# crowsonkb/k-diffusion

Measured on AMD Instinct MI355X. Metric: images/sec, 256x256 image_transformer_v2, 50-step DPM++2M (whole job), higher is better.
Workload: dtype f32

## Files before the change

### k-diffusion_amd/csrc/gemm.hip

```cpp
#include "kd_common.h"
#include <cstdlib>
#include <type_traits>

namespace kd {

constexpr int BM = 128, BN = 128, BK = 32;

using bf16x8 = __attribute__((ext_vector_type(8))) __bf16;
using u32x2 = __attribute__((ext_vector_type(2))) unsigned;

constexpr int S = BK + 4;
constexpr int NLD = BM * BK / 4 / 256;
constexpr int RT = BK / 4;
constexpr size_t EPI_STRIPS = 4 * 8 * 64 * sizeof(float);
constexpr size_t LDS_EXACT = (size_t)(2 * BM * S + 2 * BN * S + BM) * sizeof(float);
constexpr int IMG = BM * BK * 2;
constexpr int STAGE = 4 * IMG;
constexpr size_t LDS_SPLIT = (size_t)2 * STAGE + BM * sizeof(float) + EPI_STRIPS;
constexpr int WP_BLOCK = 2 * IMG;
constexpr int SCALE_TAB_MAX_K = 512;

__device__ __host__ __forceinline__ int swz(int row, int c) { return row * 64 + ((c ^ ((row >> 2) & 3)) << 4); }

__device__ __forceinline__ unsigned pack_bf16(float a, float b) {
// ... 180 lines not shown
#pragma unroll
        for (int i = 0; i < 2; ++i)
#pragma unroll
          for (int j = 0; j < 2; ++j) acc[i][j] = __builtin_amdgcn_mfma_f32_32x32x16_bf16(al[i], bh[j], acc[i][j], 0, 0, 0);
#pragma unroll
        for (int i = 0; i < 2; ++i)
#pragma unroll
          for (int j = 0; j < 2; ++j) acc[i][j] = __builtin_amdgcn_mfma_f32_32x32x16_bf16(ah[i], bl[j], acc[i][j], 0, 0, 0);
#pragma unroll
        for (int i = 0; i < 2; ++i)
#pragma unroll
          for (int j = 0; j < 2; ++j) acc[i][j] = __builtin_amdgcn_mfma_f32_32x32x16_bf16(ah[i], bh[j], acc[i][j], 0, 0, 0);
      }
    } else {
      const float* a_base = As + (buf * BM + wr * 64) * S + frag_off;
      const float* b_base = Bs + (buf * BN + wc * 64) * S + frag_off;
#pragma unroll
      for (int kk = 0; kk < BK; kk += 8) {
        const f32x4 a0 = *reinterpret_cast<const f32x4*>(a_base + kk);
        const f32x4 a1 = *reinterpret_cast<const f32x4*>(a_base + 32 * S + kk);
        const f32x4 b0 = *reinterpret_cast<const f32x4*>(b_base + kk);
        const f32x4 b1 = *reinterpret_cast<const f32x4*>(b_base + 32 * S + kk);
#pragma unroll
        for (int s = 0; s < 4; ++s) {
          acc[0][0] = __builtin_amdgcn_mfma_f32_32x32x2f32(a0[s], b0[s], acc[0][0], 0, 0, 0);
          acc[0][1] = __builtin_amdgcn_mfma_f32_32x32x2f32(a0[s], b1[s], acc[0][1], 0, 0, 0);
          acc[1][0] = __builtin_amdgcn_mfma_f32_32x32x2f32(a1[s], b0[s], acc[1][0], 0, 0, 0);
          acc[1][1] = __builtin_amdgcn_mfma_f32_32x32x2f32(a1[s], b1[s], acc[1][1], 0, 0, 0);
        }
      }
    }
  };

  load_a(kt0 * BK, ra0); load_b(kt0, rb0);
  if (nk > 1) { load_a((kt0 + 1) * BK, ra1); load_b(kt0 + 1, rb1); }
  store_tiles(0, kt0 * BK, ra0, rb0);
  __syncthreads();
  for (int kt = 0; kt < nk; kt += 2) {
    if (kt + 2 < nk) { load_a((kt0 + kt + 2) * BK, ra0); load_b(kt0 + kt + 2, rb0); }
    compute(0);
    if (kt + 1 < nk) store_tiles(1, (kt0 + kt + 1) * BK, ra1, rb1);
    __syncthreads();
    if (kt + 1 >= nk) break;
    if (kt + 3 < nk) { load_a((kt0 + kt + 3) * BK, ra1); load_b(kt0 + kt + 3, rb1); }
    compute(1);
    if (kt + 2 < nk) store_tiles(0, (kt0 + kt + 2) * BK, ra0, rb0);
    __syncthreads();
  }

  if (KS == 2) {
    f32x4* xch = reinterpret_cast<f32x4*>(reinterpret_cast<char*>(smem) + 2 * STAGE);
    if (grp == 1) {
#pragma unroll
      for (int i = 0; i < 2; ++i)
#pragma unroll
        for (int j = 0; j < 2; ++j)
#pragma unroll
          for (int q = 0; q < 4; ++q)
            xch[((i * 2 + j) * 4 + q) * 256 + tid] = f32x4{acc[i][j][4 * q], acc[i][j][4 * q + 1], acc[i][j][4 * q + 2], acc[i][j][4 * q + 3]};
    }
    __syncthreads();
    if (grp == 1) return;
#pragma unroll
    for (int i = 0; i < 2; ++i)
#pragma unroll
      for (int j = 0; j < 2; ++j)
#pragma unroll
        for (int q = 0; q < 4; ++q) {
          const f32x4 o = xch[((i * 2 + j) * 4 + q) * 256 + tid];
#pragma unroll
          for (int u = 0; u < 4; ++u) acc[i][j][4 * q + u] += o[u];
        }
  }

  if (NORM) {
#pragma unroll
    for (int j = 0; j < NLD; ++j) {
      const float s = wave_sum_xor(ssq[j], RT);
      if ((tid % RT) == 0) rs[r0 + j * (256 / RT)] = rsqrtf(s / (float)K + p.eps);
    }
    __syncthreads();
  }

  if (p.debug & 1) {
#pragma unroll
    for (int i = 0; i < 2; ++i)
#pragma unroll
      for (int j = 0; j < 2; ++j) asm volatile("" ::"v"(acc[i][j]));
    return;
  }
  const int col_l = lane & 31;
  constexpr int NW = (EPI == KD_EPI_GEGLU) ? 32 : 64;
  const int wn0 = n0 + wc * NW;
  float* strip = ebuf + wid * (8 * 64);
  const bool vec_ok = (N & 3) == 0 &&
                      (EPI != KD_EPI_SPLIT_LERP || (N & 15) == 0) &&
                      (EPI != KD_EPI_UNPATCH_NCHW || (p.pw == 4 && N <= 64 && (p.gw & 7) == 0));
  const int qk_vec = wn0 >> 6, qk_which = EPI == KD_EPI_QKV ? qk_vec / p.n_heads : 2, qk_head = EPI == KD_EPI_QKV ? qk_vec - qk_which * p.n_heads : 0;
  const float qk_sqrt = (EPI == KD_EPI_QKV && qk_which < 2) ? sqrtf(p.qk_scale[qk_head]) : 1.0f;
  if (vec_ok) {
    float c_out[2] = {1.f, 1.f}, c_skip[2] = {0.f, 0.f};
#pragma unroll
    for (int i = 0; i < 2; ++i) {
      float rsv[16];
#pragma unroll
      for (int r = 0; r < 16; ++r) rsv[r] = NORM ? rs[wr * 64 + i * 32 + mfma32_row(r, lane)] : 1.0f;
#pragma unroll
      for (int g = 0; g < 4; ++g) {
        if (EPI == KD_EPI_GEGLU) {
#pragma unroll
          for (int q = 0; q < 4; q += 2) {
            const int r = 4 * g + q, row8 = q + 4 * (lane >> 5);
            const f32x2 rs2 = {rsv[r], rsv[r + 1]};
            const f32x2 gate = f32x2{acc[i][1][r], acc[i][1][r + 1]} * rs2;
            const f32x2 val = f32x2{acc[i][0][r], acc[i][0][r + 1]} * rs2;
            const f32x2 o = (p.debug & 8) ? val * gate : geglu_pair(val * 0.5f, gate);
            strip[row8 * NW + col_l] = o.x;
            strip[(row8 + 1) * NW + col_l] = o.y;
          }
        } else {
#pragma unroll
          for (int q = 0; q < 4; ++q) {
            const int r = 4 * g + q, row8 = q + 4 * (lane >> 5);
            strip[row8 * NW + col_l] = acc[i][0][r] * rsv[r];
            strip[row8 * NW + 32 + col_l] = acc[i][1][r] * rsv[r];
          }
        }
        const int row_base = m0 + wr * 64 + i * 32 + 8 * g;
        if (EPI == KD_EPI_UNPATCH_NCHW) {
          if (wn0 < N) {
            const int items = p.chan * p.ph * 8, hw = p.gh * p.gw;
            for (int it = lane; it < items; it += 64) {
              const int tok = it & 7, cb = it >> 3, c = cb % p.chan, nh = cb / p.chan;
              const int gm = row_base + tok, gmc = min(gm, M - 1);
              const int b = gmc / hw, rr = gmc - b * hw, h = rr / p.gw, w = rr - h * p.gw;
              f32x4 v;
#pragma unroll
              for (int nw = 0; nw < 4; ++nw) v[nw] = strip[tok * NW + (nh * 4 + nw) * p.chan + c];
              const long o = (((long)b * p.chan + c) * (p.gh * p.ph) + h * p.ph + nh) * (p.gw * 4) + w * 4;
              if (p.sigma) {
                const float sg = p.sigma[b], sd = p.sigma_data, var = sg * sg + sd * sd;
                const float co = sg * sd / sqrtf(var), cs = sd * sd / var;
                const f32x4 xin = *reinterpret_cast<const f32x4*>(p.R + o);
                v = v * co + xin * cs;
              }
              if (gm < M) *reinterpret_cast<f32x4*>(p.C + o) = v;
            }
          }
          (void)c_out; (void)c_skip;
          continue;
        }
        constexpr int PER_LANE = NW / 32;
        f32x4 v[PER_LANE], rv[PER_LANE], qcs[PER_LANE], qsn[PER_LANE];
        long off[PER_LANE];
        bool ok[PER_LANE];
#pragma unroll
        for (int t = 0; t < PER_LANE; ++t) {
          const int idx = lane + 64 * t, row8 = idx / (NW / 4), c4 = (idx % (NW / 4)) * 4;
          const int gm = row_base + row8, gn = wn0 + c4;
          ok[t] = gm < M && gn < N;
          const int gmc = min(gm, M - 1), gnc = min(gn, N - 4);
          v[t] = *reinterpret_cast<const f32x4*>(strip + row8 * NW + c4);
          if (EPI == KD_EPI_SPLIT_LERP) {
            const int hw = p.gh * p.gw, Cout = N >> 2;
            const int b = gmc / hw, rr = gmc - b * hw, h = rr / p.gw, w = rr - h * p.gw;
            const int q = gnc / Cout, e = gnc - q * Cout;
            off[t] = (((long)b * (2 * p.gh) + 2 * h + (q >> 1)) * (2 * p.gw) + 2 * w + (q & 1)) * Cout + e;
          } else {
            off[t] = (long)gmc * N + gnc;
          }
          if (EPI == KD_EPI_RESIDUAL || EPI == KD_EPI_SPLIT_LERP) rv[t] = *reinterpret_cast<const f32x4*>(p.R + off[t]);
          if (EPI == KD_EPI_QKV && qk_which < 2) {
            const long tr = ((long)(gmc % p.rows_per_sample) * p.n_heads + qk_head) * KD_ROT + 4 * (lane & 3);
            qcs[t] = *reinterpret_cast<const f32x4*>(p.rope_cos + tr);
            qsn[t] = *reinterpret_cast<const f32x4*>(p.rope_sin + tr);
          }
        }
        if (EPI == KD_EPI_QKV && qk_which < 2) {
#pragma unroll
          for (int t = 0; t < PER_LANE; ++t) v[t] = prep_row16_regs(v[t], lane & 15, qk_sqrt, qcs[t], qsn[t], p.eps);
        }
#pragma unroll
        for (int t = 0; t < PER_LANE; ++t) {
          f32x4 o = v[t];
          if (EPI == KD_EPI_STORE) {
            o = o + p.out_add;
          } else if (EPI == KD_EPI_RESIDUAL) {
            o = o + rv[t];
          } else if (EPI == KD_EPI_SPLIT_LERP) {
            const float fac = *p.fac;
#pragma unroll
            for (int u = 0; u < 4; ++u) {
              const float skip = rv[t][u], diff = o[u] - skip;
              o[u] = (fabsf(fac) < 0.5f) ? skip + fac * diff : o[u] - diff * (1.0f - fac);
            }
          }
          if (EPI == KD_EPI_QKV && SPLIT && p.qkv_packed) {
            u32x2 hi, lo;
            split4(o, hi, lo);
            o = f32x4{__uint_as_float(hi[0]), __uint_as_float(hi[1]), __uint_as_float(lo[0]), __uint_as_float(lo[1])};
          }
          if (ok[t]) *reinterpret_cast<f32x4*>(p.C + off[t]) = o;
        }
      }
    }
    return;
  }

#pragma unroll
  for (int i = 0; i < 2; ++i) {
#pragma unroll
    for (int r = 0; r < 16; ++r) {
      const int row_t = wr * 64 + i * 32 + mfma32_row(r, lane);
      const int gm = m0 + row_t;
      if (gm >= M) continue;
      const float rscale = NORM ? rs[row_t] : 1.0f;
      if (EPI == KD_EPI_GEGLU) {
        const int gn = n0 + wc * 32 + col_l;
        if (gn < N) p.C[(long)gm * N + gn] = (acc[i][0][r] * rscale) * gelu_erf_fast(acc[i][1][r] * rscale);
        continue;
      }
#pragma unroll
      for (int j = 0; j < 2; ++j) {
        const int gn = n0 + wc * 64 + j * 32 + col_l;
        if (gn >= N) continue;
        const float v = acc[i][j][r] * rscale;
        if (EPI == KD_EPI_STORE) {
          p.C[(long)gm * N + gn] = v + p.out_add;
        } else if (EPI == KD_EPI_RESIDUAL) {
          const long o = (long)gm * N + gn;
          p.C[o] = v + p.R[o];
        } else if (EPI == KD_EPI_SPLIT_LERP) {
          const int hw = p.gh * p.gw, Cout = N >> 2;
          const int b = gm / hw, rr = gm % hw, h = rr / p.gw, w = rr % p.gw;
          const int q = gn / Cout, e = gn - q * Cout;
          const long o = (((long)b * (2 * p.gh) + 2 * h + (q >> 1)) * (2 * p.gw) + 2 * w + (q & 1)) * Cout + e;
          const float skip = p.R[o], fac = *p.fac;
          const float diff = v - skip;
          p.C[o] = (fabsf(fac) < 0.5f) ? skip + fac * diff : v - diff * (1.0f - fac);
        } else if (EPI == KD_EPI_UNPATCH_NCHW) {
          const int hw = p.gh * p.gw;
          const int b = gm / hw, rr = gm % hw, h = rr / p.gw, w = rr % p.gw;
          const int c = gn % p.chan, q = gn / p.chan, nh = q / p.pw, nw = q - nh * p.pw;
          const long o = (((long)b * p.chan + c) * (p.gh * p.ph) + h * p.ph + nh) * (p.gw * p.pw) + w * p.pw + nw;
          if (p.sigma) {
            const float sg = p.sigma[b], sd = p.sigma_data;
            const float var = sg * sg + sd * sd;
            const float c_skip = sd * sd / var, c_out = sg * sd / sqrtf(var);
            p.C[o] = v * c_out + p.R[o] * c_skip;
          } else {
            p.C[o] = v;
          }
        }
      }
    }
  }
}

__global__ __launch_bounds__(256) void pack_weight_kernel(const float* __restrict__ W, char* __restrict__ out, int N, int K, int geglu,
                                                           int n_tiles, int nk) {
  const long idx = (long)blockIdx.x * 256 + threadIdx.x;
  const long total = (long)n_tiles * nk * BN * 4;
  if (idx >= total) return;
  const int c = idx & 3, r = (idx >> 2) & (BN - 1);
  const long blk = idx >> 9;
  const int ks = blk % nk, nt = blk / nk;
  const int wrow = w_row_of(nt, r, N, (geglu & 1) != 0);
  float v[8];
#pragma unroll
  for (int u = 0; u < 8; ++u) {
    const int k = ks * BK + ((geglu & 2) ? 16 * (c >> 1) + 4 * (c & 1) + (u & 3) + 8 * (u >> 2) : c * 8 + u);
    v[u] = (wrow >= 0 && k < K) ? W[(long)wrow * K + k] : 0.f;
  }
  u32x2 h0, l0, h1, l1;
  split4(f32x4{v[0], v[1], v[2], v[3]}, h0, l0);
  split4(f32x4{v[4], v[5], v[6], v[7]}, h1, l1);
  char* dst = out + blk * WP_BLOCK + swz(r, c);
  *reinterpret_cast<uint4*>(dst) = uint4{h0[0], h0[1], h1[0], h1[1]};
  *reinterpret_cast<uint4*>(dst + IMG) = uint4{l0[0], l0[1], l1[0], l1[1]};
}

template <int AMODE, bool NORM, int EPI, int PREC, int KS = 1>
static int launch(const GemmP& d, hipStream_t s) {
  constexpr size_t LDS_BASE = PREC == KD_PREC_SPLIT3 ? LDS_SPLIT + (KS - 1) * 2 * STAGE : LDS_EXACT;
  constexpr size_t LDS_BYTES = LDS_BASE + (NORM ? SCALE_TAB_MAX_K * sizeof(float) : 0);
  constexpr int NCOL = (EPI == KD_EPI_GEGLU) ? 64 : BN;
  const long tiles = (long)((d.M + BM - 1) / BM) * ((d.N + NCOL - 1) / NCOL);
  const double n_eff = (EPI == KD_EPI_GEGLU) ? 2.0 * d.N : (double)d.N;
  const ProfName nm("gemm", "gemm_%s<a%d,n%d,e%d%s> M=%d N=%d K=%d", PREC == KD_PREC_SPLIT3 ? "bf16x3" : "f32", AMODE, (int)NORM, EPI, KS == 2 ? ",ks2" : "", d.M, d.N, d.K);
  const double r_bytes = (EPI == KD_EPI_RESIDUAL || EPI == KD_EPI_SPLIT_LERP || (EPI == KD_EPI_UNPATCH_NCHW && d.sigma)) ? 4.0 * d.M * d.N : 0.0;
  LaunchScope prof(nm, 2.0 * d.M * n_eff * d.K, 4.0 * ((double)d.M * d.K + n_eff * d.K + (double)d.M * d.N) + r_bytes, s);
  kd::launch<gemm_kernel<AMODE, NORM, EPI, PREC, KS>>(dim3((unsigned)tiles), dim3(256 * KS), (int)LDS_BYTES, s, d);
  return check_launch("kd_gemm_f32");
}

}

namespace kd { int gemm_astat_try(const GemmP& d, hipStream_t s, int* rc); }
namespace kd { int gemm_x3_try(const GemmP& d, hipStream_t s, int* rc); }
namespace kd { int gemm_x3t_try(const GemmP& d, hipStream_t s, int* rc); }
namespace kd { int gemm_skinny_try(const GemmP& d, hipStream_t s, int* rc); }
namespace kd { int gemm_x3r_try(const GemmP& d, hipStream_t s, int* rc); }
namespace kd { int gemm_x3s_try(const GemmP& d, hipStream_t s, int* rc); }

using namespace kd;

extern "C" int kd_gemm_f32(const KdGemm* dp, void* stream) {
  if (!dp) return fail(KD_EINVAL, "kd_gemm_f32: null descriptor");
  const KdGemm& d = *dp;
  hipStream_t s = (hipStream_t)stream;
  if (d.M <= 0 || d.N <= 0 || d.K <= 0 || (d.K & 3)) return fail(KD_EINVAL, "kd_gemm_f32: bad M/N/K %d/%d/%d (K %% 4 != 0?)", d.M, d.N, d.K);
  if (!d.A || !d.C || (!d.W && d.precision == KD_PREC_EXACT)) return fail(KD_EINVAL, "kd_gemm_f32: null A/W/C");
  if (d.norm && (!d.scale || d.rows_per_sample <= 0 || (d.scale_stride & 3))) return fail(KD_EINVAL, "kd_gemm_f32: norm needs scale, rows_per_sample, scale_stride%%4==0");
  if (d.a_mode != KD_A_PLAIN && (d.gh <= 0 || d.gw <= 0 || d.M % (d.gh * d.gw))) return fail(KD_EINVAL, "kd_gemm_f32: gather mode needs gh, gw with M %% (gh*gw) == 0");
  if (d.a_mode == KD_A_MERGE2x2 && (d.K & 15)) return fail(KD_EINVAL, "kd_gemm_f32: merge needs K %% 16 == 0");
  if (d.a_mode == KD_A_PATCH_NCHW && (d.ph <= 0 || d.pw <= 0 || d.chan <= 0 || d.K != d.ph * d.pw * d.chan)) return fail(KD_EINVAL, "kd_gemm_f32: patch gather needs K == ph*pw*chan");
  if (d.epi == KD_EPI_RESIDUAL && !d.R) return fail(KD_EINVAL, "kd_gemm_f32: residual needs R");
  if (d.epi == KD_EPI_SPLIT_LERP && (!d.R || !d.fac || (d.N & 3) || d.gh <= 0 || d.gw <= 0 || d.M % (d.gh * d.gw))) return fail(KD_EINVAL, "kd_gemm_f32: split needs R, fac, N%%4==0, gh, gw");
  if (d.epi == KD_EPI_UNPATCH_NCHW && (d.ph <= 0 || d.pw <= 0 || d.chan <= 0 || d.N != d.ph * d.pw * d.chan || d.gh <= 0 || d.gw <= 0 || d.M % (d.gh * d.gw) || (d.sigma && !d.R)))
    return fail(KD_EINVAL, "kd_gemm_f32: unpatch needs N == ph*pw*chan, gh, gw (and R when sigma is given)");
  if (d.norm && d.rows_per_sample <= 0) return fail(KD_EINVAL, "kd_gemm_f32: rows_per_sample");
  if (d.epi == KD_EPI_QKV && (d.n_heads <= 0 || d.N != 3 * d.n_heads * 64 || d.rows_per_sample <= 0 || !d.qk_scale || !d.rope_cos || !d.rope_sin))
    return fail(KD_EINVAL, "kd_gemm_f32: qkv epilogue needs N == 3*n_heads*64, rows_per_sample, qk_scale, rope_cos, rope_sin");
  if (d.qkv_packed && (d.epi != KD_EPI_QKV || d.precision != KD_PREC_SPLIT3))
    return fail(KD_EINVAL, "kd_gemm_f32: qkv_packed needs the qkv epilogue and split3 precision");
  if ((d.a_split || d.c_split) && d.precision != KD_PREC_SPLIT3) return fail(KD_EINVAL, "kd_gemm_f32: a_split / c_split are KD_PREC_SPLIT3 operand formats");
  if (d.a_split && (d.norm || d.a_mode != KD_A_PLAIN || !d.A_lo)) return fail(KD_EINVAL, "kd_gemm_f32: a_split needs A_lo, a_mode KD_A_PLAIN and no norm prologue (kd_norm_split_f32 does the norm)");
  if (d.c_split && !d.C_lo) return fail(KD_EINVAL, "kd_gemm_f32: c_split needs C_lo");
  GemmP e;
  static_cast<KdGemm&>(e) = d;
  e.debug = opt(KD_OPT_gemm_debug);
  e.warm = code_warm();
  if (e.rows_per_sample <= 0) e.rows_per_sample = e.M;
  e.scale_tab = e.norm && e.a_mode == KD_A_PLAIN && e.K <= SCALE_TAB_MAX_K && (e.scale_stride == 0 || e.rows_per_sample % BM == 0);

  if (e.a_split) {
    if (e.rows_per_sample <= 0) e.rows_per_sample = e.M;
    int rc = 0;
    if (!gemm_x3t_try(e, s, &rc)) return rc;
    return fail(KD_EINVAL, "kd_gemm_f32: no kernel for pre-split A with epi=%d M=%d N=%d K=%d (K %% 32, N %% 128 (GEGLU: 64))", d.epi, d.M, d.N, d.K);
  }
  {
    const bool skinny_on = opt(KD_OPT_skinny) != 0;
    int rc = 0;
    if (skinny_on && !gemm_skinny_try(e, s, &rc)) return rc;
    if (!gemm_x3s_try(e, s, &rc)) return rc;
  }
  {
    const bool astat_on = opt(KD_OPT_astat) != 0;
    int rc = 0;
    if (astat_on && !gemm_x3_try(e, s, &rc)) return rc;
    if (e.c_split) return fail(KD_EINVAL, "kd_gemm_f32: c_split is produced by the GEGLU projections of gemm_x3.hip (K = 128 / 256, norm) and gemm_x3t.hip (a_split) only");
    if (astat_on && !gemm_astat_try(e, s, &rc)) return rc;
    if (!gemm_x3r_try(e, s, &rc)) return rc;
  }
  if (e.precision != KD_PREC_EXACT && e.precision != KD_PREC_SPLIT3) return fail(KD_EINVAL, "kd_gemm_f32: unknown precision %d", e.precision);
  if (e.precision == KD_PREC_SPLIT3 && !e.Wp) return fail(KD_EINVAL, "kd_gemm_f32: split3 needs the packed weight image Wp (kd_pack_weight_bf16x3)");
  {
    const bool ks_on = opt(KD_OPT_ksplit) != 0;
    const long tiles = (long)((e.M + BM - 1) / BM) * ((e.N + BN - 1) / BN);
    const int nk = (e.K + BK - 1) / BK;
    if (ks_on && e.precision == KD_PREC_SPLIT3 && e.Wp && e.a_mode == KD_A_PLAIN && !e.norm && !e.debug && tiles <= 256 && nk >= 8 && nk % 4 == 0) {
      if (e.epi == KD_EPI_RESIDUAL) return launch<KD_A_PLAIN, false, KD_EPI_RESIDUAL, KD_PREC_SPLIT3, 2>(e, s);
      if (e.epi == KD_EPI_STORE) return launch<KD_A_PLAIN, false, KD_EPI_STORE, KD_PREC_SPLIT3, 2>(e, s);
    }
  }
#define KD_CASE(AM, NO, EP)                                             \
  if (e.a_mode == AM && (e.norm != 0) == NO && e.epi == EP)             \
    return e.precision == KD_PREC_SPLIT3 ? launch<AM, NO, EP, KD_PREC_SPLIT3>(e, s) : launch<AM, NO, EP, KD_PREC_EXACT>(e, s);
  KD_CASE(KD_A_PLAIN, true, KD_EPI_STORE)
  KD_CASE(KD_A_PLAIN, false, KD_EPI_STORE)
  KD_CASE(KD_A_PLAIN, false, KD_EPI_RESIDUAL)
  KD_CASE(KD_A_PLAIN, true, KD_EPI_QKV)
  KD_CASE(KD_A_PLAIN, false, KD_EPI_QKV)
  KD_CASE(KD_A_PLAIN, true, KD_EPI_GEGLU)
  KD_CASE(KD_A_PLAIN, false, KD_EPI_GEGLU)
  KD_CASE(KD_A_MERGE2x2, false, KD_EPI_STORE)
  KD_CASE(KD_A_PLAIN, false, KD_EPI_SPLIT_LERP)
  KD_CASE(KD_A_PATCH_NCHW, false, KD_EPI_STORE)
  KD_CASE(KD_A_PLAIN, true, KD_EPI_UNPATCH_NCHW)
  KD_CASE(KD_A_PLAIN, false, KD_EPI_UNPATCH_NCHW)
#undef KD_CASE
  return fail(KD_EINVAL, "kd_gemm_f32: unsupported combination a_mode=%d norm=%d epi=%d", d.a_mode, d.norm, d.epi);
}

extern "C" long long kd_packed_weight_bytes(int N, int K, int geglu) {
  if (N <= 0 || K <= 0) return 0;
  const long n_tiles = (N + ((geglu & 1) ? 64 : BN) - 1) / ((geglu & 1) ? 64 : BN), nk = (K + BK - 1) / BK;
  return n_tiles * nk * (long long)WP_BLOCK;
}

extern "C" int kd_pack_weight_bf16x3(const float* W, void* out, int N, int K, int geglu, void* stream) {
  if (!W || !out || N <= 0 || K <= 0 || geglu < 0 || geglu > 3) return fail(KD_EINVAL, "kd_pack_weight_bf16x3: bad arguments");
  const int n_tiles = (N + ((geglu & 1) ? 64 : BN) - 1) / ((geglu & 1) ? 64 : BN), nk = (K + BK - 1) / BK;
  const long total = (long)n_tiles * nk * BN * 4;
  hipLaunchKernelGGL(pack_weight_kernel, dim3((unsigned)((total + 255) / 256)), dim3(256), 0, (hipStream_t)stream, W,
                     reinterpret_cast<char*>(out), N, K, geglu, n_tiles, nk);
  return check_launch("kd_pack_weight_bf16x3");
}

KD_TEXT_PAD(gemm)
```

### k-diffusion_amd/csrc/gemm_x3.hip

```cpp
#include "x3_common.h"

namespace kd {
namespace x3 {

struct XArgs {
  const float* A; const char* Wp; float* C;
  b16::u16* Cl; int c_split;
  const float* scale; int scale_stride, rows_per_sample; float eps;
  int M, N, n_tiles, n_splits;
  int n_heads; const float* qk_scale; const float* pos; const float* freq; int qkv_packed;
  float out_add;
  const float* sigma; float sigma_data; int gh, gw, chan;
  const float* R;
  int warm;
  unsigned long long* clk;
};

template <int NC , int EPI>
__global__ __launch_bounds__(256, NC <= 8 ? 2 : 1) void gemm_x3_astat_kernel(const XArgs p) {
  constexpr int K = NC * 16, NK = NC / 2;
  constexpr int NSTG = NC <= 8 ? 4 : 8, PDIST = NSTG - 1, PB = 4;
  constexpr bool GEGLU = EPI == KD_EPI_GEGLU;
  constexpr int NCOL = GEGLU ? 64 : 128;
  constexpr int NST = GEGLU ? 8 : 16;
  constexpr int WAREA = (NSTG / 4) * STG;
  constexpr int KH = WAREA / 128 >= K ? K : WAREA / 128;
  constexpr bool AG = NC >= 32;
  constexpr int NR = K / KH, CPR = KH / 4;
  constexpr int PIECES = 32 * CPR / 64;
  constexpr int SCL = K * 4 < 1024 ? 1024 : K * 4;
  static_assert(NK % NSTG == 0 || NSTG % NK == 0, "ring slot of a stage must be a compile-time constant");
  static_assert(CPR >= 16 && NC % NR == 0, "source-side chunk swizzle spans 16 chunk positions");
  extern __shared__ __attribute__((aligned(16))) char smem[];
  const int tid = threadIdx.x, lane = tid & 63, l31 = lane & 31, lh = lane >> 5;
  const int wid = __builtin_amdgcn_readfirstlane(tid >> 6);
  const auto warm = code_warm_begin<(NC <= 8 ? 14 : 24) * 1024>((int)blockIdx.x < p.warm && tid < 64);
  const PanelSplit ps = panel_split(p.n_splits, p.n_tiles);
  const int nt_begin = ps.t_begin, n_tiles = ps.t_end - ps.t_begin, total = n_tiles * NK;
  const int m0 = ps.panel * 128;
  const bool probe = p.clk && blockIdx.x == 0 && tid == 0;
  if (probe) { p.clk[0] = __builtin_amdgcn_s_memtime(); p.clk[1] = __builtin_amdgcn_s_memrealtime(); }
  const WgStamp wgs = wg_stamp_begin(p.clk);

  f32x16 acc[4];
  if constexpr (EPI == KD_EPI_RESIDUAL) {
    const int rrow = min(m0 + wid * 32 + l31, p.M - 1);
    const float* rp = p.R + (size_t)rrow * p.N + nt_begin * NCOL + 4 * lh;
#pragma unroll
    for (int j = 0; j < 4; ++j)
#pragma unroll
      for (int g = 0; g < 4; ++g) {
        const f32x4 v = *reinterpret_cast<const f32x4*>(rp + 32 * j + 8 * g);
#pragma unroll
        for (int e = 0; e < 4; ++e) acc[j][4 * g + e] = v[e];
      }
  }

  const char* wp = p.Wp + (size_t)nt_begin * NK * STG + wid * (PB * 1024) + lane * 16;
  auto issue_piece = [&](int s_, int j) {
    const int s = min(s_, total - 1);
    const char* src = wp + (size_t)s * STG;
    char* dst = smem + (s_ % NSTG) * STG + wid * (PB * 1024);
    __builtin_amdgcn_global_load_lds((const __attribute__((address_space(1))) void*)(src + j * 1024),
                                     (__attribute__((address_space(3))) void*)(dst + j * 1024), 16, 0, 0);
  };
  auto issue = [&](int s_) {
#pragma unroll
    for (int j = 0; j < PB; ++j) issue_piece(s_, j);
  };

  const int row = m0 + wid * 32 + l31;
  const bool ok = row < p.M;
  const int rowc = ok ? row : p.M - 1;
  bf16x8 a_hi[AG ? 1 : NC], a_lo[AG ? 1 : NC];
  float rs;
  {
    char* stage = smem + wid * WAREA;
    char* scl = smem + NSTG * STG + wid * SCL;
    const int r_first = min(m0 + wid * 32, p.M - 1), r_last = min(m0 + wid * 32 + 31, p.M - 1);
    constexpr bool nrm = EPI != KD_EPI_RESIDUAL;
    const bool uni = nrm && (p.scale_stride == 0 || r_first / p.rows_per_sample == r_last / p.rows_per_sample);
    if (uni) {
      const char* ssrc = reinterpret_cast<const char*>(p.scale + (size_t)(r_first / p.rows_per_sample) * p.scale_stride);
#pragma unroll
      for (int i = 0; i < SCL / 1024; ++i)
        __builtin_amdgcn_global_load_lds((const __attribute__((address_space(1))) void*)(ssrc + (i * 1024 + lane * 16) % (K * 4)),
                                         (__attribute__((address_space(3))) void*)(scl + i * 1024), 16, 0, 0);
    }
    const float* sp = p.scale + (size_t)(rowc / p.rows_per_sample) * p.scale_stride + 8 * lh;
    const float* spl = reinterpret_cast<const float*>(scl) + 8 * lh;
    float ssq = 0.f;
    static_for<NR>([&](auto r_) {
      constexpr int r = decltype(r_)::value;
#pragma unroll
      for (int i = 0; i < PIECES; ++i) {
        const int ci = i * 64 + lane, rr = ci / CPR, qs = ci % CPR;
        const int grow = min(m0 + wid * 32 + rr, p.M - 1);
        const char* src = reinterpret_cast<const char*>(p.A + (size_t)grow * K + r * KH) + ((qs ^ (rr & 15)) << 4);
        __builtin_amdgcn_global_load_lds((const __attribute__((address_space(1))) void*)src,
                                         (__attribute__((address_space(3))) void*)(stage + i * 1024), 16, 0, 0);
      }
      asm volatile("s_waitcnt vmcnt(0)" ::: "memory");
      const char* rowp = stage + l31 * (KH * 4);
      static_for<NC / NR / 4>([&](auto c4_) {
        constexpr int c0 = r * (NC / NR) + 4 * decltype(c4_)::value;
        f32x4 x0[4], x1[4], s0[4], s1[4];
#pragma unroll
        for (int u = 0; u < 4; ++u) {
          const int q = 4 * (c0 - r * (NC / NR) + u) + 2 * lh;
          x0[u] = *reinterpret_cast<const f32x4*>(rowp + ((q ^ (l31 & 15)) << 4));
          x1[u] = *reinterpret_cast<const f32x4*>(rowp + (((q + 1) ^ (l31 & 15)) << 4));
          if constexpr (nrm) {
            if (uni) {
              s0[u] = *reinterpret_cast<const f32x4*>(spl + 16 * (c0 + u));
              s1[u] = *reinterpret_cast<const f32x4*>(spl + 16 * (c0 + u) + 4);
            } else {
              s0[u] = *reinterpret_cast<const f32x4*>(sp + 16 * (c0 + u));
              s1[u] = *reinterpret_cast<const f32x4*>(sp + 16 * (c0 + u) + 4);
            }
          }
        }
        __builtin_amdgcn_sched_barrier(0);
        static_for<4>([&](auto u_) {
          constexpr int u = decltype(u_)::value;
#pragma unroll
          for (int e = 0; e < 4; ++e) ssq = fmaf(x0[u][e], x0[u][e], fmaf(x1[u][e], x1[u][e], ssq));
          u32x4 hi, lo;
          if constexpr (nrm) split8(x0[u] * s0[u], x1[u] * s1[u], hi, lo);
          else split8(x0[u], x1[u], hi, lo);
          if constexpr (AG) {
            areg_write4<8 * (c0 + u)>(hi);
            areg_write4<8 * (c0 + u) + 4>(lo);
          } else {
            asm volatile("" : "+v"(hi), "+v"(lo));
            a_hi[c0 + u] = __builtin_bit_cast(bf16x8, hi);
            a_lo[c0 + u] = __builtin_bit_cast(bf16x8, lo);
          }
        });
        __builtin_amdgcn_sched_barrier(0);
      });
      if constexpr (NR > 1) asm volatile("s_waitcnt lgkmcnt(0)" ::: "memory");
    });
    ssq += __shfl_xor(ssq, 32, 64);
    rs = nrm ? rsqrtf(ssq / (float)K + p.eps) : 1.f;
  }
  float py = 0.f, px = 0.f;
  if (EPI == KD_EPI_QKV) {
    qk_tab_fill(reinterpret_cast<float*>(smem + NSTG * STG + 4 * SCL + 4 * 2048), tid, p);
    token_pos(p.pos, rowc % p.rows_per_sample, py, px);
  }
  code_warm_end(warm);
  asm volatile("s_waitcnt vmcnt(0) lgkmcnt(0)" ::: "memory");
  KD_BARRIER();
  const bool full_panel = m0 + 128 <= p.M;
#pragma unroll
  for (int s = 0; s < PDIST; ++s) issue(s);
  if (probe) p.clk[4] = __builtin_amdgcn_s_memtime();

  const int o0 = swz64(l31, lh), o1 = swz64(l31, 2 + lh);
  char* strip = smem + NSTG * STG + 4 * SCL + wid * 2048;
  const char* qkc = smem + NSTG * STG + 4 * SCL + 4 * 2048;
  float* st_row[2];
  bool st_ok[2];
#pragma unroll
  for (int it = 0; it < 2; ++it) {
    const int r = m0 + wid * 32 + 16 * it + (lane >> 2);
    st_ok[it] = r < p.M;
    st_row[it] = p.C + (size_t)min(r, p.M - 1) * p.N + 4 * (lane & 3);
  }
  if constexpr (EPI != KD_EPI_RESIDUAL) {
#pragma unroll
    for (int j = 0; j < 4; ++j)
#pragma unroll
      for (int r = 0; r < 16; ++r) acc[j][r] = 0.f;
  }
  if constexpr (AG) asm volatile("s_nop 3" : "+v"(acc[0]), "+v"(acc[1]), "+v"(acc[2]), "+v"(acc[3]));

  bf16x8 wh[2][4], wl[2][4];
  int ou0[2] = {0, 0}, ou1[2] = {0, 0};
  if constexpr (EPI == KD_EPI_UNPATCH_NCHW) {
#pragma unroll
    for (int j = 0; j < 2; ++j) {
      const int np = 32 * j + l31, q = np >> 2, py = q / p.chan, cch = q - py * p.chan;
      const int n = np < 16 * p.chan ? (py * 4 + (np & 3)) * p.chan + cch : np;
      ou0[j] = swz64(n, lh);
      ou1[j] = swz64(n, 2 + lh);
    }
  }
  auto read_frags = [&](int slot, int h, bf16x8 (&fh)[4], bf16x8 (&fl)[4]) {
    if constexpr (EPI == KD_EPI_UNPATCH_NCHW) {
#pragma unroll
      for (int j = 0; j < 2; ++j) {
        const char* st = smem + slot * STG + (h ? ou1[j] : ou0[j]);
        fh[j] = *reinterpret_cast<const bf16x8*>(st);
        fl[j] = *reinterpret_cast<const bf16x8*>(st + IMG);
      }
    } else {
      const char* st = smem + slot * STG + (h ? o1 : o0);
#pragma unroll
      for (int j = 0; j < 4; ++j) {
        fh[j] = *reinterpret_cast<const bf16x8*>(st + j * 32 * 64);
        fl[j] = *reinterpret_cast<const bf16x8*>(st + IMG + j * 32 * 64);
      }
    }
  };
  wait_vm(PB * (PDIST - 1));
  KD_BARRIER();
  read_frags(0, 0, wh[0], wl[0]);

  for (int nt = 0; nt < n_tiles; ++nt) {
    static_for<NK>([&](auto ks_) {
      constexpr int ks = decltype(ks_)::value;
      const int s = nt * NK + ks;
      auto mm = [&](auto b_, int j, bool w_lo, auto a_lo_) {
        constexpr int b = decltype(b_)::value, al = decltype(a_lo_)::value, c = 2 * ks + b;
        if (EPI == KD_EPI_UNPATCH_NCHW && j >= 2) return;
        const bf16x8& w = w_lo ? wl[b][j] : wh[b][j];
        if constexpr (AG) mfma_ag<8 * c + 4 * al>(acc[j], w);
        else mfma_a(acc[j], w, al ? a_lo[c] : a_hi[c]);
      };
      constexpr std::integral_constant<int, 0> I0{};
      constexpr std::integral_constant<int, 1> I1{};
      if constexpr (AG) {
        mm(I0, 0, true, I0);
        __builtin_amdgcn_sched_barrier(0);
        read_frags(ks % NSTG, 1, wh[1], wl[1]);
        __builtin_amdgcn_sched_barrier(0);
#pragma unroll
        for (int j = 1; j < 4; ++j) mm(I0, j, true, I0);
      } else {
        read_frags(ks % NSTG, 1, wh[1], wl[1]);
#pragma unroll
        for (int j = 0; j < 4; ++j) mm(I0, j, true, I0);
      }
#pragma unroll
      for (int j = 0; j < 4; ++j) mm(I0, j, false, I1);
#pragma unroll
      for (int j = 0; j < 4; ++j) mm(I0, j, false, I0);
      if constexpr (!AG) {
        __builtin_amdgcn_sched_group_barrier(0x008, 1, 0);
        __builtin_amdgcn_sched_group_barrier(0x100, 8, 0);
        __builtin_amdgcn_sched_group_barrier(0x008, 11, 0);
      }
      __builtin_amdgcn_sched_barrier(0);
      {
        int allow = PB * (PDIST - 2);
        if (full_panel && nt > 0 && ks + 2 <= PDIST) allow += NST;
        wait_vm(allow);
        KD_BARRIER();
      }
      mm(I1, 0, true, I0);
      if constexpr (AG) __builtin_amdgcn_sched_barrier(0);
      read_frags((ks + 1) % NSTG, 0, wh[0], wl[0]);
      if constexpr (!AG) {
        __builtin_amdgcn_sched_group_barrier(0x008, 1, 0);
        __builtin_amdgcn_sched_group_barrier(0x100, 8, 0);
      }
      __builtin_amdgcn_sched_barrier(0);
      mm(I1, 1, true, I0);
      mm(I1, 2, true, I0);
      issue_piece(s + PDIST, 0);
      __builtin_amdgcn_sched_barrier(0);
      mm(I1, 3, true, I0);
      mm(I1, 0, false, I1);
      mm(I1, 1, false, I1);
      issue_piece(s + PDIST, 1);
      __builtin_amdgcn_sched_barrier(0);
      mm(I1, 2, false, I1);
      mm(I1, 3, false, I1);
      mm(I1, 0, false, I0);
      issue_piece(s + PDIST, 2);
      __builtin_amdgcn_sched_barrier(0);
      mm(I1, 1, false, I0);
      mm(I1, 2, false, I0);
      issue_piece(s + PDIST, 3);
      mm(I1, 3, false, I0);
      __builtin_amdgcn_sched_barrier(0);
    });
    if constexpr (AG) asm volatile("s_nop 15\n\ts_nop 3" : "+v"(acc[0]), "+v"(acc[1]), "+v"(acc[2]), "+v"(acc[3]));
    if (probe && nt == 0) p.clk[5] = __builtin_amdgcn_s_memtime();

    const int n0 = (nt_begin + nt) * NCOL;
    auto store_block = [&](const f32x4 (&v)[4], int col) {
#pragma unroll
      for (int hb = 0; hb < 2; ++hb) {
#pragma unroll
        for (int gg = 0; gg < 2; ++gg)
          *reinterpret_cast<f32x4*>(strip + l31 * 64 + (((2 * gg + lh) ^ ((l31 >> 2) & 1)) << 4)) = v[2 * hb + gg];
#pragma unroll
        for (int it = 0; it < 2; ++it) {
          const int r16 = 16 * it + (lane >> 2), c = lane & 3;
          const f32x4 o = *reinterpret_cast<const f32x4*>(strip + r16 * 64 + ((c ^ ((r16 >> 2) & 1)) << 4));
          if (st_ok[it]) st16(st_row[it] + col + 16 * hb, o);
        }
      }
    };
    if (GEGLU) {
      const float rsh = 0.5f * rs;
#pragma unroll
      for (int jj = 0; jj < 2; ++jj) {
        f32x4 blk[4];
#pragma unroll
        for (int g = 0; g < 4; ++g) {
          const f32x2 a = geglu_pair(f32x2{acc[2 * jj][4 * g], acc[2 * jj][4 * g + 1]} * rsh, f32x2{acc[2 * jj + 1][4 * g], acc[2 * jj + 1][4 * g + 1]} * rs);
          const f32x2 b = geglu_pair(f32x2{acc[2 * jj][4 * g + 2], acc[2 * jj][4 * g + 3]} * rsh, f32x2{acc[2 * jj + 1][4 * g + 2], acc[2 * jj + 1][4 * g + 3]} * rs);
          blk[g] = f32x4{a.x, a.y, b.x, b.y};
        }
        if (p.c_split) {
          float v[16], hi[16], lo[16];
#pragma unroll
          for (int g = 0; g < 4; ++g)
#pragma unroll
            for (int q = 0; q < 4; ++q) v[4 * g + q] = blk[g][q];
#pragma unroll
          for (int r = 0; r < 16; r += 2) {
            const unsigned h = pack_bf16(v[r], v[r + 1]);
            hi[r] = b16::bf_lo(h);
            hi[r + 1] = b16::bf_hi(h);
            lo[r] = v[r] - hi[r];
            lo[r + 1] = v[r + 1] - hi[r + 1];
          }
          const size_t off = (size_t)rowc * p.N + n0 + 32 * jj;
          b16::store_block_bf16(reinterpret_cast<b16::u16*>(p.C) + off, hi, lh, ok);
          b16::store_block_bf16(p.Cl + off, lo, lh, ok);
        } else {
          store_block(blk, n0 + 32 * jj);
        }
      }
    } else if (EPI == KD_EPI_QKV) {
#pragma unroll
      for (int vv = 0; vv < 2; ++vv) {
        const int vec = (n0 >> 6) + vv;
        const int which = vec >= 2 * p.n_heads ? 2 : (vec >= p.n_heads ? 1 : 0), head = vec - which * p.n_heads;
        f32x16& a0 = acc[2 * vv];
        f32x16& a1 = acc[2 * vv + 1];
        if (which < 2) {
          qk_prep_head(qkc, head, lh, a0, a1, rs, p.eps, py, px);
        } else {
#pragma unroll
          for (int r = 0; r < 16; ++r) { a0[r] *= rs; a1[r] *= rs; }
        }
#pragma unroll
        for (int jj = 0; jj < 2; ++jj) {
          f32x4 blk[4];
          const f32x16& a = jj ? a1 : a0;
          if (p.qkv_packed) {
#pragma unroll
            for (int g = 0; g < 4; ++g) blk[g] = pack_split4(f32x4{a[4 * g], a[4 * g + 1], a[4 * g + 2], a[4 * g + 3]});
          } else {
#pragma unroll
            for (int g = 0; g < 4; ++g) blk[g] = f32x4{a[4 * g], a[4 * g + 1], a[4 * g + 2], a[4 * g + 3]};
          }
          store_block(blk, n0 + 64 * vv + 32 * jj);
        }
      }
    } else if (EPI == KD_EPI_UNPATCH_NCHW) {
      const int per = p.gh * p.gw, bb = rowc / per, rr = rowc - bb * per, ty = rr / p.gw, tx = rr - ty * p.gw;
      float c_out = 1.f, c_skip = 0.f;
      if (p.sigma) {
        const float sg = p.sigma[bb], sd = p.sigma_data, var = sg * sg + sd * sd;
        c_skip = sd * sd / var;
        c_out = sg * sd / sqrtf(var);
      }
      const int Himg = 4 * p.gh, Wimg = 4 * p.gw;
#pragma unroll
      for (int j = 0; j < 2; ++j)
#pragma unroll
        for (int g = 0; g < 4; ++g) {
          const int q = 8 * j + 2 * g + lh, py = q / p.chan, cch = q - py * p.chan;
          if (q < 4 * p.chan && ok) {
            const size_t o = (((size_t)bb * p.chan + cch) * Himg + 4 * ty + py) * Wimg + 4 * tx;
            f32x4 v = f32x4{acc[j][4 * g], acc[j][4 * g + 1], acc[j][4 * g + 2], acc[j][4 * g + 3]} * (rs * c_out);
            if (p.sigma) v = v + *reinterpret_cast<const f32x4*>(p.R + o) * c_skip;
            st16(p.C + o, v);
          }
        }
    } else {
#pragma unroll
      for (int j = 0; j < 4; ++j) {
        f32x4 blk[4];
#pragma unroll
        for (int g = 0; g < 4; ++g) blk[g] = f32x4{acc[j][4 * g], acc[j][4 * g + 1], acc[j][4 * g + 2], acc[j][4 * g + 3]} * rs + p.out_add;
        store_block(blk, n0 + 32 * j);
      }
    }
    if (probe && nt == 0) p.clk[6] = __builtin_amdgcn_s_memtime();
#pragma unroll
    for (int j = 0; j < 4; ++j)
#pragma unroll
      for (int r = 0; r < 16; ++r) acc[j][r] = 0.f;
    if constexpr (AG) asm volatile("s_nop 3" : "+v"(acc[0]), "+v"(acc[1]), "+v"(acc[2]), "+v"(acc[3]));
  }
  asm volatile("s_waitcnt vmcnt(0)" ::: "memory");
  if (probe) { p.clk[2] = __builtin_amdgcn_s_memtime(); p.clk[3] = __builtin_amdgcn_s_memrealtime(); p.clk[7] = (unsigned long long)total; }
  wg_stamp_end(wgs);
}

template <int EPI>
__global__ __launch_bounds__(256, 2) void gemm_x3h_kernel(const XArgs p) {
  constexpr int NC = 16, K = 256, NK = 8;
  constexpr int NSTG = 4, PDIST = NSTG - 1, PB = 4, UNIT = 4;
  constexpr bool GEGLU = EPI == KD_EPI_GEGLU;
  constexpr int HCOL = GEGLU ? 32 : 64;
  constexpr int NST = GEGLU ? 4 : 8;
  constexpr int KH = 128, NR = K / KH, CPR = KH / 4, PIECES = 32 * CPR / 64, SCL = 1024, SUB = 8192, HALF = 4096, CB = 2;
  extern __shared__ __attribute__((aligned(16))) char smem[];
  const int tid = threadIdx.x, lane = tid & 63, l31 = lane & 31, lh = lane >> 5;
  const int wid = __builtin_amdgcn_readfirstlane(tid >> 6);
  const auto warm = code_warm_begin<20 * 1024>((int)blockIdx.x < p.warm && tid < 64);
  const PanelSplit ps = panel_split(p.n_splits, p.n_tiles);
  const int ht_begin = ps.t_begin, n_ht = ps.t_end - ps.t_begin, total = n_ht * UNIT;
  const int m0 = ps.panel * 128;
  const bool probe = p.clk && blockIdx.x == (gridDim.x * 5) / 8 && tid == 0;
  if (probe) { p.clk[0] = __builtin_amdgcn_s_memtime(); p.clk[1] = __builtin_amdgcn_s_memrealtime(); }
  const WgStamp wgs = wg_stamp_begin(p.clk);

  const char* wp = p.Wp + wid * 1024 + lane * 16;
  auto issue_piece = [&](int q_, int j) {
    const int q = min(q_, total - 1), ht = ht_begin + (q >> 2), u = q & 3;
    const char* src = wp + ((size_t)(ht >> 1) * NK + 2 * u + (j >> 1)) * STG + (j & 1) * IMG + (ht & 1) * HALF;
    char* dst = smem + (q_ % NSTG) * STG + (j >> 1) * SUB + (j & 1) * HALF + wid * 1024;
    __builtin_amdgcn_global_load_lds((const __attribute__((address_space(1))) void*)src, (__attribute__((address_space(3))) void*)dst, 16, 0, 0);
  };

  const int row = m0 + wid * 32 + l31;
  const bool ok = row < p.M;
  const int rowc = ok ? row : p.M - 1;
  float rs;
  {
    char* stage = smem + wid * STG;
    char* scl = smem + NSTG * STG + wid * SCL;
    const int r_first = min(m0 + wid * 32, p.M - 1), r_last = min(m0 + wid * 32 + 31, p.M - 1);
    const bool uni = p.scale_stride == 0 || r_first / p.rows_per_sample == r_last / p.rows_per_sample;
    if (uni) {
      const char* ssrc = reinterpret_cast<const char*>(p.scale + (size_t)(r_first / p.rows_per_sample) * p.scale_stride);
      __builtin_amdgcn_global_load_lds((const __attribute__((address_space(1))) void*)(ssrc + lane * 16),
                                       (__attribute__((address_space(3))) void*)scl, 16, 0, 0);
    }
    const float* sp = p.scale + (size_t)(rowc / p.rows_per_sample) * p.scale_stride + 8 * lh;
    const float* spl = reinterpret_cast<const float*>(scl) + 8 * lh;
    float ssq = 0.f;
    static_for<NR>([&](auto r_) {
      constexpr int r = decltype(r_)::value;
#pragma unroll
      for (int i = 0; i < PIECES; ++i) {
        const int ci = i * 64 + lane, rr = ci / CPR, qs = ci % CPR;
        const int grow = min(m0 + wid * 32 + rr, p.M - 1);
        const char* src = reinterpret_cast<const char*>(p.A + (size_t)grow * K + r * KH) + ((qs ^ (rr & 15)) << 4);
        __builtin_amdgcn_global_load_lds((const __attribute__((address_space(1))) void*)src,
                                         (__attribute__((address_space(3))) void*)(stage + i * 1024), 16, 0, 0);
      }
      asm volatile("s_waitcnt vmcnt(0)" ::: "memory");
      const char* rowp = stage + l31 * (KH * 4);
      static_for<NC / NR / CB>([&](auto c4_) {
        constexpr int c0 = r * (NC / NR) + CB * decltype(c4_)::value;
        f32x4 x0[CB], x1[CB], s0[CB], s1[CB];
#pragma unroll
        for (int u = 0; u < CB; ++u) {
          const int q = 4 * (c0 - r * (NC / NR) + u) + 2 * lh;
          x0[u] = *reinterpret_cast<const f32x4*>(rowp + ((q ^ (l31 & 15)) << 4));
          x1[u] = *reinterpret_cast<const f32x4*>(rowp + (((q + 1) ^ (l31 & 15)) << 4));
          if (uni) {
            s0[u] = *reinterpret_cast<const f32x4*>(spl + 16 * (c0 + u));
            s1[u] = *reinterpret_cast<const f32x4*>(spl + 16 * (c0 + u) + 4);
          } else {
            s0[u] = *reinterpret_cast<const f32x4*>(sp + 16 * (c0 + u));
            s1[u] = *reinterpret_cast<const f32x4*>(sp + 16 * (c0 + u) + 4);
          }
        }
        __builtin_amdgcn_sched_barrier(0);
        static_for<CB>([&](auto u_) {
          constexpr int u = decltype(u_)::value;
#pragma unroll
          for (int e = 0; e < 4; ++e) ssq = fmaf(x0[u][e], x0[u][e], fmaf(x1[u][e], x1[u][e], ssq));
          u32x4 hi, lo;
          split8(x0[u] * s0[u], x1[u] * s1[u], hi, lo);
          areg_write4_lo<8 * (c0 + u)>(hi);
          areg_write4_lo<8 * (c0 + u) + 4>(lo);
        });
        __builtin_amdgcn_sched_barrier(0);
      });
      if constexpr (r + 1 < NR) asm volatile("s_waitcnt lgkmcnt(0)" ::: "memory");
    });
    ssq += __shfl_xor(ssq, 32, 64);
    rs = rsqrtf(ssq / (float)K + p.eps);
  }
  float py = 0.f, px = 0.f;
  if (EPI == KD_EPI_QKV) {
    qk_tab_fill(reinterpret_cast<float*>(smem + NSTG * STG + 4 * SCL + 4 * 2048), tid, p);
    token_pos(p.pos, rowc % p.rows_per_sample, py, px);
  }
  code_warm_end(warm);
  asm volatile("s_waitcnt vmcnt(0) lgkmcnt(0)" ::: "memory");
  KD_BARRIER();
  const bool full_panel = m0 + 128 <= p.M;
#pragma unroll
  for (int s = 0; s < PDIST; ++s)
#pragma unroll
    for (int j = 0; j < PB; ++j) issue_piece(s, j);
  if (probe) p.clk[4] = __builtin_amdgcn_s_memtime();

  const int o0 = swz64(l31, lh), o1 = swz64(l31, 2 + lh);
  char* strip = smem + NSTG * STG + 4 * SCL + wid * 2048;
  const char* qkc = smem + NSTG * STG + 4 * SCL + 4 * 2048;
  float* st_row[2];
  bool st_ok[2];
#pragma unroll
  for (int it = 0; it < 2; ++it) {
    const int r = m0 + wid * 32 + 16 * it + (lane >> 2);
    st_ok[it] = r < p.M;
    st_row[it] = p.C + (size_t)min(r, p.M - 1) * p.N + 4 * (lane & 3);
  }
  f32x16 acc[2];
  bf16x8 uh[2][2], ul[2][2];
  auto read_up = [&](int slot, int cc, bf16x8 (&fh)[2], bf16x8 (&fl)[2]) {
    const char* st = smem + slot * STG + (cc >> 1) * SUB + ((cc & 1) ? o1 : o0);
#pragma unroll
    for (int j = 0; j < 2; ++j) {
      fh[j] = *reinterpret_cast<const bf16x8*>(st + j * 32 * 64);
      fl[j] = *reinterpret_cast<const bf16x8*>(st + HALF + j * 32 * 64);
    }
  };
  auto store_block = [&](const f32x4 (&v)[4], int col) {
#pragma unroll
    for (int hb = 0; hb < 2; ++hb) {
#pragma unroll
      for (int gg = 0; gg < 2; ++gg)
        *reinterpret_cast<f32x4*>(strip + l31 * 64 + (((2 * gg + lh) ^ ((l31 >> 2) & 1)) << 4)) = v[2 * hb + gg];
#pragma unroll
      for (int it = 0; it < 2; ++it) {
        const int r16 = 16 * it + (lane >> 2), c = lane & 3;
        const f32x4 o = *reinterpret_cast<const f32x4*>(strip + r16 * 64 + ((c ^ ((r16 >> 2) & 1)) << 4));
        if (st_ok[it]) st16(st_row[it] + col + 16 * hb, o);
      }
    }
  };
  wait_vm(PB * (PDIST - 1));
  KD_BARRIER();
  read_up(0, 0, uh[0], ul[0]);

  constexpr std::integral_constant<int, 0> I0{};
  constexpr std::integral_constant<int, 1> I1{};
  constexpr std::integral_constant<int, 2> I2{};
  constexpr std::integral_constant<int, 3> I3{};
  constexpr std::integral_constant<int, 4> I4{};
  constexpr std::integral_constant<int, 5> I5{};
  for (int h = 0; h < n_ht; ++h) {
    if (probe && h == 1) p.clk[8] = __builtin_amdgcn_s_memtime();
    static_for<UNIT>([&](auto u_) {
      constexpr int u = decltype(u_)::value;
      const int s = h * UNIT + u;
      auto mm = [&](auto cc_, auto i_) {
        constexpr int cc = decltype(cc_)::value, i = decltype(i_)::value, j = i & 1, term = i >> 1, c = 4 * u + cc;
        const bf16x8& w = term == 0 ? ul[cc & 1][j] : uh[cc & 1][j];
        constexpr int al = term == 1;
        if constexpr (c == 0 && term == 0) mfma_ag0<8 * c + 4 * al>(acc[j], w);
        else mfma_ag<8 * c + 4 * al>(acc[j], w);
      };
      mm(I0, I0);
      __builtin_amdgcn_sched_barrier(0);
      read_up(u, 1, uh[1], ul[1]);
      __builtin_amdgcn_sched_barrier(0);
      mm(I0, I1); mm(I0, I2); mm(I0, I3); mm(I0, I4); mm(I0, I5);
      mm(I1, I0);
      __builtin_amdgcn_sched_barrier(0);
      read_up(u, 2, uh[0], ul[0]);
      __builtin_amdgcn_sched_barrier(0);
      mm(I1, I1); mm(I1, I2); mm(I1, I3); mm(I1, I4); mm(I1, I5);
      __builtin_amdgcn_sched_barrier(0);
      {
        int allow = PB * (PDIST - 2);
        if (full_panel && h > 0 && u + 2 <= PDIST) allow += NST;
        wait_vm(allow);
        KD_BARRIER();
      }
      mm(I2, I0);
      __builtin_amdgcn_sched_barrier(0);
      read_up(u, 3, uh[1], ul[1]);
      __builtin_amdgcn_sched_barrier(0);
      mm(I2, I1); mm(I2, I2);
      issue_piece(s + PDIST, 0);
      __builtin_amdgcn_sched_barrier(0);
      mm(I2, I3); mm(I2, I4); mm(I2, I5);
      issue_piece(s + PDIST, 1);
      __builtin_amdgcn_sched_barrier(0);
      mm(I3, I0);
      __builtin_amdgcn_sched_barrier(0);
      read_up((u + 1) % NSTG, 0, uh[0], ul[0]);
      __builtin_amdgcn_sched_barrier(0);
      mm(I3, I1); mm(I3, I2);
      issue_piece(s + PDIST, 2);
      __builtin_amdgcn_sched_barrier(0);
      mm(I3, I3); mm(I3, I4);
      issue_piece(s + PDIST, 3);
      mm(I3, I5);
      __builtin_amdgcn_sched_barrier(0);
    });
    asm volatile("s_nop 15\n\ts_nop 3" : "+v"(acc[0]), "+v"(acc[1]));
    if (probe && h == 1) p.clk[9] = __builtin_amdgcn_s_memtime();

    const int n0 = (ht_begin + h) * HCOL;
    if (GEGLU) {
      const float rsh = 0.5f * rs;
      f32x4 blk[4];
#pragma unroll
      for (int g = 0; g < 4; ++g) {
        const f32x2 a = geglu_pair(f32x2{acc[0][4 * g], acc[0][4 * g + 1]} * rsh, f32x2{acc[1][4 * g], acc[1][4 * g + 1]} * rs);
        const f32x2 b = geglu_pair(f32x2{acc[0][4 * g + 2], acc[0][4 * g + 3]} * rsh, f32x2{acc[1][4 * g + 2], acc[1][4 * g + 3]} * rs);
        blk[g] = f32x4{a.x, a.y, b.x, b.y};
      }
      store_block(blk, n0);
    } else if (EPI == KD_EPI_QKV) {
      const int vec = n0 >> 6;
      const int which = vec >= 2 * p.n_heads ? 2 : (vec >= p.n_heads ? 1 : 0), head = vec - which * p.n_heads;
      if (which < 2) {
        qk_prep_head(qkc, head, lh, acc[0], acc[1], rs, p.eps, py, px);
      } else {
#pragma unroll
        for (int r = 0; r < 16; ++r) { acc[0][r] *= rs; acc[1][r] *= rs; }
      }
#pragma unroll
      for (int jj = 0; jj < 2; ++jj) {
        f32x4 blk[4];
        const f32x16& a = acc[jj];
        if (p.qkv_packed) {
#pragma unroll
          for (int g = 0; g < 4; ++g) blk[g] = pack_split4(f32x4{a[4 * g], a[4 * g + 1], a[4 * g + 2], a[4 * g + 3]});
        } else {
#pragma unroll
          for (int g = 0; g < 4; ++g) blk[g] = f32x4{a[4 * g], a[4 * g + 1], a[4 * g + 2], a[4 * g + 3]};
        }
        store_block(blk, n0 + 32 * jj);
      }
    } else {
#pragma unroll
      for (int j = 0; j < 2; ++j) {
        f32x4 blk[4];
#pragma unroll
        for (int g = 0; g < 4; ++g) blk[g] = f32x4{acc[j][4 * g], acc[j][4 * g + 1], acc[j][4 * g + 2], acc[j][4 * g + 3]} * rs + p.out_add;
        store_block(blk, n0 + 32 * j);
      }
    }
    if (probe && h == 1) p.clk[10] = __builtin_amdgcn_s_memtime();
  }
  asm volatile("s_waitcnt vmcnt(0)" ::: "memory");
  if (probe) { p.clk[2] = __builtin_amdgcn_s_memtime(); p.clk[3] = __builtin_amdgcn_s_memrealtime(); p.clk[7] = (unsigned long long)total; }
  wg_stamp_end(wgs);
}

unsigned long long* g_clk = nullptr;


template <int NC, int EPI>
static int launch(const XArgs& a0, const char* nm, double flops, double bytes, hipStream_t s, int force_splits = 0) {
  constexpr int K = NC * 16, NSTG = NC <= 8 ? 4 : 8;
  constexpr int LDS = NSTG * STG + 4 * (K * 4 < 1024 ? 1024 : K * 4) + 4 * 2048 + 1024;
  const int panels = (a0.M + 127) / 128, best = best_n_splits(panels, a0.n_tiles, (NC <= 8 ? 2 : 1) * cu_count(), 1);
  const int forced = force_splits ? force_splits : opt(KD_OPT_x3_splits);
  XArgs a = a0;
  a.n_splits = forced > 0 && forced <= a0.n_tiles ? forced : best;
  const CfgName cfg(nm, "splits%d", a.n_splits);
  LaunchScope prof(cfg, flops, bytes, s);
  kd::launch<gemm_x3_astat_kernel<NC, EPI>>(dim3((unsigned)(panels * a.n_splits)), dim3(256), LDS, s, a);
  return check_launch("kd_gemm_f32(x3 astat)");
}

template <int EPI>
static int launch_half(const XArgs& a0, const char* nm, double flops, double bytes, hipStream_t s) {
  constexpr int LDS = 4 * STG + 4 * 1024 + 4 * 2048 + 1024;
  const int panels = (a0.M + 127) / 128, best = best_n_splits(panels, a0.n_tiles, 2 * cu_count(), 2);
  const int forced = opt(KD_OPT_x3_splits);
  XArgs a = a0;
  a.n_splits = forced > 0 && forced <= a0.n_tiles && a0.n_tiles % forced == 0 ? forced : best;
  const CfgName cfg(nm, "splits%d", a.n_splits);
  LaunchScope prof(cfg, flops, bytes, s);
  kd::launch<gemm_x3h_kernel<EPI>>(dim3((unsigned)(panels * a.n_splits)), dim3(256), LDS, s, a);
  return check_launch("kd_gemm_f32(x3 half tiles)");
}

}

int gemm_x3_try(const GemmP& d, hipStream_t s, int* rc) {
  using namespace x3;
  if (!opt(KD_OPT_x3)) return 1;
  if (d.precision != KD_PREC_SPLIT3 || d.a_mode != KD_A_PLAIN || !d.Wp || d.debug) return 1;
  const bool unpatch = d.epi == KD_EPI_UNPATCH_NCHW;
  if (unpatch && (d.K != 128 || !d.norm || d.ph != 4 || d.pw != 4 || d.N != 16 * d.chan || d.N > 64 || !opt(KD_OPT_x3_unpatch))) return 1;
  if (d.epi != KD_EPI_STORE && d.epi != KD_EPI_QKV && d.epi != KD_EPI_GEGLU && d.epi != KD_EPI_RESIDUAL && !unpatch) return 1;
  if (d.epi == KD_EPI_RESIDUAL ? (d.norm || !d.R || d.K != 512 || !opt(KD_OPT_x3_res)) : !d.norm) return 1;
  if (d.K != 128 && d.K != 256 && d.K != 512) return 1;
  const int ncol = d.epi == KD_EPI_GEGLU ? 64 : 128;
  if ((!unpatch && d.N % ncol) || d.M < opt(KD_OPT_x3_min_rows) || (d.norm && d.rows_per_sample <= 0)) return 1;
  if (d.epi == KD_EPI_QKV && (!d.rope_pos || !d.rope_freq || d.n_heads > 16)) return 1;
  if (d.c_split && (d.epi != KD_EPI_GEGLU || !d.C_lo || (d.N & 31))) return 1;
  XArgs a{};
  a.A = d.A; a.Wp = reinterpret_cast<const char*>(d.Wp); a.C = d.C;
  a.scale = d.norm ? d.scale : nullptr; a.R = d.R; a.scale_stride = d.scale_stride; a.rows_per_sample = d.rows_per_sample > 0 ? d.rows_per_sample : d.M; a.eps = d.eps;
  a.M = d.M; a.N = d.N; a.n_tiles = unpatch ? 1 : d.N / ncol; a.n_splits = 1;
  a.sigma = d.sigma; a.sigma_data = d.sigma_data; a.gh = d.gh; a.gw = d.gw; a.chan = d.chan;
// ... 33 lines not shown
```

### k-diffusion_amd/models/image_transformer_v2.py

```python
import ctypes as C
import os
import math
from dataclasses import dataclass
from typing import NamedTuple, Optional, Union

import torch
from torch import nn

from .. import _native as nat
from .. import ops
from .. import weights
from . import axial_rope
from .cond_tables import ScaleTables

D_HEAD = 64
DERIVED_KEPT = 1024
MAX_PLANS = 16
PLAN_SWITCHES = (("KDIFF_ATTN_BLOCK", "1"), ("KDIFF_PROJ_BLOCK", "1"), ("KDIFF_FFN_OUT", "all"), ("KDIFF_RUN_LIST", "1"), ("KDIFF_ATTN_FFN", "1"))
CLASS_IDS_KEPT = 4



@dataclass
class GlobalAttentionSpec:
    d_head: int


@dataclass
class NeighborhoodAttentionSpec:
    d_head: int
    kernel_size: int


@dataclass
class ShiftedWindowAttentionSpec:
    d_head: int
    window_size: int


@dataclass
class NoAttentionSpec:
    pass


@dataclass
class LevelSpec:
    depth: int
    width: int
    d_ff: int
    self_attn: Union[GlobalAttentionSpec, NeighborhoodAttentionSpec, ShiftedWindowAttentionSpec, NoAttentionSpec]
    dropout: float


@dataclass
class MappingSpec:
    depth: int
    width: int
    d_ff: int
    dropout: float



class _Holder(nn.Module):

    def __init__(self, **children):
        super().__init__()
        for k, v in children.items():
            if isinstance(v, nn.Parameter):
                self.register_parameter(k, v)
            elif isinstance(v, torch.Tensor):
                self.register_buffer(k, v)
            else:
                self.add_module(k, v)


def _linear_weight(out_f, in_f, zero=False):
    w = torch.zeros(out_f, in_f)
    if not zero:
        bound = 1.0 / math.sqrt(in_f)
        w.uniform_(-bound, bound)
    return _Holder(weight=nn.Parameter(w))


def _layer(spec: LevelSpec, cond_features: int):
    d, parts = spec.width, {}
    if not isinstance(spec.self_attn, NoAttentionSpec):
        nh = d // spec.self_attn.d_head
        parts["self_attn"] = _Holder(
            scale=nn.Parameter(torch.full([nh], 10.0)),
            norm=_Holder(linear=_linear_weight(d, cond_features, zero=True)),
            qkv_proj=_linear_weight(3 * d, d),
            pos_emb=_Holder(freqs=axial_rope.rope_freqs(spec.self_attn.d_head // 2, nh)),
            out_proj=_linear_weight(d, d, zero=True))
    parts["ff"] = _Holder(norm=_Holder(linear=_linear_weight(d, cond_features, zero=True)),
                          up_proj=_linear_weight(2 * spec.d_ff, d),
                          down_proj=_linear_weight(d, spec.d_ff, zero=True))
    return _Holder(**parts)


def _rms_scale(n):
    return _Holder(scale=nn.Parameter(torch.ones(n)))



_ATTN_KIND = {GlobalAttentionSpec: "global", NeighborhoodAttentionSpec: "neighborhood", ShiftedWindowAttentionSpec: "shifted-window"}
_CORE = {"global": "attn_global", "neighborhood": "attn_na2d", "shifted-window": "attn_window"}


def attn_geometry(spec, index):
    kind = _ATTN_KIND[type(spec)]
    if kind == "global":
        params = ()
    elif kind == "neighborhood":
        params = (spec.kernel_size,)
    else:
        params = (spec.window_size, spec.window_size // 2 if index % 2 == 1 else 0)
    return kind, _CORE[kind], params


class Step(NamedTuple):
    kind: str
    level: int
    prefix: str = ""
    module: Optional[nn.Module] = None
    index: int = 0


def hourglass(model):
    steps, top = [], len(model.level_specs) - 1
    for li in range(top):
        steps += [Step("layer", li, f"down_levels.{li}.{i}.", mod, i) for i, mod in enumerate(model.down_levels[li])]
        steps.append(Step("merge", li))
    steps += [Step("layer", top, f"mid_level.{i}.", mod, i) for i, mod in enumerate(model.mid_level)]
    for li in reversed(range(top)):
        steps.append(Step("split", li))
        depth = model.level_specs[li].depth
        steps += [Step("layer", li, f"up_levels.{li}.{i}.", mod, i + depth) for i, mod in enumerate(model.up_levels[li])]
    return steps


DROPOUT_SITE = 1 << 62


def dropout_sites(model):
    out = []
    for i, st in enumerate(hourglass(model)):
        p = model.level_specs[st.level].dropout if st.kind == "layer" else 0.0
        if p > 0:
            if hasattr(st.module, "self_attn"):
                out.append((DROPOUT_SITE | 2 * i, st, "attn", p))
            out.append((DROPOUT_SITE | (2 * i + 1), st, "ff", p))
    p = model.mapping_spec.dropout
    if p > 0:
        out += [(DROPOUT_SITE | 1 << 32 | k, k, "mapping", p) for k in range(len(model.mapping.blocks))]
    return out


def dropout_table(model, key):
    if key is None:
        return {}
    return {(("mapping", where) if kind == "mapping" else (where.prefix, kind)): (key, site, p) for site, where, kind, p in dropout_sites(model)}


def _level_pos(grids, li):
    h0, w0 = grids[0]
    pos = axial_rope.make_axial_pos(h0, w0).view(h0, w0, 2)
    for _ in range(li):
        pos = axial_rope.downscale_pos(pos)
    return pos



EPS = 1e-6


def conditioning(model, sigma, aug_cond, class_cond, mapping_cond, keep=None, drop=None):
    m = model
    B = sigma.shape[0]
    dev = sigma.device
    ff = ops.fourier_sigma(sigma, m.time_emb.weight.detach().contiguous())
    temb = ops.linear(ff, m.time_in_proj.weight)
    aug = torch.zeros(B, 9, device=dev, dtype=torch.float32) if aug_cond is None else aug_cond.to(device=dev, dtype=torch.float32).reshape(B, 9).contiguous()
    aug_ff = ops.fourier_features(aug, m.aug_emb.weight.detach().contiguous())
    aug_proj = ops.linear(aug_ff, m.aug_in_proj.weight)
    emb = ids = None
    if m.class_emb is not None:
        ids = class_cond.to(device=dev, dtype=torch.int64).reshape(B).contiguous()
        lo, hi = (int(ids.min()), int(ids.max()))
        if lo < 0 or hi >= m.class_emb.weight.shape[0]:
            raise IndexError(f"class_cond ids must lie in [0, {m.class_emb.weight.shape[0] - 1}] (got {lo}..{hi})")
        emb = m.class_emb.weight
    mterm = None
    if m.mapping_cond_in_proj is not None:
        mrows = mapping_cond.to(device=dev, dtype=torch.float32).reshape(B, -1).contiguous()
        mterm = ops.linear(mrows, m.mapping_cond_in_proj.weight)
    c = ops.cond_sum(temb, aug_proj, emb=emb, ids=ids, c=mterm)
    if keep is not None:
        keep.update(time_ff=ff, aug_ff=aug_ff, ids=ids, mapping_rows=mrows if mterm is not None else None, blocks=[])
    c_sum = c
    c = ops.rms_norm(c, m.mapping.in_norm.scale)
    for k, blk in enumerate(m.mapping.blocks):
        if keep is not None:
            keep["blocks"].append(c)
        h = ops.norm_linear(c, blk.norm.scale, blk.up_proj.weight, rows_per_sample=B, epi=nat.EPI_GEGLU)
        dr = drop.get(("mapping", k)) if drop else None
        if dr is not None:
            ops.dropout(h, *dr, out=h)
        c = ops.linear(h, blk.down_proj.weight, residual=c)
    if keep is not None:
        keep.update(c_sum=c_sum, c_last=c)
    return ops.rms_norm(c, m.mapping.out_norm.scale)


def ada_scale(cond, norm):
    return ops.linear(cond, norm.linear.weight, out_add=1.0)




@dataclass(frozen=True)
class LayerRoute:
    qkv: Optional[str]
    core: Optional[str]
    fuse_out: bool
    ff: str
    up: Optional[str] = None
    down_mx8: bool = False
    fuse_core: bool = False


def _prepass(mode, width):
    return mode == nat.PREC_SPLIT3 and width not in (128, 256, 512) and width > 256 and width % 128 == 0 and width <= 2048


def _mx8_ok(lib, mode, M, N, K, epi):
    return mode == nat.PREC_FP8 and M >= lib.kd_get_option(b"mx8_min_rows", nat.OPTION_DEFAULT) and bool(lib.kd_gemm_mx8_supported(M, N, K, epi, 1))


def route_layer(lib, mode, B, T, rps, d, d_ff, nh, attn, switches, grid=None, kernel_size=None):
    bf = mode in (nat.PREC_BF16, nat.PREC_FP8)
    proj_block = bf and switches["KDIFF_PROJ_BLOCK"] != "0"
    ffn_x3 = mode == nat.PREC_SPLIT3 and bool(lib.kd_ffn_f32_supported(T, d, d_ff))
    ffn_bf = bf and bool(lib.kd_ffn_bf16_supported(T, d, d_ff))
    fo = switches["KDIFF_FFN_OUT"]
    fuse_out = attn is not None and ((ffn_x3 and d in (128, 256)) or (ffn_bf and d == 128)) and (d == 128 if fo == "1" else fo in ("all", str(d)))
    qkv = core = None
    if attn is not None:
        if bf and attn == "global" and T % 256 == 0 and switches["KDIFF_ATTN_BLOCK"] != "0" and lib.kd_attn_block_bf16_supported(rps, d, nh) \
                and (B * nh >= 32 or switches["KDIFF_ATTN_BLOCK"] == "force"):
            qkv = "attn_block"
        elif _prepass(mode, d) and nh <= 16:
            qkv = "split"
        elif _mx8_ok(lib, mode, T, 3 * d, d, nat.EPI_QKV):
            qkv = "mx8"
        elif proj_block and lib.kd_proj_block_bf16_supported(rps, d, 3 * d, nat.EPI_QKV) and 192 <= (T // 256) * (3 * d // 384) <= 256:
            qkv = "proj_block"
        else:
            qkv = "plain"
        if qkv != "attn_block":
            core = f"kd_{_CORE[attn]}_{'bf16' if bf else 'f32'}"
    if ffn_x3 or ffn_bf:
        fuse_core = bool(ffn_x3 and fuse_out and attn == "neighborhood" and core == "kd_attn_na2d_f32" and grid is not None
                         and kernel_size is not None and switches.get("KDIFF_ATTN_FFN", "1") != "0"
                         and lib.kd_attn_ffn_f32_supported(B, grid[0], grid[1], nh, kernel_size, d, d_ff))
        return LayerRoute(qkv, core, fuse_out, "kd_ffn_f32" if ffn_x3 else "kd_ffn_bf16", fuse_core=fuse_core)
    if _prepass(mode, d) and d_ff % 64 == 0:
        return LayerRoute(qkv, core, fuse_out, "pair", "split")
    up_mx8 = _mx8_ok(lib, mode, T, d_ff, d, nat.EPI_GEGLU)
    down_mx8 = up_mx8 and d_ff % 128 == 0 and bool(lib.kd_gemm_mx8_supported(T, d, d_ff, nat.EPI_RESIDUAL, 0))
    if up_mx8:
        up = "mx8"
    elif proj_block and lib.kd_proj_block_bf16_supported(rps, d, d_ff, nat.EPI_GEGLU) and 192 <= (T // 256) * (d_ff // 192) <= 256:
        up = "proj_block"
    else:
        up = "plain"
    return LayerRoute(qkv, core, fuse_out, "pair", up, down_mx8)



class _Launch:
    __slots__ = ("name", "args", "what")

    def __init__(self, name, args, what):
        self.name, self.args, self.what = name, args, what

    def __call__(self, lib, stream):
        return getattr(lib, self.name)(*[C.byref(a) if isinstance(a, C.Structure) else a.scale if isinstance(a, _ScaleRef) else a
                                         for a in self.args], stream)


class _ScaleRef:

    def __init__(self):
        self._scale, self._call, self._index = None, None, 0

    def bind_call(self, call, index):
        self._call, self._index = call, index

    @property
    def scale(self):
        return self._scale

    @scale.setter
    def scale(self, v):
        self._scale = v
        if self._call is not None:
            self._call.p[self._index] = v


def _ptr(t):
    return C.c_void_p(t.data_ptr())


class _CondChain:

    def __init__(self, rows, lib):
        self.rows, self.lib, self.launches, self.keep = rows, lib, [], []
        self.c_sigma = self.class_ids = self.aug_in = self.map_in = self.d_scales = None

    def fill(self, sigma, aug_cond, class_cond, mapping_cond, repeat=1):
        rows = self.rows
        self.c_sigma.copy_(sigma.reshape(-1).expand(rows) if sigma.numel() == 1 else sigma.reshape(rows), non_blocking=True)
        B = rows // repeat
        if self.class_ids is not None and class_cond is not None:
            self.class_ids.view(repeat, B).copy_(class_cond.reshape(1, B).expand(repeat, B), non_blocking=True)
        if self.aug_in is not None:
            self.aug_in.view(repeat, B, 9).copy_(aug_cond.reshape(1, B, 9).expand(repeat, B, 9), non_blocking=True)
        if self.map_in is not None:
            self.map_in.view(repeat, B, -1).copy_(mapping_cond.reshape(1, B, -1).expand(repeat, B, -1), non_blocking=True)

    def run(self, table_ptr, stream):
        self.d_scales.C = table_ptr
        for ln in self.launches:
            rc = ln(self.lib, stream)
            if rc:
                nat.check(rc, ln.what)


class _Plan:

    def release(self):
        self.__dict__.clear()

    def __init__(self, model, B, H, W, grids, has_aug, has_class, has_mapping_cond, device, mode, switches):
        self.lib = nat.lib()
        m = self.model = model
        self.mode, self.switches = mode, switches
        self.precision = precision = nat.PREC_BF16 if mode == nat.PREC_FP8 else mode
        bf = precision == nat.PREC_BF16
        self.cond_precision = nat.PREC_SPLIT3 if bf else precision
        self.has_aug, self.has_class, self.has_mapping_cond, self.device = has_aug, has_class, has_mapping_cond, device
        self.keep = []
        self.launches = []
        f32 = dict(device=device, dtype=torch.float32)
        act = dict(device=device, dtype=torch.bfloat16 if bf else torch.float32)
        ph, pw = m.patch_size
        levels = self.levels = m.level_specs
        self.B, self.grids = B, grids
        self.out_shape = (B, m.out_channels, H, W)
        self.class_checked = {}

        self.sigma = torch.empty(B, **f32)
        self.sigma_ptr = self.sigma.data_ptr()
        self.xs = xs = [torch.empty(B, gh, gw, lv.width, **act) for (gh, gw), lv in zip(grids, levels)]
        self.toks = toks = [B * gh * gw for gh, gw in grids]
        self.qkv = torch.empty(max(t * 3 * lv.width for t, lv in zip(toks, levels)), **act)
        self.att = torch.empty(max(t * lv.width for t, lv in zip(toks, levels)), **act)
        self.hid = torch.empty(max(t * lv.d_ff for t, lv in zip(toks, levels)), **act)
        wide = [t * lv.width for t, lv in zip(toks, levels) if _prepass(mode, lv.width)]
        self.xn = torch.empty(max(wide), **f32) if wide else None
        norm_mods = m._ada_norm_modules()
        self.table_offsets, total = {}, 0
        for name, mod in norm_mods:
            self.table_offsets[name] = 4 * total
            total += mod.linear.weight.shape[0]
        wcat = m._packed.get("ada_norm_wcat")
        if wcat is None or wcat.device != device:
            wcat = m._packed["ada_norm_wcat"] = torch.cat([mod.linear.weight.detach() for _, mod in norm_mods], dim=0).contiguous()
        self.wcat = wcat
        self.norm_descs = []
        self.scale_width = total
        self.tables = ScaleTables(B, total, device, self.build_cond)

        L = self.launches
        self.d_patch_in = self._gemm(L, "patch_in", None, m.patch_in.proj.weight, xs[0], toks[0], levels[0].width, m.in_channels * ph * pw,
                                     a_mode=nat.A_PATCH_NCHW, grid=grids[0], patch=(ph, pw, m.in_channels))
        for st in hourglass(m):
            li = st.level
            if st.kind == "layer":
                self._add_layer(li, st.prefix, st.module, st.index)
            elif st.kind == "merge":
                self._gemm(L, f"merges.{li}", xs[li], m.merges[li].proj.weight, xs[li + 1], toks[li + 1], levels[li + 1].width,
                           4 * levels[li].width, a_mode=nat.A_MERGE2x2, grid=grids[li + 1])
            else:
                self._gemm(L, f"splits.{li}", xs[li + 1], m.splits[li].proj.weight, xs[li], toks[li + 1], 4 * levels[li].width,
                           levels[li + 1].width, epi=nat.EPI_SPLIT_LERP, residual=xs[li], fac=m.splits[li].fac, grid=grids[li + 1])
        self.d_patch_out = self._gemm(L, "patch_out", xs[0], m.patch_out.proj.weight, None, toks[0], m.out_channels * ph * pw,
                                      levels[0].width, epi=nat.EPI_UNPATCH_NCHW, norm_scale=m.out_norm.scale, scale_stride=0,
                                      rows_per_sample=grids[0][0] * grids[0][1], grid=grids[0], patch=(ph, pw, m.out_channels))
        self._encode_launches()

    def _gemm(self, launches, what, A, Wt, Cc, M, N, K, cond=False, table=None, entry=None, mx8=False, **kw):
        precision = self.cond_precision if cond else self.precision
        if table is not None:
            kw.update(scale_ptr=0, scale_stride=self.scale_width)
        d = ops.gemm(A, Wt, Cc, M=M, N=N, K=K, precision=precision, per_row=cond, mx8=mx8, launch=False, pack=self.model._packed_image, **kw)
        if table is not None:
            self.norm_descs.append((d, self.table_offsets[table]))
        launches.append(_Launch(entry or ops._gemm_entry(precision, mx8), (d,), what + ("(mx8)" if mx8 else "")))
        return d

    def _norm_split(self, launches, table, x, T, d, rps):
        ref = _ScaleRef()
        self.norm_descs.append((ref, self.table_offsets[table]))
        planes = self.xn.view(torch.bfloat16)
        hi, lo = planes[:T * d], planes[T * d:2 * T * d]
        launches.append(_Launch("kd_norm_split_f32", (_ptr(x), ref, self.scale_width, rps, _ptr(hi), _ptr(lo), T, d, 1e-6), table + " (split)"))
        return hi, lo

    def build_cond(self, rows):
        m, f32 = self.model, dict(device=self.device, dtype=torch.float32)
        mw, mdff = m.mapping_spec.width, m.mapping_spec.d_ff
        ch = _CondChain(rows, self.lib)
        L = ch.launches
        ch.c_sigma = torch.empty(rows, **f32)
        ch.class_ids = torch.zeros(rows, device=self.device, dtype=torch.int64)
        ch.aug_in = torch.zeros(rows, 9, **f32) if self.has_aug else None
        ch.map_in = torch.zeros(rows, m.mapping_cond_dim, **f32) if self.has_mapping_cond else None
        ff, temb, emb, mres, cond = (torch.empty(rows, mw, **f32) for _ in range(5))
        mh = torch.empty(rows, mdff, **f32)
        ch.keep += [ff, temb, emb, mres, cond, mh]
        L.append(_Launch("kd_fourier_sigma_f32", (_ptr(ch.c_sigma), _ptr(m.time_emb.weight), _ptr(ff), rows, mw // 2), "fourier_sigma"))
        self._gemm(L, "time_in_proj", ff, m.time_in_proj.weight, temb, rows, mw, mw, cond=True)
        if self.has_aug:
            aug_ff, aug_proj = torch.empty(rows, mw, **f32), torch.empty(rows, mw, **f32)
            ch.keep += [aug_ff, aug_proj]
            L.append(_Launch("kd_fourier_f32", (_ptr(ch.aug_in), _ptr(m.aug_emb.weight), _ptr(aug_ff), rows, 9, mw // 2), "fourier_aug"))
            self._gemm(L, "aug_in_proj", aug_ff, m.aug_in_proj.weight, aug_proj, rows, mw, mw, cond=True)
            aug_term, aug_rows = aug_proj, 1
        else:
            z_ff, aug_const = torch.empty(1, mw, **f32), torch.empty(1, mw, **f32)
            zeros9 = torch.zeros(1, 9, **f32)
            ch.keep += [z_ff, aug_const, zeros9]
            L.append(_Launch("kd_fourier_f32", (_ptr(zeros9), _ptr(m.aug_emb.weight), _ptr(z_ff), 1, 9, mw // 2), "fourier_aug0"))
            self._gemm(L, "aug_in_proj0", z_ff, m.aug_in_proj.weight, aug_const, 1, mw, mw, cond=True)
            aug_term, aug_rows = aug_const, 0
        map_term = None
        if self.has_mapping_cond:
            map_term = torch.empty(rows, mw, **f32)
            ch.keep.append(map_term)
            self._gemm(L, "mapping_cond_in_proj", ch.map_in, m.mapping_cond_in_proj.weight, map_term, rows, mw, m.mapping_cond_dim, cond=True)
        L.append(_Launch("kd_cond_sum_f32", (_ptr(emb), _ptr(temb), _ptr(aug_term), aug_rows,
                                             _ptr(m.class_emb.weight) if self.has_class else None, _ptr(ch.class_ids) if self.has_class else None,
                                             None if map_term is None else _ptr(map_term), rows, mw), "cond_sum"))
        L.append(_Launch("kd_rmsnorm_f32", (_ptr(emb), _ptr(m.mapping.in_norm.scale), _ptr(mres), rows, mw, C.c_float(1e-6)), "mapping.in_norm"))
        for blk in m.mapping.blocks:
            self._gemm(L, "mapping.up_proj", mres, blk.up_proj.weight, mh, rows, mdff, mw, cond=True, epi=nat.EPI_GEGLU,
                       norm_scale=blk.norm.scale, scale_stride=0, rows_per_sample=rows)
            self._gemm(L, "mapping.down_proj", mh, blk.down_proj.weight, mres, rows, mw, mdff, cond=True, epi=nat.EPI_RESIDUAL, residual=mres)
        L.append(_Launch("kd_rmsnorm_f32", (_ptr(mres), _ptr(m.mapping.out_norm.scale), _ptr(cond), rows, mw, C.c_float(1e-6)), "mapping.out_norm"))
        ch.d_scales = self._gemm(L, "ada_norm_scales", cond, self.wcat, None, rows, self.scale_width, mw, cond=True, out_add=1.0)
        return ch

    def _qk(self, li, sa, nh):
        m = self.model
        if self.precision == nat.PREC_BF16:
            cos_t, sin_t = m._rope(li, self.grids, sa, self.device, revs=True)
        else:
            cos_t, sin_t = m._rope(li, self.grids, sa, self.device)
        self.keep += [cos_t, sin_t]
        qk = (sa.scale, cos_t, sin_t, nh)
        if self.precision == nat.PREC_SPLIT3:
            pos_t, freq_t = m._rope(li, self.grids, sa, self.device, revs=True)
            self.keep += [pos_t, freq_t]
            qk += (pos_t, freq_t)
        return qk

    def _add_layer(self, li, prefix, mod, index):
        L, lv, (gh, gw), T = self.launches, self.levels[li], self.grids[li], self.toks[li]
        d, d_ff, x, rps = lv.width, lv.d_ff, self.xs[li], gh * gw
        spec = lv.self_attn
        nh = d // spec.d_head if hasattr(mod, "self_attn") else 0
        kind, core, params = attn_geometry(spec, index) if nh else (None, None, ())
        r = route_layer(self.lib, self.mode, self.B, T, rps, d, d_ff, nh, kind, self.switches, grid=(gh, gw),
                        kernel_size=params[0] if kind == "neighborhood" else None)
        split3 = self.precision == nat.PREC_SPLIT3
        if nh:
            sa, norm = mod.self_attn, prefix + "self_attn.norm"
            q = dict(epi=nat.EPI_QKV, rows_per_sample=rps, qk=self._qk(li, sa, nh), qkv_packed=split3)
            if r.qkv == "attn_block":
                self._gemm(L, prefix + "attn_block", x, sa.qkv_proj.weight, self.att, T, 3 * d, d, table=norm, entry="kd_attn_block_bf16", **q)
            elif r.qkv == "split":
                planes = self._norm_split(L, norm, x, T, d, rps)
                self._gemm(L, prefix + "qkv_proj", None, sa.qkv_proj.weight, self.qkv, T, 3 * d, d, a_planes=planes, **q)
            elif r.qkv == "proj_block":
                self._gemm(L, prefix + "qkv_proj(block)", x, sa.qkv_proj.weight, self.qkv, T, 3 * d, d, table=norm, entry="kd_proj_block_bf16", **q)
            else:
                self._gemm(L, prefix + "qkv_proj", x, sa.qkv_proj.weight, self.qkv, T, 3 * d, d, table=norm, mx8=r.qkv == "mx8", **q)
            if r.core is not None and not r.fuse_core:
                geo = ((rps, nh) if kind == "global" else (gh, gw, nh)) + params
                prep = () if r.core.endswith("_bf16") else (2 if split3 else 0, None, None, None, C.c_float(1e-6), self.precision)
                L.append(_Launch(r.core, (_ptr(self.qkv), _ptr(self.att), self.B, *geo, *prep), prefix + core))
            if not r.fuse_out:
                self._gemm(L, prefix + "out_proj", self.att, sa.out_proj.weight, x, T, d, d, epi=nat.EPI_RESIDUAL, residual=x)
        norm, w_up, w_down = prefix + "ff.norm", mod.ff.up_proj.weight, mod.ff.down_proj.weight
        if r.ff != "pair":
            fd = ops.ffn(x, None, w_up, w_down, out=x, scale_stride=self.scale_width, rows_per_sample=rps, attn=self.att if r.fuse_out else None,
                         w_out=mod.self_attn.out_proj.weight if r.fuse_out else None, launch=False, pack=self.model._packed_image)
            self.norm_descs.append((fd, self.table_offsets[norm]))
            if r.fuse_core:
                L.append(_Launch("kd_attn_ffn_f32", (_ptr(self.qkv), fd, self.B, gh, gw, nh, *params), prefix + core + "+ff"))
            else:
                L.append(_Launch(r.ff, (fd,), prefix + "ff"))
            return
        hid8 = None
        if r.up == "split":
            planes = self._norm_split(L, norm, x, T, d, rps)
            self._gemm(L, prefix + "up_proj", None, w_up, self.hid, T, d_ff, d, epi=nat.EPI_GEGLU, a_planes=planes)
        else:
            if r.down_mx8:
                b = self.hid.view(torch.uint8)
                hid8 = (b[:T * d_ff], b[T * d_ff:T * d_ff + T * d_ff // 32])
            block = r.up == "proj_block"
            self._gemm(L, prefix + ("up_proj(block)" if block else "up_proj"), x, w_up, self.hid, T, d_ff, d, epi=nat.EPI_GEGLU, table=norm,
                       rows_per_sample=rps, mx8=r.up == "mx8", c_planes=hid8, entry="kd_proj_block_bf16" if block else None)
        if r.down_mx8:
            self._gemm(L, prefix + "down_proj", None, w_down, x, T, d, d_ff, epi=nat.EPI_RESIDUAL, residual=x, a_planes=hid8, mx8=True)
        else:
            self._gemm(L, prefix + "down_proj", self.hid, w_down, x, T, d, d_ff, epi=nat.EPI_RESIDUAL, residual=x)

    def run(self, x, out, sigma_data, base):
        for d, off in self.norm_descs:
            d.scale = base + off
        pin, pout = self.d_patch_in, self.d_patch_out
        pin.A = x.data_ptr()
        pout.C = out.data_ptr()
        if sigma_data is None:
            pin.sigma, pout.sigma, pout.R = None, None, None
        else:
            sp = self.sigma_ptr
            pin.sigma, pout.sigma, pout.R = sp, sp, x.data_ptr()
            pin.sigma_data = pout.sigma_data = float(sigma_data)
        stream = C.c_void_p(torch.cuda.current_stream().cuda_stream)
        if self.calls is not None:
            rc = self.run_list(self.calls, len(self.launches), stream, C.byref(self.failed))
            if rc:
                nat.check(rc, self.launches[self.failed.value].what)
            return
        for ln in self.launches:
            rc = ln(self.lib, stream)
            if rc:
                nat.check(rc, ln.what)

    def _encode_launches(self):
        self.calls, self.failed, self.run_list = None, C.c_int(0), self.lib.kd_run_list
        if self.switches["KDIFF_RUN_LIST"] == "0" or not self.launches:
            return
        calls = (nat.KdCall * len(self.launches))()
        for call, ln in zip(calls, self.launches):
            if not nat.encode_call(call, ln.name, ln.args):
                return
        self.calls = calls



def _wants_input_grad(x):
    return torch.is_grad_enabled() and isinstance(x, torch.Tensor) and x.requires_grad


class _InputGrad(torch.autograd.Function):

    @staticmethod
    def forward(ctx, x, model, sigma, aug_cond, class_cond, mapping_cond, sigma_data):
        for name, t in (("sigma", sigma), ("aug_cond", aug_cond), ("class_cond", class_cond), ("mapping_cond", mapping_cond)):
            if isinstance(t, torch.Tensor) and t.requires_grad:
                raise NotImplementedError(f"ImageTransformerDenoiserModelV2: gradients w.r.t. {name} are not implemented (the backward pass "
                                          f"differentiates w.r.t. the input x only); pass {name}.detach()")
        out = model._run(x, sigma, aug_cond, class_cond, mapping_cond, sigma_data)
        ctx.model, ctx.sigma_data = model, sigma_data
        ctx.save_for_backward(x, sigma, aug_cond, class_cond, mapping_cond)
        return out

    @staticmethod
    def backward(ctx, grad):
        from . import vjp
        x, sigma, aug_cond, class_cond, mapping_cond = ctx.saved_tensors
        gx = vjp.backward(ctx.model, x, sigma, grad.to(torch.float32).contiguous(), aug_cond=aug_cond, class_cond=class_cond,
                          mapping_cond=mapping_cond, sigma_data=ctx.sigma_data)
        return gx, None, None, None, None, None, None


class _ParamGrad(torch.autograd.Function):

    @staticmethod
    def forward(ctx, x, model, sigma, aug_cond, class_cond, mapping_cond, key, *params):
        from . import vjp
        out = vjp.primal(model, x, sigma, aug_cond, class_cond, mapping_cond, dropout=key)
        ctx.model, ctx.params = model, params
        ctx.save_for_backward(x, sigma, aug_cond, class_cond, mapping_cond, key)
        return out

    @staticmethod
    def backward(ctx, grad):
        from . import vjp
        x, sigma, aug_cond, class_cond, mapping_cond, key = ctx.saved_tensors
        need = ctx.needs_input_grad[7:]
        want = [p for p, n in zip(ctx.params, need) if n]
        _, grads = vjp.backward(ctx.model, x, sigma, grad.to(torch.float32).contiguous(), aug_cond=aug_cond, class_cond=class_cond,
                                mapping_cond=mapping_cond, params=want, dropout=key)
        return (None,) * 7 + tuple(grads.get(id(p)) if n else None for p, n in zip(ctx.params, need))


class ImageTransformerDenoiserModelV2(nn.Module):
    def __init__(self, levels, mapping, in_channels, out_channels, patch_size, num_classes=0, mapping_cond_dim=0):
        super().__init__()
        for lv in levels:
            sa = lv.self_attn
            if not isinstance(sa, (GlobalAttentionSpec, NeighborhoodAttentionSpec, ShiftedWindowAttentionSpec, NoAttentionSpec)):
                raise ValueError(f"unsupported self attention spec {sa}")
            if not isinstance(sa, NoAttentionSpec) and sa.d_head != D_HEAD:
                raise ValueError(f"d_head must be {D_HEAD} (got {sa.d_head}): the HIP kernels of both arithmetic modes -- qkv epilogue (cosine-sim "
                                 f"norm + RoPE over {D_HEAD // 2} dims), attention cores, qkv layout [tokens, 3, n_heads, {D_HEAD}] of "
                                 f"include/kdiff_hip.h -- are built for {D_HEAD}-dim heads, as every shipped config uses (config.py:137-138); "
                                 f"the reference's other head sizes (image_transformer_v2.py:355-363) are not supported")
            if not isinstance(sa, NoAttentionSpec) and lv.width % sa.d_head:
                raise ValueError(f"width {lv.width} is not a multiple of d_head {sa.d_head}")
        self.level_specs, self.mapping_spec = list(levels), mapping
        self.in_channels, self.out_channels = in_channels, out_channels
        self.patch_size = (patch_size, patch_size) if isinstance(patch_size, int) else tuple(patch_size)
        self.num_classes, self.mapping_cond_dim = num_classes, mapping_cond_dim
        ph, pw = self.patch_size
        mw = mapping.width

        self.patch_in = _Holder(proj=_linear_weight(levels[0].width, in_channels * ph * pw))
        self.time_emb = _Holder(weight=torch.randn(mw // 2, 1))
        self.time_in_proj = _linear_weight(mw, mw)
        self.aug_emb = _Holder(weight=torch.randn(mw // 2, 9))
        self.aug_in_proj = _linear_weight(mw, mw)
        self.class_emb = _Holder(weight=nn.Parameter(torch.randn(num_classes, mw))) if num_classes else None
        self.mapping_cond_in_proj = _linear_weight(mw, mapping_cond_dim) if mapping_cond_dim else None
        self.mapping = _Holder(
            in_norm=_rms_scale(mw),
            blocks=nn.ModuleList([_Holder(norm=_rms_scale(mw), up_proj=_linear_weight(2 * mapping.d_ff, mw),
                                          down_proj=_linear_weight(mw, mapping.d_ff, zero=True)) for _ in range(mapping.depth)]),
            out_norm=_rms_scale(mw))
        self.down_levels, self.up_levels = nn.ModuleList(), nn.ModuleList()
        for i, lv in enumerate(levels):
            if i < len(levels) - 1:
                self.down_levels.append(nn.ModuleList([_layer(lv, mw) for _ in range(lv.depth)]))
                self.up_levels.append(nn.ModuleList([_layer(lv, mw) for _ in range(lv.depth)]))
            else:
                self.mid_level = nn.ModuleList([_layer(lv, mw) for _ in range(lv.depth)])
        self.merges = nn.ModuleList([_Holder(proj=_linear_weight(b.width, 4 * a.width)) for a, b in zip(levels[:-1], levels[1:])])
        self.splits = nn.ModuleList([_Holder(proj=_linear_weight(4 * a.width, b.width), fac=nn.Parameter(torch.ones(1) * 0.5))
                                     for a, b in zip(levels[:-1], levels[1:])])
        self.out_norm = _rms_scale(levels[0].width)
        self.patch_out = _Holder(proj=_linear_weight(out_channels * ph * pw, levels[0].width, zero=True))
        self._watch, self._plan_cache = weights.WeightWatch(self), weights.PlanCache()
        self._plans = self._plan_cache.plans
        self._fingerprint, self._packed, self._derived, self._plans_epoch = None, {}, {}, None
        self._dropout_on, self._dropout_gen = False, None
        self.wgrad_arithmetic = None

    def _ada_norm_modules(self):
        out = []

        def visit(prefix, layers):
            for i, mod in enumerate(layers):
                if hasattr(mod, "self_attn"):
                    out.append((f"{prefix}{i}.self_attn.norm", mod.self_attn.norm))
                out.append((f"{prefix}{i}.ff.norm", mod.ff.norm))
        for li, lvl in enumerate(self.down_levels):
            visit(f"down_levels.{li}.", lvl)
        for li, lvl in enumerate(self.up_levels):
            visit(f"up_levels.{li}.", lvl)
        visit("mid_level.", self.mid_level)
        return out

    def _derive(self, tag, sources, build):
        key = (tag, *[weights.ident(t, never_same=False) for t in sources])
        ent = self._derived.get(key)
        if ent is None:
            if len(self._derived) >= DERIVED_KEPT:
                self._derived.clear()
            ent = self._derived[key] = (sources, build())
        return ent[1]

    def _rope(self, li, grids, sa, device, revs=False):
        freqs = sa.pos_emb.freqs

        def build():
            pos = _level_pos(grids, li)
            if revs:
                freq = freqs.detach().to(torch.float32).cpu() / (2.0 * math.pi)
                return pos.reshape(-1, 2).to(torch.float32).contiguous().to(device), freq.contiguous().to(device)
            cos_t, sin_t = axial_rope.rope_tables(pos, freqs.detach())
            return cos_t.to(device), sin_t.to(device)
        return self._derive(("rope", li, grids[0], device, revs), (freqs,), build)

    def _drop_plans(self):
        self._plan_cache.drop_all()

    def invalidate(self):
        self._watch.bump()
        self._derived = {}

    def _apply(self, fn, *args, **kwargs):
        out = super()._apply(fn, *args, **kwargs)
        self._watch.bump()
        return out

    def _packed_image(self, W, N, K, geglu, bf16=False):
        key = (id(W), N, K, int(geglu), bf16 if bf16 == "mx8" else bool(bf16))
        ent = self._packed.get(key)
        if ent is None:
            ent = self._packed[key] = (W, ops.pack_weight(W, N, K, geglu, cache=False, bf16=bf16))
        return ent[1]

    def _weights_fingerprint(self):
        return self._watch.fingerprint()

    def _param_tags(self, name):
        tags = set()
        if name.endswith(".weight") and not name.startswith(("time_in_proj.", "aug_in_proj.", "class_emb.", "mapping_cond_in_proj.")):
            tags.add("wd")
        if name.startswith("mapping.") or name.endswith(".norm.linear.weight"):
            tags.add("mapping")
        return tags

    def param_groups(self, base_lr=5e-4, mapping_lr_scale=1 / 3):
        groups = {(wd, mp): [] for mp in (False, True) for wd in (True, False)}
        for name, p in self.named_parameters():
            tags = self._param_tags(name)
            groups[("wd" in tags, "mapping" in tags)].append(p)
        return [
            {"params": groups[(True, False)], "lr": base_lr},
            {"params": groups[(False, False)], "lr": base_lr, "weight_decay": 0.0},
            {"params": groups[(True, True)], "lr": base_lr * mapping_lr_scale},
            {"params": groups[(False, True)], "lr": base_lr * mapping_lr_scale, "weight_decay": 0.0},
        ]

    def _dropout_rates(self):
        return [(f"levels[{i}].dropout", lv.dropout) for i, lv in enumerate(self.level_specs)] + [("mapping dropout", self.mapping_spec.dropout)]

    def enable_dropout(self, generator=None):
        bad = [f"{name} = {p}" for name, p in self._dropout_rates() if not 0.0 <= p < 1.0]
        if bad:
            raise ValueError(f"ImageTransformerDenoiserModelV2.enable_dropout: dropout rates must lie in [0, 1) ({', '.join(bad)})")
        if generator is not None and not isinstance(generator, torch.Generator):
            raise TypeError(f"enable_dropout: generator must be a torch.Generator or None (got {type(generator)})")
        self._dropout_on, self._dropout_gen = True, generator
        return self

    def set_wgrad_arithmetic(self, arithmetic=None):
        if arithmetic not in (None, "bf16"):
            raise ValueError(f"ImageTransformerDenoiserModelV2.set_wgrad_arithmetic: {arithmetic!r} (None or 'bf16')")
        self.wgrad_arithmetic = arithmetic
        return self

    def _dropout_applies(self):
        return self.training and any(p > 0 for _, p in self._dropout_rates())

    def _refuse_when_dropping(self, what):
        if self._dropout_on and self._dropout_applies():
            raise NotImplementedError(f"ImageTransformerDenoiserModelV2.{what}: dropout is enabled and the model is in training mode, and this "
                                      f"pass has no dropout; call model.eval() first (dropout applies to loss_forward / Denoiser.loss only)")

    def loss_forward(self, x, sigma, aug_cond=None, class_cond=None, mapping_cond=None):
        key = None
        if self._dropout_applies():
            if not self._dropout_on:
                drop = [f"{name} = {p}" for name, p in self._dropout_rates() if p > 0]
                raise NotImplementedError(f"ImageTransformerDenoiserModelV2: dropout in training mode needs model.enable_dropout() "
                                          f"({', '.join(drop)}; masks from this project's counter-based generator); or call model.eval() "
                                          f"for the dropout-free objective")
            if isinstance(x, torch.Tensor) and x.is_cuda:
                key = torch.randint(-2 ** 63, 2 ** 63 - 1, (1,), dtype=torch.int64, device=x.device, generator=self._dropout_gen)
        params = [p for p in self.parameters() if p.requires_grad] if torch.is_grad_enabled() else []
        if params:
            return _ParamGrad.apply(x, self, sigma, aug_cond, class_cond, mapping_cond, key, *params)
        from . import vjp
        return vjp.primal(self, x, sigma, aug_cond, class_cond, mapping_cond, dropout=key)

    def forward(self, x, sigma, aug_cond=None, class_cond=None, mapping_cond=None):
        self._refuse_when_dropping("forward")
        if _wants_input_grad(x):
            return _InputGrad.apply(x, self, sigma, aug_cond, class_cond, mapping_cond, None)
        return self._run(x, sigma, aug_cond, class_cond, mapping_cond, None)

    def forward_preconditioned(self, x, sigma, sigma_data, aug_cond=None, class_cond=None, mapping_cond=None):
        self._refuse_when_dropping("forward_preconditioned")
        if _wants_input_grad(x):
            return _InputGrad.apply(x, self, sigma, aug_cond, class_cond, mapping_cond, sigma_data)
        return self._run(x, sigma, aug_cond, class_cond, mapping_cond, sigma_data)

    def forward_jvp(self, x, sigma, x_dot, aug_cond=None, class_cond=None, mapping_cond=None, sigma_data=None):
        self._refuse_when_dropping("forward_jvp")
        from . import jvp
        return jvp.forward_jvp(self, x, sigma, x_dot, aug_cond=aug_cond, class_cond=class_cond, mapping_cond=mapping_cond, sigma_data=sigma_data)

    def _check_input(self, x, class_cond, mapping_cond, subject, other=None):
# ... 116 lines not shown
```

### k-diffusion_amd/ops.py

```python
import ctypes as C
import os

import math

import torch

from . import _native as nat
from . import weights


def _stream():
    return C.c_void_p(torch.cuda.current_stream().cuda_stream)


def _chk(t, name, dtype=torch.float32):
    if not isinstance(t, torch.Tensor):
        raise TypeError(f"{name}: expected a tensor, got {type(t)}")
    if not t.is_cuda:
        raise RuntimeError(f"{name}: the HIP path needs a tensor on a ROCm device (got {t.device}); there is no CPU fallback")
    if t.dtype != dtype:
        raise TypeError(f"{name}: expected {dtype}, got {t.dtype}")
    if not t.is_contiguous():
        raise ValueError(f"{name}: tensor must be contiguous")
    return t


def _p(t):
    return None if t is None else C.c_void_p(t.data_ptr())


_packed = weights.WeakCache()


def pack_weight(W, N, K, geglu, cache=True, bf16=False):
    geglu = int(geglu)

    def build():
        _chk(W, "W")
        lib = nat.lib()
        if bf16 == "mx8":
            size = lib.kd_packed_weight_bytes_mx8(N, K, geglu)
            if size <= 0:
                raise ValueError(f"kd_pack_weight_mx8: N={N} K={K} is not taken (K must be a multiple of 128)")
            img = torch.empty(size, device=W.device, dtype=torch.uint8)
            nat.check(lib.kd_pack_weight_mx8(_p(W), _p(img), N, K, geglu, _stream()), "kd_pack_weight_mx8")
        elif bf16:
            img = torch.empty(lib.kd_packed_weight_bytes_bf16(N, K, geglu), device=W.device, dtype=torch.uint8)
            nat.check(lib.kd_pack_weight_bf16(_p(W), _p(img), N, K, geglu, _stream()), "kd_pack_weight_bf16")
        else:
            img = torch.empty(lib.kd_packed_weight_bytes(N, K, geglu), device=W.device, dtype=torch.uint8)
            nat.check(lib.kd_pack_weight_bf16x3(_p(W), _p(img), N, K, geglu, _stream()), "kd_pack_weight_bf16x3")
        return img
    return _packed.get(W, (bf16 if bf16 == "mx8" else bool(bf16), geglu), (N, K), build, cache=cache)


def gemm(A, W, out, *, M, N, K, a_mode=nat.A_PLAIN, epi=nat.EPI_STORE, norm_scale=None, scale_stride=0,
         rows_per_sample=0, residual=None, grid=(0, 0), patch=(0, 0, 0), eps=1e-6, out_add=0.0,
         sigma=None, sigma_data=1.0, fac=None, scale_ptr=None, precision=None, qk=None, qkv_packed=False, per_row=False,
         a_planes=None, c_planes=None, launch=True, mx8=False, pack=pack_weight):
    d = nat.KdGemm()
    d.per_row = 1 if per_row else 0
    d.precision = nat.kernel_precision() if precision is None else precision
    bf = d.precision == nat.PREC_BF16
    act = torch.bfloat16 if bf else torch.float32
    a_dt = torch.float32 if a_mode == nat.A_PATCH_NCHW else act
    c_dt = torch.float32 if epi == nat.EPI_UNPATCH_NCHW else act
    if mx8:
        if not bf:
            raise TypeError("mx8: bf16 activations only (precision=PREC_BF16)")
        d.Wp = pack(W, N, K, epi == nat.EPI_GEGLU, bf16="mx8").data_ptr()
    elif bf:
        d.Wp = pack(W, N, K, epi == nat.EPI_GEGLU, bf16=True).data_ptr()
    elif d.precision == nat.PREC_SPLIT3:
        d.Wp = pack(W, N, K, epi == nat.EPI_GEGLU).data_ptr()
    d.M, d.N, d.K = M, N, K
    d.a_mode, d.epi = a_mode, epi
    d.norm = 1 if (norm_scale is not None or scale_ptr is not None) else 0
    d.rows_per_sample, d.scale_stride = rows_per_sample, scale_stride
    d.gh, d.gw = grid
    d.ph, d.pw, d.chan = patch
    d.eps, d.out_add, d.sigma_data = eps, out_add, sigma_data
    d.W = _chk(W, "W").data_ptr()
    if a_planes is not None and mx8:
        d.a_split, d.A, d.A_lo = 1, _chk(a_planes[0], "A e4m3", torch.uint8).data_ptr(), _chk(a_planes[1], "A scales", torch.uint8).data_ptr()
    elif a_planes is not None:
        d.a_split, d.A, d.A_lo = 1, _chk(a_planes[0], "A hi", torch.bfloat16).data_ptr(), _chk(a_planes[1], "A lo", torch.bfloat16).data_ptr()
    elif A is not None or launch:
        d.A = _chk(A, "A", a_dt).data_ptr()
    if c_planes is not None and mx8:
        d.c_split, d.C, d.C_lo = 1, _chk(c_planes[0], "C e4m3", torch.uint8).data_ptr(), _chk(c_planes[1], "C scales", torch.uint8).data_ptr()
        out = c_planes
    elif c_planes is not None:
        d.c_split, d.C, d.C_lo = 1, _chk(c_planes[0], "C hi", torch.bfloat16).data_ptr(), _chk(c_planes[1], "C lo", torch.bfloat16).data_ptr()
        out = c_planes
    elif out is not None or launch:
        d.C = _chk(out, "C", c_dt).data_ptr()
    d.R = None if residual is None else _chk(residual, "R", c_dt).data_ptr()
    d.scale = scale_ptr if scale_ptr is not None else (None if norm_scale is None else _chk(norm_scale, "scale").data_ptr())
    d.sigma = None if sigma is None else _chk(sigma, "sigma").data_ptr()
    d.fac = None if fac is None else _chk(fac, "fac").data_ptr()
    if qk is not None and bf:
        d.qk_scale, d.rope_pos, d.rope_freq = (_chk(t, n).data_ptr() for t, n in zip(qk[:3], ("qk_scale", "rope_pos", "rope_freq")))
        d.n_heads = qk[3]
    elif qk is not None:
        d.qk_scale, d.rope_cos, d.rope_sin = (_chk(t, n).data_ptr() for t, n in zip(qk[:3], ("qk_scale", "cos", "sin")))
        d.n_heads = qk[3]
        if len(qk) >= 6:
            d.rope_pos, d.rope_freq = _chk(qk[4], "rope_pos").data_ptr(), _chk(qk[5], "rope_freq").data_ptr()
        d.qkv_packed = 1 if qkv_packed else 0
    if not launch:
        return d
    name = _gemm_entry(d.precision, mx8)
    nat.check(getattr(nat.lib(), name)(C.byref(d), _stream()), name)
    return out


def _gemm_entry(precision, mx8=False):
    return "kd_gemm_mx8" if mx8 else ("kd_gemm_bf16" if precision == nat.PREC_BF16 else "kd_gemm_f32")


def _prec_of(x):
    if x.dtype == torch.bfloat16:
        return nat.PREC_BF16
    p = nat.kernel_precision()
    return nat.PREC_SPLIT3 if p == nat.PREC_BF16 else p


def linear(x, weight, residual=None, out=None, out_add=0.0):
    K = x.shape[-1]
    M = x.numel() // K
    Nn = weight.shape[0]
    out = torch.empty(*x.shape[:-1], Nn, device=x.device, dtype=x.dtype) if out is None else out
    return gemm(x, weight, out, M=M, N=Nn, K=K, epi=nat.EPI_RESIDUAL if residual is not None else nat.EPI_STORE,
                residual=residual, out_add=out_add, precision=_prec_of(x))


def linear_geglu(x, weight, out=None):
    K = x.shape[-1]
    M = x.numel() // K
    d_ff = weight.shape[0] // 2
    out = torch.empty(*x.shape[:-1], d_ff, device=x.device, dtype=x.dtype) if out is None else out
    return gemm(x, weight, out, M=M, N=d_ff, K=K, epi=nat.EPI_GEGLU, precision=_prec_of(x))


def norm_split(x, scale=None, *, rows_per_sample=0, eps=1e-6):
    K = x.shape[-1]
    M = x.numel() // K
    hi, lo = torch.empty(x.shape, device=x.device, dtype=torch.bfloat16), torch.empty(x.shape, device=x.device, dtype=torch.bfloat16)
    stride = 0 if scale is None or scale.dim() == 1 else K
    nat.check(nat.lib().kd_norm_split_f32(_p(_chk(x, "x")), None if scale is None else _p(_chk(scale, "scale")), stride, rows_per_sample or M,
                                          _p(hi), _p(lo), M, K, eps, _stream()), "kd_norm_split_f32")
    return hi, lo


def rms_norm(x, scale, eps=1e-6, out=None):
    d = x.shape[-1]
    out = torch.empty_like(x) if out is None else out
    nat.check(nat.lib().kd_rmsnorm_f32(_p(_chk(x, "x")), _p(_chk(scale, "scale")), _p(_chk(out, "y")), x.numel() // d, d, eps, _stream()),
            "kd_rmsnorm_f32")
    return out


def norm_linear(x, scale, weight, *, rows_per_sample, epi=nat.EPI_STORE, out=None, eps=1e-6, qk=None, qkv_packed=False, mx8=False, c_fp8=False):
    K = x.shape[-1]
    M = x.numel() // K
    Nn = weight.shape[0] // (2 if epi == nat.EPI_GEGLU else 1)
    if c_fp8:
        planes = (torch.empty(*x.shape[:-1], Nn, device=x.device, dtype=torch.uint8), torch.empty(*x.shape[:-1], Nn // 32, device=x.device, dtype=torch.uint8))
        return gemm(x, weight, None, M=M, N=Nn, K=K, epi=epi, norm_scale=scale, scale_stride=K if scale.dim() == 2 else 0,
                    rows_per_sample=rows_per_sample, eps=eps, precision=_prec_of(x), mx8=True, c_planes=planes)
    out = torch.empty(*x.shape[:-1], Nn, device=x.device, dtype=x.dtype) if out is None else out
    return gemm(x, weight, out, M=M, N=Nn, K=K, epi=epi, norm_scale=scale, scale_stride=K if scale.dim() == 2 else 0,
                rows_per_sample=rows_per_sample, eps=eps, qk=qk, qkv_packed=qkv_packed, precision=_prec_of(x), mx8=mx8)


def linear_mx8(a8, a_scales, weight, residual=None, out=None):
    K = a8.shape[-1]
    M = a8.numel() // K
    Nn = weight.shape[0]
    out = torch.empty(*a8.shape[:-1], Nn, device=a8.device, dtype=torch.bfloat16) if out is None else out
    return gemm(None, weight, out, M=M, N=Nn, K=K, epi=nat.EPI_RESIDUAL if residual is not None else nat.EPI_STORE, residual=residual,
                precision=nat.PREC_BF16, mx8=True, a_planes=(a8, a_scales))


def attn_block(x, scale, weight, *, rows_per_sample, qk, out=None, eps=1e-6):
    K = x.shape[-1]
    M = x.numel() // K
    out = torch.empty_like(x) if out is None else out
    d = gemm(x, weight, out, M=M, N=3 * K, K=K, epi=nat.EPI_QKV, norm_scale=scale, scale_stride=K, rows_per_sample=rows_per_sample, eps=eps,
             qk=qk, precision=nat.PREC_BF16, launch=False)
    nat.check(nat.lib().kd_attn_block_bf16(C.byref(d), _stream()), "kd_attn_block_bf16")
    return out


def proj_block(x, scale, weight, *, rows_per_sample, epi=nat.EPI_GEGLU, qk=None, out=None, eps=1e-6):
    K = x.shape[-1]
    M = x.numel() // K
    N = weight.shape[0] // (2 if epi == nat.EPI_GEGLU else 1)
    out = torch.empty(*x.shape[:-1], N, device=x.device, dtype=x.dtype) if out is None else out
    d = gemm(x, weight, out, M=M, N=N, K=K, epi=epi, norm_scale=scale, scale_stride=K, rows_per_sample=rows_per_sample, eps=eps, qk=qk,
             precision=nat.PREC_BF16, launch=False)
    nat.check(nat.lib().kd_proj_block_bf16(C.byref(d), _stream()), "kd_proj_block_bf16")
    return out


def token_merge(x, weight, out=None):
    B, H2, W2, Cc = x.shape
    h, w = H2 // 2, W2 // 2
    Nn = weight.shape[0]
    out = torch.empty(B, h, w, Nn, device=x.device, dtype=x.dtype) if out is None else out
    return gemm(x, weight, out, M=B * h * w, N=Nn, K=4 * Cc, a_mode=nat.A_MERGE2x2, grid=(h, w), precision=_prec_of(x))


def token_split_lerp(x, weight, skip, fac, out=None):
    B, h, w, K = x.shape
    Nn = weight.shape[0]
    out = torch.empty_like(skip) if out is None else out
    return gemm(x, weight, out, M=B * h * w, N=Nn, K=K, epi=nat.EPI_SPLIT_LERP, residual=skip, fac=fac, grid=(h, w), precision=_prec_of(x))


def patch_in(image, weight, patch, sigma=None, sigma_data=1.0, out=None, precision=None):
    B, Cc, H, W = image.shape
    ph, pw = patch
    h, w = H // ph, W // pw
    Nn = weight.shape[0]
    precision = nat.kernel_precision() if precision is None else precision
    act = torch.bfloat16 if precision == nat.PREC_BF16 else torch.float32
    out = torch.empty(B, h, w, Nn, device=image.device, dtype=act) if out is None else out
    return gemm(image, weight, out, M=B * h * w, N=Nn, K=Cc * ph * pw, a_mode=nat.A_PATCH_NCHW, grid=(h, w),
                patch=(ph, pw, Cc), sigma=sigma, sigma_data=sigma_data, precision=precision)


def patch_out(x, norm_scale, weight, patch, channels, x_in=None, sigma=None, sigma_data=1.0, out=None, eps=1e-6):
    B, h, w, K = x.shape
    ph, pw = patch
    out = torch.empty(B, channels, h * ph, w * pw, device=x.device, dtype=torch.float32) if out is None else out
    return gemm(x, weight, out, M=B * h * w, N=channels * ph * pw, K=K, epi=nat.EPI_UNPATCH_NCHW, norm_scale=norm_scale,
                scale_stride=0, rows_per_sample=h * w, grid=(h, w), patch=(ph, pw, channels), residual=x_in, sigma=sigma,
                sigma_data=sigma_data, eps=eps, precision=_prec_of(x))


def ffn_supported(M, K, d_ff, bf16=True):
    fn = nat.lib().kd_ffn_bf16_supported if bf16 else nat.lib().kd_ffn_f32_supported
    return bool(fn(int(M), int(K), int(d_ff)))


def ffn(x, norm_scale, w_up, w_down, out=None, scale_stride=None, rows_per_sample=None, eps=1e-6, attn=None, w_out=None, launch=True,
        pack=pack_weight):
    K = x.shape[-1]
    M = x.numel() // K
    d_ff = w_down.shape[1]
    if x.dtype not in (torch.bfloat16, torch.float32):
        raise TypeError("ffn: bf16 activations (KDIFF_GEMM=bf16) or fp32 activations (the fp32-parity split3 mode)")
    bf = x.dtype == torch.bfloat16
    out = torch.empty_like(x) if out is None else out
    d = nat.KdFfn()
    d.x, d.out = _p(_chk(x, "x", x.dtype)), _p(_chk(out, "out", x.dtype))
    if norm_scale is not None or launch:
        d.scale = _p(_chk(norm_scale, "norm_scale"))
    d.scale_stride = norm_scale.shape[-1] if scale_stride is None else scale_stride
    d.rows_per_sample = (M // max(norm_scale.numel() // norm_scale.shape[-1], 1)) if rows_per_sample is None else rows_per_sample
    d.eps = eps
    fused_out = attn is not None
    if fused_out and w_out is None:
        raise ValueError("ffn: attn and w_out go together")
    up_img, down_img = pack(w_up, d_ff, K, 3 if fused_out else 1, bf16=bf), pack(w_down, K, d_ff, 2, bf16=bf)
    d.Wp_up, d.Wp_down = _p(up_img), _p(down_img)
    d.M, d.K, d.d_ff = M, K, d_ff
    if fused_out:
        out_img = pack(w_out, K, K, 0, bf16=bf)
        d.attn, d.Wp_out = _p(_chk(attn, "attn", x.dtype)), _p(out_img)
    if not launch:
        return d
    name = "kd_ffn_bf16" if bf else "kd_ffn_f32"
    nat.check(getattr(nat.lib(), name)(C.byref(d), _stream()), name)
    return out


def attn_ffn_supported(batch, H, W, nh, kernel_size, K, d_ff):
    return bool(nat.lib().kd_attn_ffn_f32_supported(int(batch), int(H), int(W), int(nh), int(kernel_size), int(K), int(d_ff)))


def attn_ffn(qkv, nh, kernel_size, x, norm_scale, w_up, w_down, w_out, out=None, eps=1e-6):
    B, H, W = qkv.shape[0], qkv.shape[1], qkv.shape[2]
    out = torch.empty_like(x) if out is None else out
    d = ffn(x, norm_scale, w_up, w_down, out=out, rows_per_sample=H * W, eps=eps, attn=x, w_out=w_out, launch=False)
    d.attn = None
    nat.check(nat.lib().kd_attn_ffn_f32(_p(_chk(qkv, "qkv")), C.byref(d), B, H, W, nh, kernel_size, _stream()), "kd_attn_ffn_f32")
    return out


def fourier_sigma(sigma, weight, out=None):
    half = weight.shape[0]
    out = torch.empty(sigma.shape[0], 2 * half, device=sigma.device, dtype=torch.float32) if out is None else out
    nat.check(nat.lib().kd_fourier_sigma_f32(_p(_chk(sigma, "sigma")), _p(_chk(weight, "weight")), _p(_chk(out, "ff")), sigma.shape[0], half,
                                         _stream()), "kd_fourier_sigma_f32")
    return out


def fourier_features(x, weight, out=None):
    half, in_dim = weight.shape
    B = x.numel() // in_dim
    out = torch.empty(*x.shape[:-1], 2 * half, device=x.device, dtype=torch.float32) if out is None else out
    nat.check(nat.lib().kd_fourier_f32(_p(_chk(x, "x")), _p(_chk(weight, "weight")), _p(_chk(out, "ff")), B, in_dim, half, _stream()), "kd_fourier_f32")
    return out


def cond_sum(a, b, emb=None, ids=None, c=None, out=None):
    B, d = a.shape
    out = torch.empty_like(a) if out is None else out
    if emb is not None:
        _chk(ids, "ids", torch.int64)
    nat.check(nat.lib().kd_cond_sum_f32(_p(_chk(out, "out")), _p(_chk(a, "a")), _p(_chk(b, "b")), 1 if b.dim() == 2 else 0,
                                    _p(None if emb is None else _chk(emb, "emb")), _p(ids), _p(None if c is None else _chk(c, "c")),
                                    B, d, _stream()), "kd_cond_sum_f32")
    return out


def _qkv_dims(qkv, nh):
    if qkv.shape[-1] != 3 * nh * 64:
        raise ValueError(f"qkv last dim {qkv.shape[-1]} != 3*{nh}*64 (head dim is fixed at 64)")


def qk_prep_(qkv, scale_h, cos_t, sin_t, nh, eps=1e-6):
    _qkv_dims(qkv, nh)
    B = qkv.shape[0]
    T = qkv.numel() // (B * 3 * nh * 64)
    nat.check(nat.lib().kd_qk_prep_f32(_p(_chk(qkv, "qkv")), _p(_chk(scale_h, "scale")), _p(_chk(cos_t, "cos")), _p(_chk(sin_t, "sin")),
                                   B, T, nh, eps, _stream()), "kd_qk_prep_f32")
    return qkv


def _prep_args(prep):
    if prep is None:
        return 0, None, None, None, 1e-6
    if isinstance(prep, str):
        if prep != "packed":
            raise ValueError("prep: None (q, k prepared), (scale_h, cos, sin[, eps]) or 'packed' (prepared and stored split by the qkv GEMM)")
        return 2, None, None, None, 1e-6
    scale_h, cos_t, sin_t = prep[:3]
    eps = prep[3] if len(prep) > 3 else 1e-6
    return 1, _p(_chk(scale_h, "scale")), _p(_chk(cos_t, "cos")), _p(_chk(sin_t, "sin")), eps


def _bf16_prep(prep):
    if prep is not None:
        raise ValueError("the bf16 attention cores take q, k already prepared by the qkv GEMM's epilogue (prep=None)")


def attn_global(qkv, nh, prep=None, out=None):
    _qkv_dims(qkv, nh)
    B = qkv.shape[0]
    T = qkv.numel() // (B * 3 * nh * 64)
    out = torch.empty(*qkv.shape[:-1], nh * 64, device=qkv.device, dtype=qkv.dtype) if out is None else out
    if qkv.dtype == torch.bfloat16:
        _bf16_prep(prep)
        nat.check(nat.lib().kd_attn_global_bf16(_p(_chk(qkv, "qkv", torch.bfloat16)), _p(_chk(out, "out", torch.bfloat16)), B, T, nh, _stream()),
                  "kd_attn_global_bf16")
        return out
    f, s, c, sn, eps = _prep_args(prep)
    nat.check(nat.lib().kd_attn_global_f32(_p(_chk(qkv, "qkv")), _p(_chk(out, "out")), B, T, nh, f, s, c, sn, eps, _prec_of(qkv), _stream()), "kd_attn_global_f32")
    return out


def attn_window(qkv, nh, window_size, shift, prep=None, out=None):
    _qkv_dims(qkv, nh)
    B, H, W, _ = qkv.shape
    out = torch.empty(B, H, W, nh * 64, device=qkv.device, dtype=qkv.dtype) if out is None else out
    if qkv.dtype == torch.bfloat16:
        _bf16_prep(prep)
        nat.check(nat.lib().kd_attn_window_bf16(_p(_chk(qkv, "qkv", torch.bfloat16)), _p(_chk(out, "out", torch.bfloat16)), B, H, W, nh, window_size, shift,
                                                _stream()), "kd_attn_window_bf16")
        return out
    f, s, c, sn, eps = _prep_args(prep)
    nat.check(nat.lib().kd_attn_window_f32(_p(_chk(qkv, "qkv")), _p(_chk(out, "out")), B, H, W, nh, window_size, shift, f, s, c, sn, eps, _prec_of(qkv),
                                           _stream()), "kd_attn_window_f32")
    return out


def attn_na2d(qkv, nh, kernel_size, prep=None, out=None):
    _qkv_dims(qkv, nh)
    B, H, W, _ = qkv.shape
    out = torch.empty(B, H, W, nh * 64, device=qkv.device, dtype=qkv.dtype) if out is None else out
    if qkv.dtype == torch.bfloat16:
        _bf16_prep(prep)
        nat.check(nat.lib().kd_attn_na2d_bf16(_p(_chk(qkv, "qkv", torch.bfloat16)), _p(_chk(out, "out", torch.bfloat16)), B, H, W, nh, kernel_size, _stream()),
                  "kd_attn_na2d_bf16")
        return out
    f, s, c, sn, eps = _prep_args(prep)
    nat.check(nat.lib().kd_attn_na2d_f32(_p(_chk(qkv, "qkv")), _p(_chk(out, "out")), B, H, W, nh, kernel_size, f, s, c, sn, eps, _prec_of(qkv), _stream()),
            "kd_attn_na2d_f32")
    return out


def sampler_step(op, x, den, in2=None, out=None, aux=None, c0=0.0, c1=0.0, c2=1.0, c3=0.0):
    out = torch.empty_like(den) if out is None else out
    for name, t in (("x", x), ("den", den), ("in2", in2), ("out", out), ("aux", aux)):
        if t is not None:
            _chk(t, name)
            if t.numel() != den.numel():
                raise ValueError(f"sampler_step: {name} has {t.numel()} elements, expected {den.numel()}")
    nat.check(nat.lib().kd_sampler_step_f32(op, _p(x), _p(den), _p(in2), _p(out), _p(aux), float(c0), float(c1), float(c2), float(c3),
                                        den.numel(), _stream()), "kd_sampler_step_f32")
    return out


def precond_in(x, sigma, sigma_data, out=None):
    out = torch.empty_like(x) if out is None else out
    B = x.shape[0]
    nat.check(nat.lib().kd_precond_in_f32(_p(_chk(x, "x")), _p(_chk(sigma, "sigma")), _p(_chk(out, "y")), float(sigma_data), B, x.numel() // B, _stream()),
            "kd_precond_in_f32")
    return out


def precond_out(f, x, sigma, sigma_data, out=None):
    out = torch.empty_like(x) if out is None else out
    B = x.shape[0]
    nat.check(nat.lib().kd_precond_out_f32(_p(_chk(f, "f")), _p(_chk(x, "x")), _p(_chk(sigma, "sigma")), _p(_chk(out, "y")), float(sigma_data), B,
                                       x.numel() // B, _stream()), "kd_precond_out_f32")
    return out


def rows_affine(f, a, x=None, c=None, out=None):
    out = torch.empty_like(f) if out is None else out
    B = f.shape[0]
    nat.check(nat.lib().kd_rows_affine_f32(_p(_chk(f, "f")), _p(None if x is None else _chk(x, "x")), _p(_chk(a, "a")),
                                       _p(None if c is None else _chk(c, "c")), _p(_chk(out, "y")), B, f.numel() // B, _stream()),
            "kd_rows_affine_f32")
    return out


def sigma_to_t(sigma, log_sigmas, quantize):
    out = torch.empty(sigma.shape, device=sigma.device, dtype=torch.float32)
    nat.check(nat.lib().kd_sigma_to_t_f32(_p(_chk(sigma.contiguous(), "sigma")), _p(_chk(log_sigmas, "log_sigmas")), _p(out), sigma.numel(),
                                      log_sigmas.numel(), int(bool(quantize)), _stream()), "kd_sigma_to_t_f32")
    return out


def t_to_sigma(t, log_sigmas):
    out = torch.empty(t.shape, device=t.device, dtype=torch.float32)
    nat.check(nat.lib().kd_t_to_sigma_f32(_p(_chk(t.contiguous(), "t")), _p(_chk(log_sigmas, "log_sigmas")), _p(out), t.numel(), log_sigmas.numel(),
                                      _stream()), "kd_t_to_sigma_f32")
    return out


def dpm_eps(x, denoised, sigma, out=None):
    out = torch.empty_like(x) if out is None else out
    nat.check(nat.lib().kd_dpm_eps_f32(_p(_chk(out, "out")), _p(_chk(x, "x")), _p(_chk(denoised, "denoised")), float(sigma), x.numel(), _stream()),
              "kd_dpm_eps_f32")
    return out


def dpm_combine(x, eps, a, eps_r=None, b=0.0, out=None):
    out = torch.empty_like(x) if out is None else out
    nat.check(nat.lib().kd_dpm_combine_f32(_p(_chk(out, "out")), _p(_chk(x, "x")), _p(_chk(eps, "eps")), None if eps_r is None else _p(_chk(eps_r, "eps_r")),
                                           float(a), float(b), x.numel(), _stream()), "kd_dpm_combine_f32")
    return out


def dpm_error(x_low, x_high, x_prev, atol, rtol):
    part = torch.empty(nat.lib().kd_dpm_error_partials(), device=x_low.device, dtype=torch.float32)
    nat.check(nat.lib().kd_dpm_error_f32(_p(_chk(x_low, "x_low")), _p(_chk(x_high, "x_high")), _p(_chk(x_prev, "x_prev")), float(atol), float(rtol),
                                         x_low.numel(), _p(part), _stream()), "kd_dpm_error_f32")
    return math.sqrt(float(part.double().sum().item()) / x_low.numel())


def brownian(out, seeds, T0, T1, t0, t1, mult, depth=36):
    B = out.shape[0]
    _chk(seeds, "seeds", torch.int64)
    nat.check(nat.lib().kd_brownian_f32(_p(_chk(out, "out")), _p(seeds), B, out.numel() // B, float(T0), float(T1), float(t0), float(t1),
                                    float(mult), depth, _stream()), "kd_brownian_f32")
    return out


def brownian_cached(out, w0, have0, w1, have1, seeds, T0, T1, t0, t1, mult, depth=36):
    B = out.shape[0]
    _chk(seeds, "seeds", torch.int64)
    for w in (w0, w1):
        if w is not None and _chk(w, "w").numel() != out.numel():
            raise ValueError("end-point buffers must match out")
    nat.check(nat.lib().kd_brownian_cached_f32(_p(_chk(out, "out")), _p(w0) if w0 is not None else None, _p(w1) if w1 is not None else None,
                                           int(bool(have0)), int(bool(have1)), _p(seeds), B, out.numel() // B, float(T0), float(T1),
                                           float(t0), float(t1), float(mult), depth, _stream()), "kd_brownian_cached_f32")
    return out


def randn_indexed(out, seeds, draw=0, scale=1.0):
    B = out.shape[0]
    _chk(seeds, "seeds", torch.int64)
    if seeds.numel() != B:
        raise ValueError(f"one seed per batch item: {seeds.numel()} seeds for batch {B}")
    nat.check(nat.lib().kd_randn_f32(_p(_chk(out, "out")), _p(seeds), B, out.numel() // B, int(draw), float(scale), _stream()), "kd_randn_f32")
    return out


def to_uint8(x, out=None):
    out = torch.empty(x.shape, device=x.device, dtype=torch.uint8) if out is None else out
    if x.numel() == 0:
        _chk(x, "x"), _chk(out, "y", torch.uint8)
        return out
    nat.check(nat.lib().kd_to_uint8(_p(_chk(x, "x")), _p(_chk(out, "y", torch.uint8)), x.numel(), _stream()), "kd_to_uint8")
    return out



def rms_norm_jvp(x, x_dot, scale, rows_per_sample=None, eps=1e-6):
    d = x.shape[-1]
    rows = x.numel() // d
    y, yd = torch.empty_like(x), torch.empty_like(x)
    stride = 0 if scale.dim() == 1 else scale.shape[-1]
    rps = rows if stride == 0 else (rows_per_sample or rows // scale.shape[0])
    nat.check(nat.lib().kd_rmsnorm_jvp_f32(_p(_chk(x, "x")), _p(_chk(x_dot, "x_dot")), _p(_chk(scale, "scale")), stride, rps, _p(y), _p(yd), rows, d,
                                           float(eps), _stream()), "kd_rmsnorm_jvp_f32")
    return y, yd


def geglu_jvp(h, h_dot):
    d_ff = h.shape[-1] // 2
    rows = h.numel() // h.shape[-1]
    y = torch.empty(*h.shape[:-1], d_ff, device=h.device, dtype=torch.float32)
    yd = torch.empty_like(y)
    nat.check(nat.lib().kd_geglu_jvp_f32(_p(_chk(h, "h")), _p(_chk(h_dot, "h_dot")), _p(y), _p(yd), rows, d_ff, _stream()), "kd_geglu_jvp_f32")
    return y, yd


def qk_prep_jvp_(qkv, qkv_dot, scale_h, cos_t, sin_t, nh, eps=1e-6):
    _qkv_dims(qkv, nh)
    B = qkv.shape[0]
    T = qkv.numel() // (B * 3 * nh * 64)
    nat.check(nat.lib().kd_qk_prep_jvp_f32(_p(_chk(qkv, "qkv")), _p(_chk(qkv_dot, "qkv_dot")), _p(_chk(scale_h, "scale")), _p(_chk(cos_t, "cos")),
                                           _p(_chk(sin_t, "sin")), B, T, nh, float(eps), _stream()), "kd_qk_prep_jvp_f32")
    return qkv, qkv_dot

# ... 550 lines not shown
```

Before: 244.9.

## Fuse patch-in projection into first layer's norm+QKV projection kernel

Adds an entry kernel that gathers 4x4 NCHW patches, applies the Karras c_in scale, and runs the patch-in GEMM on split-bf16 MFMA. It writes x to global memory and then feeds the rows into the astat norm+QKV GEMM as a prologue, so the first layer's separate qkv_proj launch is removed and the plan patches the launch list. The gemm_x3 astat kernel is moved into a shared header and templated on a row-source policy. This saves one launch and one round trip of x through memory at level 0, at the cost of more code and a narrowly gated shape-specific path.

```diff
diff --git a/k-diffusion_amd/csrc/entry_qkv_x3.hip b/k-diffusion_amd/csrc/entry_qkv_x3.hip
--- /dev/null
+++ b/k-diffusion_amd/csrc/entry_qkv_x3.hip
@@ -0,0 +1,152 @@
+#include "gemm_x3_core.h"
+
+namespace kd {
+namespace x3 {
+
+extern unsigned long long* g_clk;
+
+struct PatchArgs {
+  const float* img; const char* Wp; float* X;
+  const float* sigma; float sigma_data;
+  int gh, gw;
+};
+
+__device__ __forceinline__ float karras_c_in(float sigma, float sd) { return 1.0f / sqrtf(__builtin_fmaf(sigma, sigma, sd * sd)); }
+
+constexpr int PG_ROW = 208;
+
+struct RowsFromPatch {
+  template <int K, int KH, int CPR, int PIECES, int R>
+  static __device__ __forceinline__ void stage(char* smem, char* stage, const float*, int M, int m0, int wid, int lane, const PatchArgs& a) {
+    static_assert(K == 128 && KH == 128 && R == 0, "level 0: one staging round of whole rows");
+    const int l31 = lane & 31, lh = lane >> 5;
+    {
+      const char* wsrc = a.Wp + wid * 4096 + lane * 16;
+#pragma unroll
+      for (int s = 0; s < 2; ++s)
+#pragma unroll
+        for (int j = 0; j < 4; ++j)
+          __builtin_amdgcn_global_load_lds((const __attribute__((address_space(1))) void*)(wsrc + s * STG + j * 1024),
+                                           (__attribute__((address_space(3))) void*)(smem + s * STG + wid * 4096 + j * 1024), 16, 0, 0);
+    }
+    char* garea = smem + 2 * STG + wid * 8192 + l31 * PG_ROW;
+    {
+      const int row = min(m0 + wid * 32 + l31, M - 1);
+      const int per = a.gh * a.gw, b = row / per, rr = row - b * per, ty = rr / a.gw, tx = rr - ty * a.gw;
+      const float cin = a.sigma ? karras_c_in(a.sigma[b], a.sigma_data) : 1.0f;
+      const int Wimg = 4 * a.gw;
+      const size_t plane = (size_t)16 * per;
+      const float* tp = a.img + (size_t)b * 3 * plane + (size_t)(4 * ty) * Wimg + 4 * tx;
+      f32x4 v[6];
+#pragma unroll
+      for (int i = 0; i < 6; ++i) {
+        const int seg = 2 * i + lh, c = seg >> 2, nh = seg & 3;
+        v[i] = *reinterpret_cast<const f32x4*>(tp + c * plane + nh * Wimg);
+      }
+#pragma unroll
+      for (int i = 0; i < 6; ++i) {
+        const int seg = 2 * i + lh, c = seg >> 2, nh = seg & 3;
+        const f32x4 s = v[i] * cin;
+#pragma unroll
+        for (int nw = 0; nw < 4; ++nw) *reinterpret_cast<float*>(garea + ((nh * 4 + nw) * 3 + c) * 4) = s[nw];
+      }
+    }
+    bf16x8 a_hi[3], a_lo[3];
+#pragma unroll
+    for (int c = 0; c < 3; ++c) {
+      const f32x4 x0 = *reinterpret_cast<const f32x4*>(garea + (16 * c + 8 * lh) * 4);
+      const f32x4 x1 = *reinterpret_cast<const f32x4*>(garea + (16 * c + 8 * lh) * 4 + 16);
+      u32x4 hi, lo;
+      split8(x0, x1, hi, lo);
+      a_hi[c] = __builtin_bit_cast(bf16x8, hi);
+      a_lo[c] = __builtin_bit_cast(bf16x8, lo);
+    }
+    asm volatile("s_waitcnt vmcnt(0)" ::: "memory");
+    KD_BARRIER();
+    f32x16 acc[4];
+#pragma unroll
+    for (int j = 0; j < 4; ++j)
+#pragma unroll
+      for (int r = 0; r < 16; ++r) acc[j][r] = 0.f;
+#pragma unroll
+    for (int c = 0; c < 3; ++c) {
+      const char* st = smem + (c >> 1) * STG + swz64(l31, 2 * (c & 1) + lh);
+      bf16x8 wh[4], wl[4];
+#pragma unroll
+      for (int j = 0; j < 4; ++j) {
+        wh[j] = *reinterpret_cast<const bf16x8*>(st + j * 32 * 64);
+        wl[j] = *reinterpret_cast<const bf16x8*>(st + IMG + j * 32 * 64);
+      }
+#pragma unroll
+      for (int j = 0; j < 4; ++j) mfma_a(acc[j], wh[j], a_lo[c]);
+#pragma unroll
+      for (int j = 0; j < 4; ++j) mfma_a(acc[j], wl[j], a_hi[c]);
+#pragma unroll
+      for (int j = 0; j < 4; ++j) mfma_a(acc[j], wh[j], a_hi[c]);
+    }
+    asm volatile("s_waitcnt lgkmcnt(0)" ::: "memory");
+    KD_BARRIER();
+    {
+      char* rowp = stage + l31 * 512;
+#pragma unroll
+      for (int j = 0; j < 4; ++j)
+#pragma unroll
+        for (int g = 0; g < 4; ++g)
+          *reinterpret_cast<f32x4*>(rowp + (((8 * j + 2 * g + lh) ^ (l31 & 15)) << 4)) = f32x4{acc[j][4 * g], acc[j][4 * g + 1], acc[j][4 * g + 2], acc[j][4 * g + 3]};
+    }
+#pragma unroll
+    for (int i = 0; i < 16; ++i) {
+      const int ci = i * 64 + lane, rr = ci >> 5, qs = ci & 31, row = m0 + wid * 32 + rr;
+      const f32x4 o = *reinterpret_cast<const f32x4*>(stage + rr * 512 + ((qs ^ (rr & 15)) << 4));
+      if (row < M) st16(a.X + (size_t)row * 128 + qs * 4, o);
+    }
+    asm volatile("; kd_phase_b" ::: "memory");
+  }
+};
+
+constexpr int EQ_LDS = 4 * STG + 4 * 1024 + 4 * 2048 + 1024;
+static_assert(EQ_LDS <= 80 * 1024, "two workgroups per CU");
+static_assert(32 * PG_ROW <= 8192 && PG_ROW % 16 == 0 && PG_ROW >= 48 * 4, "a wave's gather area: half a ring slot");
+
+}
+
+static bool entry_qkv_takes(const KdGemm& pr, const KdGemm& q, const char** why) {
+  if (pr.precision != KD_PREC_SPLIT3 || q.precision != KD_PREC_SPLIT3 || !pr.Wp || !q.Wp) return *why = "both descriptors KD_PREC_SPLIT3 with packed images", false;
+  if (pr.a_mode != KD_A_PATCH_NCHW || pr.epi != KD_EPI_STORE || pr.norm || pr.a_split || pr.c_split || pr.per_row || pr.out_add != 0.f)
+    return *why = "producer: the plain patch projection (KD_A_PATCH_NCHW, KD_EPI_STORE, no norm, out_add 0)", false;
+  if (pr.K != 48 || pr.N != 128 || pr.ph != 4 || pr.pw != 4 || pr.chan != 3 || pr.gh <= 0 || pr.gw <= 0 || pr.M <= 0 || pr.M % (pr.gh * pr.gw))
+    return *why = "producer: 4 x 4 patches of 3 channels to width 128, M a multiple of gh gw", false;
+  if (q.a_mode != KD_A_PLAIN || q.epi != KD_EPI_QKV || !q.norm || q.a_split || q.c_split || q.per_row || q.K != 128 || q.N != 384 || q.n_heads != 2)
+    return *why = "projection: norm -> qkv of width 128, 2 heads of 64", false;
+  if (q.M != pr.M || q.rows_per_sample != pr.gh * pr.gw || (q.scale_stride & 3) || !q.qk_scale || !q.rope_pos || !q.rope_freq)
+    return *why = "projection: M and rows_per_sample of the producer's token grid, qk_scale, rope_pos, rope_freq", false;
+  return true;
+}
+
+int entry_qkv_launch(const KdGemm& pr, hipStream_t stream) {
+  const KdGemm& q = *reinterpret_cast<const KdGemm*>(pr.C_lo);
+  const char* why = "";
+  if (!entry_qkv_takes(pr, q, &why)) return fail(KD_EINVAL, "kd_gemm_f32(patch-in + qkv): %s", why);
+  if (!pr.A || !pr.C || !q.C || !q.scale || q.A != pr.C) return fail(KD_EINVAL, "kd_gemm_f32(patch-in + qkv): null image / x / qkv / scale, or the projection does not read the producer's x");
+  if ((reinterpret_cast<size_t>(pr.A) | reinterpret_cast<size_t>(pr.C) | reinterpret_cast<size_t>(q.C)) & 15) return fail(KD_EINVAL, "kd_gemm_f32(patch-in + qkv): 16-byte aligned buffers");
+  x3::XArgs a{};
+  a.A = q.A; a.Wp = reinterpret_cast<const char*>(q.Wp); a.C = q.C;
+  a.scale = q.scale; a.scale_stride = q.scale_stride; a.rows_per_sample = q.rows_per_sample; a.eps = q.eps;
+  a.M = q.M; a.N = q.N; a.n_tiles = q.N / 128; a.n_splits = 1;
+  a.n_heads = q.n_heads; a.qk_scale = q.qk_scale; a.pos = q.rope_pos; a.freq = q.rope_freq; a.qkv_packed = q.qkv_packed;
+  a.out_add = q.out_add;
+  a.warm = code_warm();
+  a.clk = x3::g_clk;
+  x3::PatchArgs pa{pr.A, reinterpret_cast<const char*>(pr.Wp), pr.C, pr.sigma, pr.sigma_data, pr.gh, pr.gw};
+  const double M = q.M;
+  const double flops = 2.0 * M * pr.N * pr.K + 2.0 * M * q.N * q.K;
+  const double bytes = 4.0 * (M * pr.K + (double)pr.N * pr.K + M * pr.N) + 4.0 * (M * q.K + (double)q.N * q.K + M * q.N) - 8.0 * M * 128;
+  const ProfName nm("entry_qkv_x3", "entry_qkv_x3<patch> M=%d N=%d K=%d+%d", q.M, q.N, pr.K, q.K);
+  LaunchScope prof(nm, flops, bytes, stream);
+  launch<x3::gemm_x3_astat_kernel<8, KD_EPI_QKV, x3::RowsFromPatch, x3::PatchArgs>>(dim3((unsigned)((q.M + 127) / 128)), dim3(256), x3::EQ_LDS, stream, a, pa);
+  return check_launch("kd_gemm_f32(patch-in + qkv)");
+}
+
+}
+
+KD_TEXT_PAD(entry_qkv_x3)
diff --git a/k-diffusion_amd/csrc/gemm.hip b/k-diffusion_amd/csrc/gemm.hip
--- a/k-diffusion_amd/csrc/gemm.hip
+++ b/k-diffusion_amd/csrc/gemm.hip
@@ -506,6 +506,7 @@
 namespace kd { int gemm_skinny_try(const GemmP& d, hipStream_t s, int* rc); }
 namespace kd { int gemm_x3r_try(const GemmP& d, hipStream_t s, int* rc); }
 namespace kd { int gemm_x3s_try(const GemmP& d, hipStream_t s, int* rc); }
+namespace kd { int entry_qkv_launch(const KdGemm& producer, hipStream_t s); }
 
 using namespace kd;
 
@@ -531,6 +532,7 @@
   if ((d.a_split || d.c_split) && d.precision != KD_PREC_SPLIT3) return fail(KD_EINVAL, "kd_gemm_f32: a_split / c_split are KD_PREC_SPLIT3 operand formats");
   if (d.a_split && (d.norm || d.a_mode != KD_A_PLAIN || !d.A_lo)) return fail(KD_EINVAL, "kd_gemm_f32: a_split needs A_lo, a_mode KD_A_PLAIN and no norm prologue (kd_norm_split_f32 does the norm)");
   if (d.c_split && !d.C_lo) return fail(KD_EINVAL, "kd_gemm_f32: c_split needs C_lo");
+  if (d.a_mode == KD_A_PATCH_NCHW && !d.c_split && d.C_lo) return entry_qkv_launch(d, s);
   GemmP e;
   static_cast<KdGemm&>(e) = d;
   e.debug = opt(KD_OPT_gemm_debug);
diff --git a/k-diffusion_amd/csrc/gemm_x3.hip b/k-diffusion_amd/csrc/gemm_x3.hip
--- a/k-diffusion_amd/csrc/gemm_x3.hip
+++ b/k-diffusion_amd/csrc/gemm_x3.hip
@@ -1,400 +1,7 @@
-#include "x3_common.h"
+#include "gemm_x3_core.h"
 
 namespace kd {
 namespace x3 {
-
-struct XArgs {
-  const float* A; const char* Wp; float* C;
-  b16::u16* Cl; int c_split;
-  const float* scale; int scale_stride, rows_per_sample; float eps;
-  int M, N, n_tiles, n_splits;
-  int n_heads; const float* qk_scale; const float* pos; const float* freq; int qkv_packed;
-  float out_add;
-  const float* sigma; float sigma_data; int gh, gw, chan;
-  const float* R;
-  int warm;
-  unsigned long long* clk;
-};
-
-template <int NC , int EPI>
-__global__ __launch_bounds__(256, NC <= 8 ? 2 : 1) void gemm_x3_astat_kernel(const XArgs p) {
-  constexpr int K = NC * 16, NK = NC / 2;
-  constexpr int NSTG = NC <= 8 ? 4 : 8, PDIST = NSTG - 1, PB = 4;
-  constexpr bool GEGLU = EPI == KD_EPI_GEGLU;
-  constexpr int NCOL = GEGLU ? 64 : 128;
-  constexpr int NST = GEGLU ? 8 : 16;
-  constexpr int WAREA = (NSTG / 4) * STG;
-  constexpr int KH = WAREA / 128 >= K ? K : WAREA / 128;
-  constexpr bool AG = NC >= 32;
-  constexpr int NR = K / KH, CPR = KH / 4;
-  constexpr int PIECES = 32 * CPR / 64;
-  constexpr int SCL = K * 4 < 1024 ? 1024 : K * 4;
-  static_assert(NK % NSTG == 0 || NSTG % NK == 0, "ring slot of a stage must be a compile-time constant");
-  static_assert(CPR >= 16 && NC % NR == 0, "source-side chunk swizzle spans 16 chunk positions");
-  extern __shared__ __attribute__((aligned(16))) char smem[];
-  const int tid = threadIdx.x, lane = tid & 63, l31 = lane & 31, lh = lane >> 5;
-  const int wid = __builtin_amdgcn_readfirstlane(tid >> 6);
-  const auto warm = code_warm_begin<(NC <= 8 ? 14 : 24) * 1024>((int)blockIdx.x < p.warm && tid < 64);
-  const PanelSplit ps = panel_split(p.n_splits, p.n_tiles);
-  const int nt_begin = ps.t_begin, n_tiles = ps.t_end - ps.t_begin, total = n_tiles * NK;
-  const int m0 = ps.panel * 128;
-  const bool probe = p.clk && blockIdx.x == 0 && tid == 0;
-  if (probe) { p.clk[0] = __builtin_amdgcn_s_memtime(); p.clk[1] = __builtin_amdgcn_s_memrealtime(); }
-  const WgStamp wgs = wg_stamp_begin(p.clk);
-
-  f32x16 acc[4];
-  if constexpr (EPI == KD_EPI_RESIDUAL) {
-    const int rrow = min(m0 + wid * 32 + l31, p.M - 1);
-    const float* rp = p.R + (size_t)rrow * p.N + nt_begin * NCOL + 4 * lh;
-#pragma unroll
-    for (int j = 0; j < 4; ++j)
-#pragma unroll
-      for (int g = 0; g < 4; ++g) {
-        const f32x4 v = *reinterpret_cast<const f32x4*>(rp + 32 * j + 8 * g);
-#pragma unroll
-        for (int e = 0; e < 4; ++e) acc[j][4 * g + e] = v[e];
-      }
-  }
-
-  const char* wp = p.Wp + (size_t)nt_begin * NK * STG + wid * (PB * 1024) + lane * 16;
-  auto issue_piece = [&](int s_, int j) {
-    const int s = min(s_, total - 1);
-    const char* src = wp + (size_t)s * STG;
-    char* dst = smem + (s_ % NSTG) * STG + wid * (PB * 1024);
-    __builtin_amdgcn_global_load_lds((const __attribute__((address_space(1))) void*)(src + j * 1024),
-                                     (__attribute__((address_space(3))) void*)(dst + j * 1024), 16, 0, 0);
-  };
-  auto issue = [&](int s_) {
-#pragma unroll
-    for (int j = 0; j < PB; ++j) issue_piece(s_, j);
-  };
-
-  const int row = m0 + wid * 32 + l31;
-  const bool ok = row < p.M;
-  const int rowc = ok ? row : p.M - 1;
-  bf16x8 a_hi[AG ? 1 : NC], a_lo[AG ? 1 : NC];
-  float rs;
-  {
-    char* stage = smem + wid * WAREA;
-    char* scl = smem + NSTG * STG + wid * SCL;
-    const int r_first = min(m0 + wid * 32, p.M - 1), r_last = min(m0 + wid * 32 + 31, p.M - 1);
-    constexpr bool nrm = EPI != KD_EPI_RESIDUAL;
-    const bool uni = nrm && (p.scale_stride == 0 || r_first / p.rows_per_sample == r_last / p.rows_per_sample);
-    if (uni) {
-      const char* ssrc = reinterpret_cast<const char*>(p.scale + (size_t)(r_first / p.rows_per_sample) * p.scale_stride);
-#pragma unroll
-      for (int i = 0; i < SCL / 1024; ++i)
-        __builtin_amdgcn_global_load_lds((const __attribute__((address_space(1))) void*)(ssrc + (i * 1024 + lane * 16) % (K * 4)),
-                                         (__attribute__((address_space(3))) void*)(scl + i * 1024), 16, 0, 0);
-    }
-    const float* sp = p.scale + (size_t)(rowc / p.rows_per_sample) * p.scale_stride + 8 * lh;
-    const float* spl = reinterpret_cast<const float*>(scl) + 8 * lh;
-    float ssq = 0.f;
-    static_for<NR>([&](auto r_) {
-      constexpr int r = decltype(r_)::value;
-#pragma unroll
-      for (int i = 0; i < PIECES; ++i) {
-        const int ci = i * 64 + lane, rr = ci / CPR, qs = ci % CPR;
-        const int grow = min(m0 + wid * 32 + rr, p.M - 1);
-        const char* src = reinterpret_cast<const char*>(p.A + (size_t)grow * K + r * KH) + ((qs ^ (rr & 15)) << 4);
-        __builtin_amdgcn_global_load_lds((const __attribute__((address_space(1))) void*)src,
-                                         (__attribute__((address_space(3))) void*)(stage + i * 1024), 16, 0, 0);
-      }
-      asm volatile("s_waitcnt vmcnt(0)" ::: "memory");
-      const char* rowp = stage + l31 * (KH * 4);
-      static_for<NC / NR / 4>([&](auto c4_) {
-        constexpr int c0 = r * (NC / NR) + 4 * decltype(c4_)::value;
-        f32x4 x0[4], x1[4], s0[4], s1[4];
-#pragma unroll
-        for (int u = 0; u < 4; ++u) {
-          const int q = 4 * (c0 - r * (NC / NR) + u) + 2 * lh;
-          x0[u] = *reinterpret_cast<const f32x4*>(rowp + ((q ^ (l31 & 15)) << 4));
-          x1[u] = *reinterpret_cast<const f32x4*>(rowp + (((q + 1) ^ (l31 & 15)) << 4));
-          if constexpr (nrm) {
-            if (uni) {
-              s0[u] = *reinterpret_cast<const f32x4*>(spl + 16 * (c0 + u));
-              s1[u] = *reinterpret_cast<const f32x4*>(spl + 16 * (c0 + u) + 4);
-            } else {
-              s0[u] = *reinterpret_cast<const f32x4*>(sp + 16 * (c0 + u));
-              s1[u] = *reinterpret_cast<const f32x4*>(sp + 16 * (c0 + u) + 4);
-            }
-          }
-        }
-        __builtin_amdgcn_sched_barrier(0);
-        static_for<4>([&](auto u_) {
-          constexpr int u = decltype(u_)::value;
-#pragma unroll
-          for (int e = 0; e < 4; ++e) ssq = fmaf(x0[u][e], x0[u][e], fmaf(x1[u][e], x1[u][e], ssq));
-          u32x4 hi, lo;
-          if constexpr (nrm) split8(x0[u] * s0[u], x1[u] * s1[u], hi, lo);
-          else split8(x0[u], x1[u], hi, lo);
-          if constexpr (AG) {
-            areg_write4<8 * (c0 + u)>(hi);
-            areg_write4<8 * (c0 + u) + 4>(lo);
-          } else {
-            asm volatile("" : "+v"(hi), "+v"(lo));
-            a_hi[c0 + u] = __builtin_bit_cast(bf16x8, hi);
-            a_lo[c0 + u] = __builtin_bit_cast(bf16x8, lo);
-          }
-        });
-        __builtin_amdgcn_sched_barrier(0);
-      });
-      if constexpr (NR > 1) asm volatile("s_waitcnt lgkmcnt(0)" ::: "memory");
-    });
-    ssq += __shfl_xor(ssq, 32, 64);
-    rs = nrm ? rsqrtf(ssq / (float)K + p.eps) : 1.f;
-  }
-  float py = 0.f, px = 0.f;
-  if (EPI == KD_EPI_QKV) {
-    qk_tab_fill(reinterpret_cast<float*>(smem + NSTG * STG + 4 * SCL + 4 * 2048), tid, p);
-    token_pos(p.pos, rowc % p.rows_per_sample, py, px);
-  }
-  code_warm_end(warm);
-  asm volatile("s_waitcnt vmcnt(0) lgkmcnt(0)" ::: "memory");
-  KD_BARRIER();
-  const bool full_panel = m0 + 128 <= p.M;
-#pragma unroll
-  for (int s = 0; s < PDIST; ++s) issue(s);
-  if (probe) p.clk[4] = __builtin_amdgcn_s_memtime();
-
-  const int o0 = swz64(l31, lh), o1 = swz64(l31, 2 + lh);
-  char* strip = smem + NSTG * STG + 4 * SCL + wid * 2048;
-  const char* qkc = smem + NSTG * STG + 4 * SCL + 4 * 2048;
-  float* st_row[2];
-  bool st_ok[2];
-#pragma unroll
-  for (int it = 0; it < 2; ++it) {
-    const int r = m0 + wid * 32 + 16 * it + (lane >> 2);
-    st_ok[it] = r < p.M;
-    st_row[it] = p.C + (size_t)min(r, p.M - 1) * p.N + 4 * (lane & 3);
-  }
-  if constexpr (EPI != KD_EPI_RESIDUAL) {
-#pragma unroll
-    for (int j = 0; j < 4; ++j)
-#pragma unroll
-      for (int r = 0; r < 16; ++r) acc[j][r] = 0.f;
-  }
-  if constexpr (AG) asm volatile("s_nop 3" : "+v"(acc[0]), "+v"(acc[1]), "+v"(acc[2]), "+v"(acc[3]));
-
-  bf16x8 wh[2][4], wl[2][4];
-  int ou0[2] = {0, 0}, ou1[2] = {0, 0};
-  if constexpr (EPI == KD_EPI_UNPATCH_NCHW) {
-#pragma unroll
-    for (int j = 0; j < 2; ++j) {
-      const int np = 32 * j + l31, q = np >> 2, py = q / p.chan, cch = q - py * p.chan;
-      const int n = np < 16 * p.chan ? (py * 4 + (np & 3)) * p.chan + cch : np;
-      ou0[j] = swz64(n, lh);
-      ou1[j] = swz64(n, 2 + lh);
-    }
-  }
-  auto read_frags = [&](int slot, int h, bf16x8 (&fh)[4], bf16x8 (&fl)[4]) {
-    if constexpr (EPI == KD_EPI_UNPATCH_NCHW) {
-#pragma unroll
-      for (int j = 0; j < 2; ++j) {
-        const char* st = smem + slot * STG + (h ? ou1[j] : ou0[j]);
-        fh[j] = *reinterpret_cast<const bf16x8*>(st);
-        fl[j] = *reinterpret_cast<const bf16x8*>(st + IMG);
-      }
-    } else {
-      const char* st = smem + slot * STG + (h ? o1 : o0);
-#pragma unroll
-      for (int j = 0; j < 4; ++j) {
-        fh[j] = *reinterpret_cast<const bf16x8*>(st + j * 32 * 64);
-        fl[j] = *reinterpret_cast<const bf16x8*>(st + IMG + j * 32 * 64);
-      }
-    }
-  };
-  wait_vm(PB * (PDIST - 1));
-  KD_BARRIER();
-  read_frags(0, 0, wh[0], wl[0]);
-
-  for (int nt = 0; nt < n_tiles; ++nt) {
-    static_for<NK>([&](auto ks_) {
-      constexpr int ks = decltype(ks_)::value;
-      const int s = nt * NK + ks;
-      auto mm = [&](auto b_, int j, bool w_lo, auto a_lo_) {
-        constexpr int b = decltype(b_)::value, al = decltype(a_lo_)::value, c = 2 * ks + b;
-        if (EPI == KD_EPI_UNPATCH_NCHW && j >= 2) return;
-        const bf16x8& w = w_lo ? wl[b][j] : wh[b][j];
-        if constexpr (AG) mfma_ag<8 * c + 4 * al>(acc[j], w);
-        else mfma_a(acc[j], w, al ? a_lo[c] : a_hi[c]);
-      };
-      constexpr std::integral_constant<int, 0> I0{};
-      constexpr std::integral_constant<int, 1> I1{};
-      if constexpr (AG) {
-        mm(I0, 0, true, I0);
-        __builtin_amdgcn_sched_barrier(0);
-        read_frags(ks % NSTG, 1, wh[1], wl[1]);
-        __builtin_amdgcn_sched_barrier(0);
-#pragma unroll
-        for (int j = 1; j < 4; ++j) mm(I0, j, true, I0);
-      } else {
-        read_frags(ks % NSTG, 1, wh[1], wl[1]);
-#pragma unroll
-        for (int j = 0; j < 4; ++j) mm(I0, j, true, I0);
-      }
-#pragma unroll
-      for (int j = 0; j < 4; ++j) mm(I0, j, false, I1);
-#pragma unroll
-      for (int j = 0; j < 4; ++j) mm(I0, j, false, I0);
-      if constexpr (!AG) {
-        __builtin_amdgcn_sched_group_barrier(0x008, 1, 0);
-        __builtin_amdgcn_sched_group_barrier(0x100, 8, 0);
-        __builtin_amdgcn_sched_group_barrier(0x008, 11, 0);
-      }
-      __builtin_amdgcn_sched_barrier(0);
-      {
-        int allow = PB * (PDIST - 2);
-        if (full_panel && nt > 0 && ks + 2 <= PDIST) allow += NST;
-        wait_vm(allow);
-        KD_BARRIER();
-      }
-      mm(I1, 0, true, I0);
-      if constexpr (AG) __builtin_amdgcn_sched_barrier(0);
-      read_frags((ks + 1) % NSTG, 0, wh[0], wl[0]);
-      if constexpr (!AG) {
-        __builtin_amdgcn_sched_group_barrier(0x008, 1, 0);
-        __builtin_amdgcn_sched_group_barrier(0x100, 8, 0);
-      }
-      __builtin_amdgcn_sched_barrier(0);
-      mm(I1, 1, true, I0);
-      mm(I1, 2, true, I0);
-      issue_piece(s + PDIST, 0);
-      __builtin_amdgcn_sched_barrier(0);
-      mm(I1, 3, true, I0);
-      mm(I1, 0, false, I1);
-      mm(I1, 1, false, I1);
-      issue_piece(s + PDIST, 1);
-      __builtin_amdgcn_sched_barrier(0);
-      mm(I1, 2, false, I1);
-      mm(I1, 3, false, I1);
-      mm(I1, 0, false, I0);
-      issue_piece(s + PDIST, 2);
-      __builtin_amdgcn_sched_barrier(0);
-      mm(I1, 1, false, I0);
-      mm(I1, 2, false, I0);
-      issue_piece(s + PDIST, 3);
-      mm(I1, 3, false, I0);
-      __builtin_amdgcn_sched_barrier(0);
-    });
-    if constexpr (AG) asm volatile("s_nop 15\n\ts_nop 3" : "+v"(acc[0]), "+v"(acc[1]), "+v"(acc[2]), "+v"(acc[3]));
-    if (probe && nt == 0) p.clk[5] = __builtin_amdgcn_s_memtime();
-
-    const int n0 = (nt_begin + nt) * NCOL;
-    auto store_block = [&](const f32x4 (&v)[4], int col) {
-#pragma unroll
-      for (int hb = 0; hb < 2; ++hb) {
-#pragma unroll
-        for (int gg = 0; gg < 2; ++gg)
-          *reinterpret_cast<f32x4*>(strip + l31 * 64 + (((2 * gg + lh) ^ ((l31 >> 2) & 1)) << 4)) = v[2 * hb + gg];
-#pragma unroll
-        for (int it = 0; it < 2; ++it) {
-          const int r16 = 16 * it + (lane >> 2), c = lane & 3;
-          const f32x4 o = *reinterpret_cast<const f32x4*>(strip + r16 * 64 + ((c ^ ((r16 >> 2) & 1)) << 4));
-          if (st_ok[it]) st16(st_row[it] + col + 16 * hb, o);
-        }
-      }
-    };
-    if (GEGLU) {
-      const float rsh = 0.5f * rs;
-#pragma unroll
-      for (int jj = 0; jj < 2; ++jj) {
-        f32x4 blk[4];
-#pragma unroll
-        for (int g = 0; g < 4; ++g) {
-          const f32x2 a = geglu_pair(f32x2{acc[2 * jj][4 * g], acc[2 * jj][4 * g + 1]} * rsh, f32x2{acc[2 * jj + 1][4 * g], acc[2 * jj + 1][4 * g + 1]} * rs);
-          const f32x2 b = geglu_pair(f32x2{acc[2 * jj][4 * g + 2], acc[2 * jj][4 * g + 3]} * rsh, f32x2{acc[2 * jj + 1][4 * g + 2], acc[2 * jj + 1][4 * g + 3]} * rs);
-          blk[g] = f32x4{a.x, a.y, b.x, b.y};
-        }
-        if (p.c_split) {
-          float v[16], hi[16], lo[16];
-#pragma unroll
-          for (int g = 0; g < 4; ++g)
-#pragma unroll
-            for (int q = 0; q < 4; ++q) v[4 * g + q] = blk[g][q];
-#pragma unroll
-          for (int r = 0; r < 16; r += 2) {
-            const unsigned h = pack_bf16(v[r], v[r + 1]);
-            hi[r] = b16::bf_lo(h);
-            hi[r + 1] = b16::bf_hi(h);
-            lo[r] = v[r] - hi[r];
-            lo[r + 1] = v[r + 1] - hi[r + 1];
-          }
-          const size_t off = (size_t)rowc * p.N + n0 + 32 * jj;
-          b16::store_block_bf16(reinterpret_cast<b16::u16*>(p.C) + off, hi, lh, ok);
-          b16::store_block_bf16(p.Cl + off, lo, lh, ok);
-        } else {
-          store_block(blk, n0 + 32 * jj);
-        }
-      }
-    } else if (EPI == KD_EPI_QKV) {
-#pragma unroll
-      for (int vv = 0; vv < 2; ++vv) {
-        const int vec = (n0 >> 6) + vv;
-        const int which = vec >= 2 * p.n_heads ? 2 : (vec >= p.n_heads ? 1 : 0), head = vec - which * p.n_heads;
-        f32x16& a0 = acc[2 * vv];
-        f32x16& a1 = acc[2 * vv + 1];
-        if (which < 2) {
-          qk_prep_head(qkc, head, lh, a0, a1, rs, p.eps, py, px);
-        } else {
-#pragma unroll
-          for (int r = 0; r < 16; ++r) { a0[r] *= rs; a1[r] *= rs; }
-        }
-#pragma unroll
-        for (int jj = 0; jj < 2; ++jj) {
-          f32x4 blk[4];
-          const f32x16& a = jj ? a1 : a0;
-          if (p.qkv_packed) {
-#pragma unroll
-            for (int g = 0; g < 4; ++g) blk[g] = pack_split4(f32x4{a[4 * g], a[4 * g + 1], a[4 * g + 2], a[4 * g + 3]});
-          } else {
-#pragma unroll
-            for (int g = 0; g < 4; ++g) blk[g] = f32x4{a[4 * g], a[4 * g + 1], a[4 * g + 2], a[4 * g + 3]};
-          }
-          store_block(blk, n0 + 64 * vv + 32 * jj);
-        }
-      }
-    } else if (EPI == KD_EPI_UNPATCH_NCHW) {
-      const int per = p.gh * p.gw, bb = rowc / per, rr = rowc - bb * per, ty = rr / p.gw, tx = rr - ty * p.gw;
-      float c_out = 1.f, c_skip = 0.f;
-      if (p.sigma) {
-        const float sg = p.sigma[bb], sd = p.sigma_data, var = sg * sg + sd * sd;
-        c_skip = sd * sd / var;
-        c_out = sg * sd / sqrtf(var);
-      }
-      const int Himg = 4 * p.gh, Wimg = 4 * p.gw;
-#pragma unroll
-      for (int j = 0; j < 2; ++j)
-#pragma unroll
-        for (int g = 0; g < 4; ++g) {
-          const int q = 8 * j + 2 * g + lh, py = q / p.chan, cch = q - py * p.chan;
-          if (q < 4 * p.chan && ok) {
-            const size_t o = (((size_t)bb * p.chan + cch) * Himg + 4 * ty + py) * Wimg + 4 * tx;
-            f32x4 v = f32x4{acc[j][4 * g], acc[j][4 * g + 1], acc[j][4 * g + 2], acc[j][4 * g + 3]} * (rs * c_out);
-            if (p.sigma) v = v + *reinterpret_cast<const f32x4*>(p.R + o) * c_skip;
-            st16(p.C + o, v);
-          }
-        }
-    } else {
-#pragma unroll
-      for (int j = 0; j < 4; ++j) {
-        f32x4 blk[4];
-#pragma unroll
-        for (int g = 0; g < 4; ++g) blk[g] = f32x4{acc[j][4 * g], acc[j][4 * g + 1], acc[j][4 * g + 2], acc[j][4 * g + 3]} * rs + p.out_add;
-        store_block(blk, n0 + 32 * j);
-      }
-    }
-    if (probe && nt == 0) p.clk[6] = __builtin_amdgcn_s_memtime();
-#pragma unroll
-    for (int j = 0; j < 4; ++j)
-#pragma unroll
-      for (int r = 0; r < 16; ++r) acc[j][r] = 0.f;
-    if constexpr (AG) asm volatile("s_nop 3" : "+v"(acc[0]), "+v"(acc[1]), "+v"(acc[2]), "+v"(acc[3]));
-  }
-  asm volatile("s_waitcnt vmcnt(0)" ::: "memory");
-  if (probe) { p.clk[2] = __builtin_amdgcn_s_memtime(); p.clk[3] = __builtin_amdgcn_s_memrealtime(); p.clk[7] = (unsigned long long)total; }
-  wg_stamp_end(wgs);
-}
 
 template <int EPI>
 __global__ __launch_bounds__(256, 2) void gemm_x3h_kernel(const XArgs p) {
diff --git a/k-diffusion_amd/csrc/gemm_x3_core.h b/k-diffusion_amd/csrc/gemm_x3_core.h
--- /dev/null
+++ b/k-diffusion_amd/csrc/gemm_x3_core.h
@@ -0,0 +1,408 @@
+#pragma once
+#include "x3_common.h"
+
+namespace kd {
+namespace x3 {
+
+struct XArgs {
+  const float* A; const char* Wp; float* C;
+  b16::u16* Cl; int c_split;
+  const float* scale; int scale_stride, rows_per_sample; float eps;
+  int M, N, n_tiles, n_splits;
+  int n_heads; const float* qk_scale; const float* pos; const float* freq; int qkv_packed;
+  float out_add;
+  const float* sigma; float sigma_data; int gh, gw, chan;
+  const float* R;
+  int warm;
+  unsigned long long* clk;
+};
+
+struct RowsFromHBM {
+  template <int K, int KH, int CPR, int PIECES, int R>
+  static __device__ __forceinline__ void stage(char*, char* stage, const float* A, int M, int m0, int wid, int lane) {
+#pragma unroll
+    for (int i = 0; i < PIECES; ++i) {
+      const int ci = i * 64 + lane, rr = ci / CPR, qs = ci % CPR;
+      const int grow = min(m0 + wid * 32 + rr, M - 1);
+      const char* src = reinterpret_cast<const char*>(A + (size_t)grow * K + R * KH) + ((qs ^ (rr & 15)) << 4);
+      __builtin_amdgcn_global_load_lds((const __attribute__((address_space(1))) void*)src,
+                                       (__attribute__((address_space(3))) void*)(stage + i * 1024), 16, 0, 0);
+    }
+    asm volatile("s_waitcnt vmcnt(0)" ::: "memory");
+  }
+};
+
+template <int NC , int EPI, class Rows = RowsFromHBM, class... RowArgs>
+__global__ __launch_bounds__(256, NC <= 8 ? 2 : 1) void gemm_x3_astat_kernel(const XArgs p, const RowArgs... ra) {
+  extern __shared__ __attribute__((aligned(16))) char smem[];
+  constexpr int K = NC * 16, NK = NC / 2;
+  constexpr int NSTG = NC <= 8 ? 4 : 8, PDIST = NSTG - 1, PB = 4;
+  constexpr bool GEGLU = EPI == KD_EPI_GEGLU;
+  constexpr int NCOL = GEGLU ? 64 : 128;
+  constexpr int NST = GEGLU ? 8 : 16;
+  constexpr int WAREA = (NSTG / 4) * STG;
+  constexpr int KH = WAREA / 128 >= K ? K : WAREA / 128;
+  constexpr bool AG = NC >= 32;
+  constexpr int NR = K / KH, CPR = KH / 4;
+  constexpr int PIECES = 32 * CPR / 64;
+  constexpr int SCL = K * 4 < 1024 ? 1024 : K * 4;
+  static_assert(NK % NSTG == 0 || NSTG % NK == 0, "ring slot of a stage must be a compile-time constant");
+  static_assert(CPR >= 16 && NC % NR == 0, "source-side chunk swizzle spans 16 chunk positions");
+  const int tid = threadIdx.x, lane = tid & 63, l31 = lane & 31, lh = lane >> 5;
+  const int wid = __builtin_amdgcn_readfirstlane(tid >> 6);
+  const auto warm = code_warm_begin<(NC <= 8 ? 14 : 24) * 1024>((int)blockIdx.x < p.warm && tid < 64);
+  const PanelSplit ps = panel_split(p.n_splits, p.n_tiles);
+  const int nt_begin = ps.t_begin, n_tiles = ps.t_end - ps.t_begin, total = n_tiles * NK;
+  const int m0 = ps.panel * 128;
+  const bool probe = p.clk && blockIdx.x == 0 && tid == 0;
+  if (probe) { p.clk[0] = __builtin_amdgcn_s_memtime(); p.clk[1] = __builtin_amdgcn_s_memrealtime(); }
+  const WgStamp wgs = wg_stamp_begin(p.clk);
+
+  f32x16 acc[4];
+  if constexpr (EPI == KD_EPI_RESIDUAL) {
+    const int rrow = min(m0 + wid * 32 + l31, p.M - 1);
+    const float* rp = p.R + (size_t)rrow * p.N + nt_begin * NCOL + 4 * lh;
+#pragma unroll
+    for (int j = 0; j < 4; ++j)
+#pragma unroll
+      for (int g = 0; g < 4; ++g) {
+        const f32x4 v = *reinterpret_cast<const f32x4*>(rp + 32 * j + 8 * g);
+#pragma unroll
+        for (int e = 0; e < 4; ++e) acc[j][4 * g + e] = v[e];
+      }
+  }
+
+  const char* wp = p.Wp + (size_t)nt_begin * NK * STG + wid * (PB * 1024) + lane * 16;
+  auto issue_piece = [&](int s_, int j) {
+    const int s = min(s_, total - 1);
+    const char* src = wp + (size_t)s * STG;
+    char* dst = smem + (s_ % NSTG) * STG + wid * (PB * 1024);
+    __builtin_amdgcn_global_load_lds((const __attribute__((address_space(1))) void*)(src + j * 1024),
+                                     (__attribute__((address_space(3))) void*)(dst + j * 1024), 16, 0, 0);
+  };
+  auto issue = [&](int s_) {
+#pragma unroll
+    for (int j = 0; j < PB; ++j) issue_piece(s_, j);
+  };
+
+  const int row = m0 + wid * 32 + l31;
+  const bool ok = row < p.M;
+  const int rowc = ok ? row : p.M - 1;
+  bf16x8 a_hi[AG ? 1 : NC], a_lo[AG ? 1 : NC];
+  float rs;
+  {
+    char* stage = smem + wid * WAREA;
+    char* scl = smem + NSTG * STG + wid * SCL;
+    const int r_first = min(m0 + wid * 32, p.M - 1), r_last = min(m0 + wid * 32 + 31, p.M - 1);
+    constexpr bool nrm = EPI != KD_EPI_RESIDUAL;
+    const bool uni = nrm && (p.scale_stride == 0 || r_first / p.rows_per_sample == r_last / p.rows_per_sample);
+    if (uni) {
+      const char* ssrc = reinterpret_cast<const char*>(p.scale + (size_t)(r_first / p.rows_per_sample) * p.scale_stride);
+#pragma unroll
+      for (int i = 0; i < SCL / 1024; ++i)
+        __builtin_amdgcn_global_load_lds((const __attribute__((address_space(1))) void*)(ssrc + (i * 1024 + lane * 16) % (K * 4)),
+                                         (__attribute__((address_space(3))) void*)(scl + i * 1024), 16, 0, 0);
+    }
+    const float* sp = p.scale + (size_t)(rowc / p.rows_per_sample) * p.scale_stride + 8 * lh;
+    const float* spl = reinterpret_cast<const float*>(scl) + 8 * lh;
+    float ssq = 0.f;
+    static_for<NR>([&](auto r_) {
+      constexpr int r = decltype(r_)::value;
+      Rows::template stage<K, KH, CPR, PIECES, r>(smem, stage, p.A, p.M, m0, wid, lane, ra...);
+      const char* rowp = stage + l31 * (KH * 4);
+      static_for<NC / NR / 4>([&](auto c4_) {
+        constexpr int c0 = r * (NC / NR) + 4 * decltype(c4_)::value;
+        f32x4 x0[4], x1[4], s0[4], s1[4];
+#pragma unroll
+        for (int u = 0; u < 4; ++u) {
+          const int q = 4 * (c0 - r * (NC / NR) + u) + 2 * lh;
+          x0[u] = *reinterpret_cast<const f32x4*>(rowp + ((q ^ (l31 & 15)) << 4));
+          x1[u] = *reinterpret_cast<const f32x4*>(rowp + (((q + 1) ^ (l31 & 15)) << 4));
+          if constexpr (nrm) {
+            if (uni) {
+              s0[u] = *reinterpret_cast<const f32x4*>(spl + 16 * (c0 + u));
+              s1[u] = *reinterpret_cast<const f32x4*>(spl + 16 * (c0 + u) + 4);
+            } else {
+              s0[u] = *reinterpret_cast<const f32x4*>(sp + 16 * (c0 + u));
+              s1[u] = *reinterpret_cast<const f32x4*>(sp + 16 * (c0 + u) + 4);
+            }
+          }
+        }
+        __builtin_amdgcn_sched_barrier(0);
+        static_for<4>([&](auto u_) {
+          constexpr int u = decltype(u_)::value;
+#pragma unroll
+          for (int e = 0; e < 4; ++e) ssq = fmaf(x0[u][e], x0[u][e], fmaf(x1[u][e], x1[u][e], ssq));
+          u32x4 hi, lo;
+          if constexpr (nrm) split8(x0[u] * s0[u], x1[u] * s1[u], hi, lo);
+          else split8(x0[u], x1[u], hi, lo);
+          if constexpr (AG) {
+            areg_write4<8 * (c0 + u)>(hi);
+            areg_write4<8 * (c0 + u) + 4>(lo);
+          } else {
+            asm volatile("" : "+v"(hi), "+v"(lo));
+            a_hi[c0 + u] = __builtin_bit_cast(bf16x8, hi);
+            a_lo[c0 + u] = __builtin_bit_cast(bf16x8, lo);
+          }
+        });
+        __builtin_amdgcn_sched_barrier(0);
+      });
+      if constexpr (NR > 1) asm volatile("s_waitcnt lgkmcnt(0)" ::: "memory");
+    });
+    ssq += __shfl_xor(ssq, 32, 64);
+    rs = nrm ? rsqrtf(ssq / (float)K + p.eps) : 1.f;
+  }
+  float py = 0.f, px = 0.f;
+  if (EPI == KD_EPI_QKV) {
+    qk_tab_fill(reinterpret_cast<float*>(smem + NSTG * STG + 4 * SCL + 4 * 2048), tid, p);
+    token_pos(p.pos, rowc % p.rows_per_sample, py, px);
+  }
+  code_warm_end(warm);
+  asm volatile("s_waitcnt vmcnt(0) lgkmcnt(0)" ::: "memory");
+  KD_BARRIER();
+  const bool full_panel = m0 + 128 <= p.M;
+#pragma unroll
+  for (int s = 0; s < PDIST; ++s) issue(s);
+  if (probe) p.clk[4] = __builtin_amdgcn_s_memtime();
+
+  const int o0 = swz64(l31, lh), o1 = swz64(l31, 2 + lh);
+  char* strip = smem + NSTG * STG + 4 * SCL + wid * 2048;
+  const char* qkc = smem + NSTG * STG + 4 * SCL + 4 * 2048;
+  float* st_row[2];
+  bool st_ok[2];
+#pragma unroll
+  for (int it = 0; it < 2; ++it) {
+    const int r = m0 + wid * 32 + 16 * it + (lane >> 2);
+    st_ok[it] = r < p.M;
+    st_row[it] = p.C + (size_t)min(r, p.M - 1) * p.N + 4 * (lane & 3);
+  }
+  if constexpr (EPI != KD_EPI_RESIDUAL) {
+#pragma unroll
+    for (int j = 0; j < 4; ++j)
+#pragma unroll
+      for (int r = 0; r < 16; ++r) acc[j][r] = 0.f;
+  }
+  if constexpr (AG) asm volatile("s_nop 3" : "+v"(acc[0]), "+v"(acc[1]), "+v"(acc[2]), "+v"(acc[3]));
+
+  bf16x8 wh[2][4], wl[2][4];
+  int ou0[2] = {0, 0}, ou1[2] = {0, 0};
+  if constexpr (EPI == KD_EPI_UNPATCH_NCHW) {
+#pragma unroll
+    for (int j = 0; j < 2; ++j) {
+      const int np = 32 * j + l31, q = np >> 2, py = q / p.chan, cch = q - py * p.chan;
+      const int n = np < 16 * p.chan ? (py * 4 + (np & 3)) * p.chan + cch : np;
+      ou0[j] = swz64(n, lh);
+      ou1[j] = swz64(n, 2 + lh);
+    }
+  }
+  auto read_frags = [&](int slot, int h, bf16x8 (&fh)[4], bf16x8 (&fl)[4]) {
+    if constexpr (EPI == KD_EPI_UNPATCH_NCHW) {
+#pragma unroll
+      for (int j = 0; j < 2; ++j) {
+        const char* st = smem + slot * STG + (h ? ou1[j] : ou0[j]);
+        fh[j] = *reinterpret_cast<const bf16x8*>(st);
+        fl[j] = *reinterpret_cast<const bf16x8*>(st + IMG);
+      }
+    } else {
+      const char* st = smem + slot * STG + (h ? o1 : o0);
+#pragma unroll
+      for (int j = 0; j < 4; ++j) {
+        fh[j] = *reinterpret_cast<const bf16x8*>(st + j * 32 * 64);
+        fl[j] = *reinterpret_cast<const bf16x8*>(st + IMG + j * 32 * 64);
+      }
+    }
+  };
+  wait_vm(PB * (PDIST - 1));
+  KD_BARRIER();
+  read_frags(0, 0, wh[0], wl[0]);
+
+  for (int nt = 0; nt < n_tiles; ++nt) {
+    static_for<NK>([&](auto ks_) {
+      constexpr int ks = decltype(ks_)::value;
+      const int s = nt * NK + ks;
+      auto mm = [&](auto b_, int j, bool w_lo, auto a_lo_) {
+        constexpr int b = decltype(b_)::value, al = decltype(a_lo_)::value, c = 2 * ks + b;
+        if (EPI == KD_EPI_UNPATCH_NCHW && j >= 2) return;
+        const bf16x8& w = w_lo ? wl[b][j] : wh[b][j];
+        if constexpr (AG) mfma_ag<8 * c + 4 * al>(acc[j], w);
+        else mfma_a(acc[j], w, al ? a_lo[c] : a_hi[c]);
+      };
+      constexpr std::integral_constant<int, 0> I0{};
+      constexpr std::integral_constant<int, 1> I1{};
+      if constexpr (AG) {
+        mm(I0, 0, true, I0);
+        __builtin_amdgcn_sched_barrier(0);
+        read_frags(ks % NSTG, 1, wh[1], wl[1]);
+        __builtin_amdgcn_sched_barrier(0);
+#pragma unroll
+        for (int j = 1; j < 4; ++j) mm(I0, j, true, I0);
+      } else {
+        read_frags(ks % NSTG, 1, wh[1], wl[1]);
+#pragma unroll
+        for (int j = 0; j < 4; ++j) mm(I0, j, true, I0);
+      }
+#pragma unroll
+      for (int j = 0; j < 4; ++j) mm(I0, j, false, I1);
+#pragma unroll
+      for (int j = 0; j < 4; ++j) mm(I0, j, false, I0);
+      if constexpr (!AG) {
+        __builtin_amdgcn_sched_group_barrier(0x008, 1, 0);
+        __builtin_amdgcn_sched_group_barrier(0x100, 8, 0);
+        __builtin_amdgcn_sched_group_barrier(0x008, 11, 0);
+      }
+      __builtin_amdgcn_sched_barrier(0);
+      {
+        int allow = PB * (PDIST - 2);
+        if (full_panel && nt > 0 && ks + 2 <= PDIST) allow += NST;
+        wait_vm(allow);
+        KD_BARRIER();
+      }
+      mm(I1, 0, true, I0);
+      if constexpr (AG) __builtin_amdgcn_sched_barrier(0);
+      read_frags((ks + 1) % NSTG, 0, wh[0], wl[0]);
+      if constexpr (!AG) {
+        __builtin_amdgcn_sched_group_barrier(0x008, 1, 0);
+        __builtin_amdgcn_sched_group_barrier(0x100, 8, 0);
+      }
+      __builtin_amdgcn_sched_barrier(0);
+      mm(I1, 1, true, I0);
+      mm(I1, 2, true, I0);
+      issue_piece(s + PDIST, 0);
+      __builtin_amdgcn_sched_barrier(0);
+      mm(I1, 3, true, I0);
+      mm(I1, 0, false, I1);
+      mm(I1, 1, false, I1);
+      issue_piece(s + PDIST, 1);
+      __builtin_amdgcn_sched_barrier(0);
+      mm(I1, 2, false, I1);
+      mm(I1, 3, false, I1);
+      mm(I1, 0, false, I0);
+      issue_piece(s + PDIST, 2);
+      __builtin_amdgcn_sched_barrier(0);
+      mm(I1, 1, false, I0);
+      mm(I1, 2, false, I0);
+      issue_piece(s + PDIST, 3);
+      mm(I1, 3, false, I0);
+      __builtin_amdgcn_sched_barrier(0);
+    });
+    if constexpr (AG) asm volatile("s_nop 15\n\ts_nop 3" : "+v"(acc[0]), "+v"(acc[1]), "+v"(acc[2]), "+v"(acc[3]));
+    if (probe && nt == 0) p.clk[5] = __builtin_amdgcn_s_memtime();
+
+    const int n0 = (nt_begin + nt) * NCOL;
+    auto store_block = [&](const f32x4 (&v)[4], int col) {
+#pragma unroll
+      for (int hb = 0; hb < 2; ++hb) {
+#pragma unroll
+        for (int gg = 0; gg < 2; ++gg)
+          *reinterpret_cast<f32x4*>(strip + l31 * 64 + (((2 * gg + lh) ^ ((l31 >> 2) & 1)) << 4)) = v[2 * hb + gg];
+#pragma unroll
+        for (int it = 0; it < 2; ++it) {
+          const int r16 = 16 * it + (lane >> 2), c = lane & 3;
+          const f32x4 o = *reinterpret_cast<const f32x4*>(strip + r16 * 64 + ((c ^ ((r16 >> 2) & 1)) << 4));
+          if (st_ok[it]) st16(st_row[it] + col + 16 * hb, o);
+        }
+      }
+    };
+    if (GEGLU) {
+      const float rsh = 0.5f * rs;
+#pragma unroll
+      for (int jj = 0; jj < 2; ++jj) {
+        f32x4 blk[4];
+#pragma unroll
+        for (int g = 0; g < 4; ++g) {
+          const f32x2 a = geglu_pair(f32x2{acc[2 * jj][4 * g], acc[2 * jj][4 * g + 1]} * rsh, f32x2{acc[2 * jj + 1][4 * g], acc[2 * jj + 1][4 * g + 1]} * rs);
+          const f32x2 b = geglu_pair(f32x2{acc[2 * jj][4 * g + 2], acc[2 * jj][4 * g + 3]} * rsh, f32x2{acc[2 * jj + 1][4 * g + 2], acc[2 * jj + 1][4 * g + 3]} * rs);
+          blk[g] = f32x4{a.x, a.y, b.x, b.y};
+        }
+        if (p.c_split) {
+          float v[16], hi[16], lo[16];
+#pragma unroll
+          for (int g = 0; g < 4; ++g)
+#pragma unroll
+            for (int q = 0; q < 4; ++q) v[4 * g + q] = blk[g][q];
+#pragma unroll
+          for (int r = 0; r < 16; r += 2) {
+            const unsigned h = pack_bf16(v[r], v[r + 1]);
+            hi[r] = b16::bf_lo(h);
+            hi[r + 1] = b16::bf_hi(h);
+            lo[r] = v[r] - hi[r];
+            lo[r + 1] = v[r + 1] - hi[r + 1];
+          }
+          const size_t off = (size_t)rowc * p.N + n0 + 32 * jj;
+          b16::store_block_bf16(reinterpret_cast<b16::u16*>(p.C) + off, hi, lh, ok);
+          b16::store_block_bf16(p.Cl + off, lo, lh, ok);
+        } else {
+          store_block(blk, n0 + 32 * jj);
+        }
+      }
+    } else if (EPI == KD_EPI_QKV) {
+#pragma unroll
+      for (int vv = 0; vv < 2; ++vv) {
+        const int vec = (n0 >> 6) + vv;
+        const int which = vec >= 2 * p.n_heads ? 2 : (vec >= p.n_heads ? 1 : 0), head = vec - which * p.n_heads;
+        f32x16& a0 = acc[2 * vv];
+        f32x16& a1 = acc[2 * vv + 1];
+        if (which < 2) {
+          qk_prep_head(qkc, head, lh, a0, a1, rs, p.eps, py, px);
+        } else {
+#pragma unroll
+          for (int r = 0; r < 16; ++r) { a0[r] *= rs; a1[r] *= rs; }
+        }
+#pragma unroll
+        for (int jj = 0; jj < 2; ++jj) {
+          f32x4 blk[4];
+          const f32x16& a = jj ? a1 : a0;
+          if (p.qkv_packed) {
+#pragma unroll
+            for (int g = 0; g < 4; ++g) blk[g] = pack_split4(f32x4{a[4 * g], a[4 * g + 1], a[4 * g + 2], a[4 * g + 3]});
+          } else {
+#pragma unroll
+            for (int g = 0; g < 4; ++g) blk[g] = f32x4{a[4 * g], a[4 * g + 1], a[4 * g + 2], a[4 * g + 3]};
+          }
+          store_block(blk, n0 + 64 * vv + 32 * jj);
+        }
+      }
+    } else if (EPI == KD_EPI_UNPATCH_NCHW) {
+      const int per = p.gh * p.gw, bb = rowc / per, rr = rowc - bb * per, ty = rr / p.gw, tx = rr - ty * p.gw;
+      float c_out = 1.f, c_skip = 0.f;
+      if (p.sigma) {
+        const float sg = p.sigma[bb], sd = p.sigma_data, var = sg * sg + sd * sd;
+        c_skip = sd * sd / var;
+        c_out = sg * sd / sqrtf(var);
+      }
+      const int Himg = 4 * p.gh, Wimg = 4 * p.gw;
+#pragma unroll
+      for (int j = 0; j < 2; ++j)
+#pragma unroll
+        for (int g = 0; g < 4; ++g) {
+          const int q = 8 * j + 2 * g + lh, py = q / p.chan, cch = q - py * p.chan;
+          if (q < 4 * p.chan && ok) {
+            const size_t o = (((size_t)bb * p.chan + cch) * Himg + 4 * ty + py) * Wimg + 4 * tx;
+            f32x4 v = f32x4{acc[j][4 * g], acc[j][4 * g + 1], acc[j][4 * g + 2], acc[j][4 * g + 3]} * (rs * c_out);
+            if (p.sigma) v = v + *reinterpret_cast<const f32x4*>(p.R + o) * c_skip;
+            st16(p.C + o, v);
+          }
+        }
+    } else {
+#pragma unroll
+      for (int j = 0; j < 4; ++j) {
+        f32x4 blk[4];
+#pragma unroll
+        for (int g = 0; g < 4; ++g) blk[g] = f32x4{acc[j][4 * g], acc[j][4 * g + 1], acc[j][4 * g + 2], acc[j][4 * g + 3]} * rs + p.out_add;
+        store_block(blk, n0 + 32 * j);
+      }
+    }
+    if (probe && nt == 0) p.clk[6] = __builtin_amdgcn_s_memtime();
+#pragma unroll
+    for (int j = 0; j < 4; ++j)
+#pragma unroll
+      for (int r = 0; r < 16; ++r) acc[j][r] = 0.f;
+    if constexpr (AG) asm volatile("s_nop 3" : "+v"(acc[0]), "+v"(acc[1]), "+v"(acc[2]), "+v"(acc[3]));
+  }
+  asm volatile("s_waitcnt vmcnt(0)" ::: "memory");
+  if (probe) { p.clk[2] = __builtin_amdgcn_s_memtime(); p.clk[3] = __builtin_amdgcn_s_memrealtime(); p.clk[7] = (unsigned long long)total; }
+  wg_stamp_end(wgs);
+}
+
+}
+}
diff --git a/k-diffusion_amd/models/image_transformer_v2.py b/k-diffusion_amd/models/image_transformer_v2.py
--- a/k-diffusion_amd/models/image_transformer_v2.py
+++ b/k-diffusion_amd/models/image_transformer_v2.py
@@ -16,7 +16,8 @@
 D_HEAD = 64
 DERIVED_KEPT = 1024
 MAX_PLANS = 16
-PLAN_SWITCHES = (("KDIFF_ATTN_BLOCK", "1"), ("KDIFF_PROJ_BLOCK", "1"), ("KDIFF_FFN_OUT", "all"), ("KDIFF_RUN_LIST", "1"), ("KDIFF_ATTN_FFN", "1"))
+PLAN_SWITCHES = (("KDIFF_ATTN_BLOCK", "1"), ("KDIFF_PROJ_BLOCK", "1"), ("KDIFF_FFN_OUT", "all"), ("KDIFF_RUN_LIST", "1"), ("KDIFF_ATTN_FFN", "1"),
+                 ("KDIFF_ENTRY_QKV", "1"))
 CLASS_IDS_KEPT = 4
 
 
@@ -385,10 +386,13 @@
         L = self.launches
         self.d_patch_in = self._gemm(L, "patch_in", None, m.patch_in.proj.weight, xs[0], toks[0], levels[0].width, m.in_channels * ph * pw,
                                      a_mode=nat.A_PATCH_NCHW, grid=grids[0], patch=(ph, pw, m.in_channels))
+        entry_on = precision == nat.PREC_SPLIT3 and switches.get("KDIFF_ENTRY_QKV", "1") != "0"
+        self._entry = (len(L) - 1, self.d_patch_in) if entry_on else None
         for st in hourglass(m):
             li = st.level
+            entry, self._entry = self._entry, None
             if st.kind == "layer":
-                self._add_layer(li, st.prefix, st.module, st.index)
+                self._add_layer(li, st.prefix, st.module, st.index, entry=entry if li == 0 else None)
             elif st.kind == "merge":
                 self._gemm(L, f"merges.{li}", xs[li], m.merges[li].proj.weight, xs[li + 1], toks[li + 1], levels[li + 1].width,
                            4 * levels[li].width, a_mode=nat.A_MERGE2x2, grid=grids[li + 1])
@@ -476,7 +480,7 @@
             qk += (pos_t, freq_t)
         return qk
 
-    def _add_layer(self, li, prefix, mod, index):
+    def _add_layer(self, li, prefix, mod, index, entry=None):
         L, lv, (gh, gw), T = self.launches, self.levels[li], self.grids[li], self.toks[li]
         d, d_ff, x, rps = lv.width, lv.d_ff, self.xs[li], gh * gw
         spec = lv.self_attn
@@ -496,7 +500,11 @@
             elif r.qkv == "proj_block":
                 self._gemm(L, prefix + "qkv_proj(block)", x, sa.qkv_proj.weight, self.qkv, T, 3 * d, d, table=norm, entry="kd_proj_block_bf16", **q)
             else:
-                self._gemm(L, prefix + "qkv_proj", x, sa.qkv_proj.weight, self.qkv, T, 3 * d, d, table=norm, mx8=r.qkv == "mx8", **q)
+                dq = self._gemm(L, prefix + "qkv_proj", x, sa.qkv_proj.weight, self.qkv, T, 3 * d, d, table=norm, mx8=r.qkv == "mx8", **q)
+                if entry is not None and r.qkv == "plain" and ops._entry_qkv_supported(entry[1], dq, self.device):
+                    L.pop()
+                    entry[1].C_lo = C.addressof(dq)
+                    L[entry[0]].what += "+" + prefix + "qkv_proj"
             if r.core is not None and not r.fuse_core:
                 geo = ((rps, nh) if kind == "global" else (gh, gw, nh)) + params
                 prep = () if r.core.endswith("_bf16") else (2 if split3 else 0, None, None, None, C.c_float(1e-6), self.precision)
diff --git a/k-diffusion_amd/ops.py b/k-diffusion_amd/ops.py
--- a/k-diffusion_amd/ops.py
+++ b/k-diffusion_amd/ops.py
@@ -229,6 +229,64 @@
     out = torch.empty(B, h, w, Nn, device=image.device, dtype=act) if out is None else out
     return gemm(image, weight, out, M=B * h * w, N=Nn, K=Cc * ph * pw, a_mode=nat.A_PATCH_NCHW, grid=(h, w),
                 patch=(ph, pw, Cc), sigma=sigma, sigma_data=sigma_data, precision=precision)
+
+
+def _x3s_takes_qkv(M, N, K, cus, opt):
+    if M > opt("x3s_max_rows") or (K & 31) or K < 64 or N % 64:
+        return False
+    wgs = -(-M // 32) * (N // 64)
+    cap = opt("x3s_max_wgs")
+    if cap >= 0:
+        return wgs <= cap
+    mine = 5.0 + float(-(-wgs // cus)) * (1.6 + K / 130.0 + 1.0)
+    return not mine * 1.15 >= (22.0 if K >= 512 else 13.5)
+
+
+def _entry_qkv_supported(dp, dq, device=None):
+    lib = nat.lib()
+
+    def opt(name):
+        return lib.kd_get_option(name.encode(), nat.OPTION_DEFAULT)
+    S3 = nat.PREC_SPLIT3
+    if dp.precision != S3 or dq.precision != S3 or not dp.Wp or not dq.Wp:
+        return False
+    if dp.a_mode != nat.A_PATCH_NCHW or dp.epi != nat.EPI_STORE or dp.norm or dp.a_split or dp.c_split or dp.per_row or dp.out_add != 0.0:
+        return False
+    if (dp.K, dp.N, dp.ph, dp.pw, dp.chan) != (48, 128, 4, 4, 3) or dp.gh <= 0 or dp.gw <= 0 or dp.M <= 0 or dp.M % (dp.gh * dp.gw):
+        return False
+    if dq.a_mode != nat.A_PLAIN or dq.epi != nat.EPI_QKV or not dq.norm or dq.a_split or dq.c_split or dq.per_row:
+        return False
+    if (dq.K, dq.N, dq.n_heads) != (128, 384, 2) or dq.M != dp.M or dq.rows_per_sample != dp.gh * dp.gw or dq.scale_stride & 3:
+        return False
+    if not dq.qk_scale or not dq.rope_pos or not dq.rope_freq or dq.A != dp.C:
+        return False
+    if not opt("x3") or not opt("astat") or opt("gemm_debug") or dq.M < opt("x3_min_rows") or (opt("skinny") and dq.M <= 128):
+        return False
+    cus = torch.cuda.get_device_properties(torch.cuda.current_device() if device is None else device).multi_processor_count
+    return not _x3s_takes_qkv(dq.M, dq.N, dq.K, cus, opt)
+
+
+def _patch_in_qkv_descs(image, weight, patch, x, scale, w_qkv, qkv, qk, sigma, sigma_data, eps):
+    B, Cc, H, W = image.shape
+    ph, pw = patch
+    h, w = H // ph, W // pw
+    d = weight.shape[0]
+    M = B * h * w
+    dp = gemm(image, weight, x, M=M, N=d, K=Cc * ph * pw, a_mode=nat.A_PATCH_NCHW, grid=(h, w), patch=(ph, pw, Cc), sigma=sigma,
+              sigma_data=sigma_data, precision=nat.PREC_SPLIT3, launch=False)
+    dq = gemm(x, w_qkv, qkv, M=M, N=w_qkv.shape[0], K=d, epi=nat.EPI_QKV, norm_scale=scale, scale_stride=d if scale.dim() == 2 else 0,
+              rows_per_sample=h * w, eps=eps, qk=qk, qkv_packed=True, precision=nat.PREC_SPLIT3, launch=False)
+    return dp, dq
+
+
+def _patch_in_qkv(image, weight, patch, scale, w_qkv, qk, sigma=None, sigma_data=1.0, x=None, qkv=None, eps=1e-6):
+    B, _, H, W = image.shape
+    x = torch.empty(B, H // patch[0], W // patch[1], weight.shape[0], device=image.device, dtype=torch.float32) if x is None else x
+    qkv = torch.empty(*x.shape[:-1], w_qkv.shape[0], device=image.device, dtype=torch.float32) if qkv is None else qkv
+    dp, dq = _patch_in_qkv_descs(image, weight, patch, x, scale, w_qkv, qkv, qk, sigma, sigma_data, eps)
+    dp.C_lo = C.addressof(dq)
+    nat.check(nat.lib().kd_gemm_f32(C.byref(dp), _stream()), "kd_gemm_f32(patch-in + qkv)")
+    return x, qkv
 
 
 def patch_out(x, norm_scale, weight, patch, channels, x_in=None, sigma=None, sigma_data=1.0, out=None, eps=1e-6):
```

Measured after the change: 246.9, median of 6. About the same (+0.8%).
